# Kiteretsu77/This_and_That_VDM

Measured on AMD Instinct MI355X. Metric: denoise-steps/sec (14-frame 256x448 VGL, 25 steps), higher is better.
Workload: dtype bf16; 1 GPU; VGL denoise step: GestureNet ControlNet + spatio-temporal UNet + per-frame CFG + Euler, latent 14x4x32x56, CFG batch 2, 78 context tokens, heads (5,10,20,20); mode=vgl, requests_per_gpu=1, parallelism=1 independent request(s), one per GPU; RCCL weight broadcast at start-up only, hipgraph=True, finite_output=True, spatial_self_attention=bf16, weights_identical_on_all_ranks=True

## Files before the change

this_and_that_vdm_amd/csrc/gemm.hip:

```cpp
#include <stdlib.h>
#include "gemm_kernel.h"

namespace ttg {
void launch_bf16(GemmP& p, int cfg, hipStream_t st);
void launch_f16(GemmP& p, int cfg, hipStream_t st);
void launch_f32(GemmP& p, int cfg, hipStream_t st);
void launch_sq320_bf16(const GemmP& p, hipStream_t st);
void launch_sq320_f16(const GemmP& p, hipStream_t st);
void launch_pp_bf16(GemmP& p, hipStream_t st);
void launch_pp_f16(GemmP& p, hipStream_t st);
void launch_w320_bf16(GemmP& p, hipStream_t st);
void launch_w320_f16(GemmP& p, hipStream_t st);
void launch_w320h_bf16(GemmP& p, hipStream_t st);
void launch_w320h_f16(GemmP& p, hipStream_t st);
}
using namespace ttg;

namespace {
inline int gemm_taps(int mode) { return mode == 1 || mode == 3 ? 9 : (mode == 2 ? 3 : 1); }

int env_int(const char* name, int dflt) { const char* e = getenv(name); return e ? atoi(e) : dflt; }
int big_tile_bits(int on) { return on == 0 ? 0 : (on == 2 ? 1 : (on == 3 ? 11 : (on == 4 ? 7 : 15))); }
struct Knobs {
  int forced_cfg = env_int("TT_GEMM_CFG", -1);
  int group_m = env_int("TT_GEMM_GROUP_M", 0);
  int forced_split = env_int("TT_GEMM_SPLITK", -1);
  int deep = env_int("TT_GEMM_DEEP", 1);
  int small64 = env_int("TT_GEMM_SMALL64", 2);
  int sq320 = env_int("TT_GEMM_SQ320", 2);
  int sq320_rowvec = env_int("TT_SQ320_ROWVEC", 1);
  int sq320_min_rows = env_int("TT_SQ320_MIN_ROWS", 131072);
  int pp = env_int("TT_GEMM_PP", 1);
  int pp_geglu_min_tiles = env_int("TT_PP_GEGLU_MIN_TILES", 400);
  int pp_geglu_min_fill = env_int("TT_PP_GEGLU_MIN_FILL", 75);
  int pp_min_tiles = env_int("TT_PP_MIN_TILES", 460);
  int pp_min_fill = env_int("TT_PP_MIN_FILL", 90);
  int pp_split_whole = env_int("TT_PP_SPLIT_WHOLE", 1);
  int w320 = big_tile_bits(env_int("TT_GEMM_W320", 1));
  int w320_force = env_int("TT_W320_FORCE", 0);
  int w320_min_fill = env_int("TT_W320_MIN_FILL", 60);
  int f32_split = env_int("TT_F32_SPLIT", 0) ? 1 : 0;
  int f32_split_min_tiles = env_int("TT_F32_SPLIT_MIN_TILES", 160);
  int f32_splitk = env_int("TT_F32_SPLITK", 1);
};
Knobs& knobs() { static Knobs k; return k; }

struct Plan { int cfg, splitk; };

Plan make_plan(int forced, int m, int n, long ktot, bool allow_split, bool wide_ok = true, bool mode0 = false, bool k128 = false) {
  Plan pl{0, 1};
  const int f = forced;
  const long b128 = (long)ceil_div(m, 128) * ceil_div(n, 128);
  const long b12864 = (long)ceil_div(m, 128) * ceil_div(n, 64);
  if (f >= 0 && f < kNumCfgs) pl.cfg = f;
  else if (n % 160 == 0 && n % 128 != 0 && n <= 960 && m >= 2048) pl.cfg = 7;
  else if (m >= 8192 && n >= 1024 && wide_ok) pl.cfg = 3;
  else if (m < 2048 && n >= 2560 && n % 160 == 0) pl.cfg = 7;
  else if (b128 >= 384) pl.cfg = 11;
  else if (b12864 >= 384) pl.cfg = 1;
  else pl.cfg = 2;
  const int fs = knobs().forced_split;
  if (fs >= 1) { pl.splitk = allow_split ? fs : 1; return pl; }
  const long kt = (ktot + 63) / 64;
  const int deep = knobs().deep;
  if (deep && f < 0 && b128 <= 256 && ktot > 0) {
    const int small64 = knobs().small64;
    if (small64 && (small64 != 2 || (m <= 64 && n >= 4096)) && mode0 && ktot <= 2048 && (long)ceil_div(m, 64) * ceil_div(n, 64) <= 512) { pl.cfg = 2; return pl; }
    pl.cfg = (deep == 2 && k128) ? 20 : 16;
    long s = allow_split ? 256 / b128 : 1;
    if (s > kt / 8) s = kt / 8;
    if (s > 16) s = 16;
    pl.splitk = s >= 2 ? (int)s : 1;
    return pl;
  }
  if (allow_split && f < 0 && b128 < 384 && kt >= 40) {
    long s = (512 + b128 - 1) / b128;
    if (s > kt / 8) s = kt / 8;
    if (s > 16) s = 16;
    if (s >= 2) { pl.cfg = 11; pl.splitk = (int)s; }
  }
  return pl;
}

int plan_f32(int m, int n, int min_tiles = 256) { return (long)ceil_div(m, 128) * ceil_div(n, 128) >= min_tiles ? 0 : 1; }

bool sq320_rowvec_ok(const TtGemmArgs* a) {
  if (!a->rowvec) return true;
  if (!knobs().sq320_rowvec || !a->residual) return false;
  if (a->rowvec_mod == 2 && a->rowvec_rows == 1) return true;
  return a->rowvec_mod == 0 && a->rowvec_rows >= 32 && a->rowvec_rows % 32 == 0 && (long)a->rowvec_rows * 2 >= a->m;
}
bool sq320_ok(const TtGemmArgs* a) {
  const int on = knobs().sq320;
  if (on == 2 && a->m < knobs().sq320_min_rows) return false;
  return on && a->dtype != TT_F32 && !a->ln_fold && !a->out_fp8 && knobs().forced_cfg < 0 && a->mode == 0 && a->k1 == 0 && a->k0 == SQ_K && a->n == SQ_N && a->m >= 4096 &&
         !a->geglu && sq320_rowvec_ok(a) && !a->out_f32 && !a->out_col_hw &&
         (!a->blend || (a->blend == a->residual && a->ld_blend == a->ld_res));
}
bool pp_ok(const TtGemmArgs* a) {
  const Knobs& k = knobs();
  if (!k.pp || k.forced_cfg >= 0 || a->dtype == TT_F32 || a->mode != 0 || a->k1 != 0 || a->ln_fold > 1 || a->out_fp8 || a->residual || a->blend ||
      a->rowvec || a->out_f32 || a->out_col_hw || (a->k0 & 63) || a->k0 < 128 || (a->n & 15) || (a->ldo & 7))
    return false;
  const long tiles = (long)ceil_div(a->m, 256) * ceil_div(a->n, 256);
  const long rounds = (tiles + 255) / 256;
  if (a->geglu) return tiles >= k.pp_geglu_min_tiles && tiles * 100 >= rounds * 256 * k.pp_geglu_min_fill;
  return tiles >= k.pp_min_tiles && tiles * 100 >= rounds * 256 * k.pp_min_fill;
}
bool w320_eligible(const TtGemmArgs* a) {
  if (!knobs().w320 || knobs().forced_cfg >= 0 || a->mode == 3 || a->dtype == TT_F32 || a->n % 320 || (a->k0 & 63) || (a->k1 & 63) || gemm_taps(a->mode) * (a->k0 + a->k1) < 128 || a->geglu ||
      a->out_fp8 || a->out_f32 || a->out_col_hw || a->ln_fold > 1 || (a->ln_fold && (a->mode != 0 || a->k1)))
    return false;
  if (a->mode == 1 && (a->stride != 1 || a->upsample || a->hin != a->hout || a->win != a->wout || a->win >= 32768 || a->hin >= 32768)) return false;
  if (a->rowvec && a->rowvec_rows < 32 && !(a->rowvec_rows == 1 && a->rowvec_mod == 2)) return false;
  if ((a->ldo & 3) || (a->residual && (a->ld_res & 3)) || (a->blend && (a->ld_blend & 3)) || (a->rowvec && (a->ld_rowvec & 3))) return false;
  if ((((size_t)a->out | (size_t)a->residual | (size_t)a->blend) & 7) || (((size_t)a->rowvec | (size_t)a->bias) & 15)) return false;
  return true;
}
int w320_route(const TtGemmArgs* a) {
  if (!w320_eligible(a)) return 0;
  const Knobs& k = knobs();
  if (k.w320_force == 1 || k.w320_force == 2) return k.w320_force;
  for (int half = 0; half < 2; ++half) {
    if (half && (!(k.w320 & 2) || ((k.w320 & 4) && a->mode != 1))) break;
    const long tiles = (long)ceil_div(a->m, half ? 128 : 256) * (a->n / 320);
    const long rounds = (tiles + 255) / 256;
    if (tiles * 100 >= rounds * 256 * k.w320_min_fill) return 1 + half;
  }
  return 0;
}
int w320_split(const TtGemmArgs* a) {
  const int bits = knobs().w320;
  if (!w320_eligible(a) || !(bits & 8) || a->ln_fold || a->mode == 2) return 0;
  const long tiles = (long)ceil_div(a->m, 128) * (a->n / 320);
  if ((bits & 4) && (a->mode != 1 || tiles < 64)) return 0;
  const long slabs = (long)gemm_taps(a->mode) * (a->k0 + a->k1) / 64;
  long s = 256 / tiles;
  const long by_k = slabs / (a->mode == 1 ? 20 : 32);
  if (s > by_k) s = by_k;
  if (s > 16) s = 16;
  if (s < 2 || tiles * s < 160 || s * a->m * a->n * 4 >= (1L << 31)) return 0;
  return (int)s;
}
size_t slab_bytes(const TtGemmArgs* a, int split) { return (size_t)split * a->m * a->n * sizeof(float); }
bool ws_fits(const TtGemmArgs* a, int split) { return a->ws && (size_t)a->ws_bytes >= slab_bytes(a, split); }
int pp_head_rows(const TtGemmArgs* a, bool served) {
  if (a->m < 512) return 0;
  if ((a->m & 255) == 0 && (!knobs().pp_split_whole || served)) return 0;
  TtGemmArgs head = *a;
  for (int tr = a->m >> 8; tr >= 2 && (long)(a->m - tr * 256) * 8 <= a->m; --tr) {
    head.m = tr * 256;
    if (head.m < a->m && pp_ok(&head)) return head.m;
  }
  return 0;
}
void pp_split(const TtGemmArgs* a, int rows, TtGemmArgs* head, TtGemmArgs* tail) {
  const size_t es = 2;
  *head = *a; *tail = *a;
  head->m = rows;
  tail->m = a->m - rows;
  tail->a0 = (const char*)a->a0 + (size_t)rows * a->lda0 * es;
  tail->out = (char*)a->out + (size_t)rows * a->ldo * es;
}

const TileCfg& tile_of(int dtype, int cfg) { return dtype == TT_F32 ? kCfgsF32[cfg] : kCfgs[cfg]; }
bool ln_capable(int cfg) { return kCfgs[cfg].ln; }
bool mode3_capable(int cfg) { return kCfgs[cfg].m3; }
Plan mode3_plan(const TtGemmArgs* a, Plan pl) {
  if (a->mode != 3 || a->dtype == TT_F32 || knobs().forced_cfg >= 0 || mode3_capable(pl.cfg)) return pl;
  if (pl.cfg == 20) return Plan{16, pl.splitk};
  const long b128 = (long)ceil_div(a->m, 128) * ceil_div(a->n, 128), b12864 = (long)ceil_div(a->m, 128) * ceil_div(a->n, 64);
  return Plan{b128 >= 384 ? 11 : (b12864 >= 384 ? 1 : 2), 1};
}
bool mode3_served(const TtGemmArgs* a, const Plan& pl) { return a->mode != 3 || tile_of(a->dtype, pl.cfg).m3; }
Plan plan_for(const TtGemmArgs* a) {
  if (a->dtype == TT_F32) {
    const int split_min = knobs().f32_split_min_tiles;
    if (knobs().f32_split) {
      const long b128 = (long)ceil_div(a->m, 128) * ceil_div(a->n, 128);
      const long kt = (long)gemm_taps(a->mode) * (a->k0 + a->k1) / 32;
      if (knobs().f32_splitk && !a->geglu && !a->ln_fold && !a->out_col_hw && b128 < split_min && kt >= 64) {
        long sp = 448 / b128;
        if (sp > kt / 16) sp = kt / 16;
        if (sp > 16) sp = 16;
        if (sp >= 2) return Plan{0, (int)sp};
      }
    }
    return Plan{plan_f32(a->m, a->n, knobs().f32_split ? split_min : 256), 1};
  }
  const long ktot = (long)gemm_taps(a->mode) * (a->k0 + a->k1);
  const bool allow = !a->geglu && !a->ln_fold && !a->out_fp8;
  const bool k128 = (a->k0 & 127) == 0 && (a->k1 & 127) == 0;
  const bool wide_ok = !(a->residual || a->blend || a->rowvec);
  Plan pl = make_plan(knobs().forced_cfg, a->m, a->n, ktot, allow, wide_ok, a->mode == 0, k128);
  if (a->ln_fold && !ln_capable(pl.cfg))
    pl = make_plan(-1, a->m, a->n, ktot, false, wide_ok, a->mode == 0);
  return mode3_plan(a, pl);
}
Plan unsplit_plan(const TtGemmArgs* a) {
  if (a->dtype == TT_F32) return Plan{plan_f32(a->m, a->n, 256), 1};
  return mode3_plan(a, Plan{make_plan(knobs().forced_cfg, a->m, a->n, 0, false, !(a->residual || a->blend || a->rowvec)).cfg, 1});
}

enum class Kind { PP, PP_TWO_PART, SQ320, W320, W320H, W320H_SPLIT, TILED, UNSUPPORTED };
struct Route { Kind kind; int cfg; int splitk; int head_rows; };

Route tiled_route(const TtGemmArgs* a, Plan pl) { return Route{mode3_served(a, pl) ? Kind::TILED : Kind::UNSUPPORTED, pl.cfg, pl.splitk, 0}; }
Route wanted_route(const TtGemmArgs* a) {
  if (pp_ok(a)) return Route{Kind::PP, -1, 1, 0};
  const bool sq = sq320_ok(a);
  const int big = w320_route(a);
  if (const int rows = pp_head_rows(a, sq || big)) return Route{Kind::PP_TWO_PART, -1, 1, rows};
  if (sq) return Route{Kind::SQ320, -1, 1, 0};
  if (big) return Route{big == 1 ? Kind::W320 : Kind::W320H, -1, 1, 0};
  if (const int split = w320_split(a)) return Route{Kind::W320H_SPLIT, -1, split, 0};
  return tiled_route(a, plan_for(a));
}
Route granted_route(const TtGemmArgs* a, Route r) {
  if (r.kind == Kind::W320H_SPLIT && !ws_fits(a, r.splitk)) r = tiled_route(a, plan_for(a));
  if (r.kind == Kind::TILED && r.splitk > 1 && (!ws_fits(a, r.splitk) || slab_bytes(a, r.splitk) >= ((size_t)1 << 31))) r = tiled_route(a, unsplit_plan(a));
  return r;
}
Route resolve(const TtGemmArgs* a) { return granted_route(a, wanted_route(a)); }

TileCfg route_tile(const TtGemmArgs* a, const Route& r) {
  switch (r.kind) {
    case Kind::PP: case Kind::PP_TWO_PART: return TileCfg{-1, 256, 256, 64, 0, 2, 4};
    case Kind::SQ320: return TileCfg{-1, SQ_ROWS, SQ_N, SQ_K, a->residual ? 3 : 5, 1, SQ_WAVES};
    case Kind::W320: return TileCfg{-1, 256, 320, 64, 0, 4, 2};
    case Kind::W320H: case Kind::W320H_SPLIT: return TileCfg{-1, 128, 320, 64, 0, 2, 2};
    default: return tile_of(a->dtype, r.cfg);
  }
}

int32_t stats_rows_on(const TtGemmArgs* a, const Route& r) {
  if (a->geglu || a->out_fp8 || a->out_f32 || a->out_col_hw > 0 || a->ln_fold == 2) return 0;
  if (r.kind == Kind::PP || r.kind == Kind::PP_TWO_PART || r.kind == Kind::SQ320 || r.kind == Kind::UNSUPPORTED) return 0;
  const int seg = a->stats_seg;
  if (r.splitk != 1) {
    if (seg <= 0) return 0;
    for (int rows = seg < 128 ? seg : 128; rows > 0; --rows)
      if (seg % rows == 0) return a->m % rows == 0 ? rows : 0;
    return 0;
  }
  const TileCfg t = route_tile(a, r);
  if (a->blend && !(a->blend == a->residual && a->ld_blend == a->ld_res)) return 0;
  if (a->rowvec && a->rowvec_rows < 32 && !(a->rowvec_rows == 1 && a->rowvec_mod == 2)) return 0;
  if (t.bm > 128 && t.bn != 320 && a->residual) return 0;
  if (a->dtype == TT_F32 && knobs().f32_split && a->residual) return 0;
  if (t.bn == 320 || t.nst == 0) {
    if (a->m % t.bm) return 0;
    return (t.bm == 128 && seg > 0 && seg % 128 && seg % 64 == 0) ? 64 : t.bm;
  }
  const int wave_rows = t.bm / t.wgm;
  const int rows = (seg <= 0 || seg % t.bm == 0) ? t.bm : (seg % wave_rows == 0 ? wave_rows : t.bm);
  return a->m % rows == 0 ? rows : 0;
}
int32_t gn_fused_on(const TtGemmArgs* a, const Route& r) {
  if (a->dtype == TT_F32 || a->geglu || a->out_fp8 || a->out_f32 || a->out_col_hw > 0 || a->stats_out) return 0;
  const int seg = a->stats_seg;
  if (seg <= 0 || a->m % seg || (a->n & 127)) return 0;
  if (r.kind != Kind::W320H_SPLIT && r.kind != Kind::TILED) return 0;
  if (r.splitk <= 1) return 0;
  return splitk_gn_rows(seg, a->n, nullptr) > 0 ? 1 : 0;
}
}

int tt_internal_f32_split() { return knobs().f32_split; }

extern "C" int tt_gemm_set_tile_override(int32_t cfg) {
  if (cfg < -1 || cfg >= kNumCfgs) TT_FAIL(TT_EINVAL, "tt_gemm_set_tile_override: cfg %d (valid -1..%d)", cfg, kNumCfgs - 1);
  knobs().forced_cfg = cfg;
  return TT_OK;
}
extern "C" int tt_gemm_set_streaming_square(int32_t on) {
  knobs().sq320 = on == 2 ? 2 : (on ? 1 : 0);
  return TT_OK;
}
extern "C" int tt_gemm_set_f32_split(int32_t on) { knobs().f32_split = on ? 1 : 0; return TT_OK; }
extern "C" int tt_gemm_set_big_tile(int32_t on) { knobs().w320 = big_tile_bits(on); return TT_OK; }

extern "C" int tt_gemm_plan(const TtGemmArgs* a, int32_t cfg[7]) {
  if (!a || !cfg || a->m <= 0 || a->n <= 0) TT_FAIL(TT_EINVAL, "tt_gemm_plan: bad arguments");
  const Route r = resolve(a);
  if (r.kind == Kind::UNSUPPORTED)
    TT_FAIL(TT_EUNSUPPORTED, "tt_gemm_plan: forced tile configuration %d has no mode-3 variant (mode 3 is built for 1, 2, 11, 16)", r.cfg);
  const TileCfg t = route_tile(a, r);
  cfg[0] = t.bm; cfg[1] = t.bn; cfg[2] = t.bk; cfg[3] = t.nst; cfg[4] = t.wgm; cfg[5] = t.wgn; cfg[6] = r.splitk;
  return TT_OK;
}

extern "C" int32_t tt_gemm_stats_rows(const TtGemmArgs* a) {
  if (!a || a->m <= 0 || a->n <= 0) return 0;
  return stats_rows_on(a, resolve(a));
}

extern "C" int32_t tt_gemm_gn_fused(const TtGemmArgs* a) {
  if (!a || a->m <= 0 || a->n <= 0) return 0;
  return gn_fused_on(a, resolve(a));
}

extern "C" size_t tt_gemm_ws_bytes(const TtGemmArgs* a) {
  if (!a || a->m <= 0 || a->n <= 0) return 0;
  const Route r = wanted_route(a);
  if (r.kind == Kind::PP_TWO_PART) { TtGemmArgs head, tail; pp_split(a, r.head_rows, &head, &tail); return tt_gemm_ws_bytes(&tail); }
  return (r.kind == Kind::W320H_SPLIT || r.kind == Kind::TILED) && r.splitk > 1 ? slab_bytes(a, r.splitk) : 0;
}

namespace {
int fill_params(const TtGemmArgs* a, const Route& r, GemmP& p) {
  if (a->geglu && ((a->n & 15) || a->residual || a->blend || a->rowvec || a->out_f32 || a->out_col_hw))
    TT_FAIL(TT_EINVAL, "tt_gemm: geglu needs n %% 16 == 0 and no other epilogue terms");
  if (a->rowvec && a->rowvec_rows <= 0) TT_FAIL(TT_EINVAL, "tt_gemm: rowvec_rows");
  if (a->gn_out) {
    if (!a->gn_gamma || !a->gn_beta || (a->ld_gn & 3) || ((size_t)a->gn_out & 7)) TT_FAIL(TT_EINVAL, "tt_gemm: gn_out needs gn_gamma, gn_beta, ld_gn %% 4 == 0 and an 8-byte aligned pointer");
    if (!gn_fused_on(a, r)) TT_FAIL(TT_EUNSUPPORTED, "tt_gemm: gn_out on a problem without a split-K reduction pass (tt_gemm_gn_fused(args) == 0)");
  }
  if (a->stats_out && stats_rows_on(a, r) == 0)
    TT_FAIL(TT_EUNSUPPORTED, "tt_gemm: stats_out on a route without a statistics epilogue (tt_gemm_stats_rows(args) == 0)");
  if (a->rowvec_mod < 0 || (a->rowvec_mod > 0 && !a->rowvec)) TT_FAIL(TT_EINVAL, "tt_gemm: rowvec_mod %d (>= 0, needs rowvec)", a->rowvec_mod);
  if (a->ln_fold < 0 || a->ln_fold > 2) TT_FAIL(TT_EINVAL, "tt_gemm: ln_fold %d (0 none, 1 rows of A, 2 rows of W)", a->ln_fold);
  if (a->ln_fold && (a->mode != 0 || a->k1 != 0 || !(a->ln_eps > 0.f)))
    TT_FAIL(TT_EINVAL, "tt_gemm: ln_fold needs mode 0, one source spanning the whole LayerNorm row (k0 = C) and ln_eps > 0");
  if (a->ln_fold == 2 && a->geglu) TT_FAIL(TT_EINVAL, "tt_gemm: ln_fold 2 (columns) cannot be combined with geglu");
  if (a->out_fp8 && (a->dtype == TT_F32 || a->mode != 0 || a->geglu || a->residual || a->blend || a->rowvec || a->out_f32 || (a->ldo & 3)))
    TT_FAIL(TT_EINVAL, "tt_gemm: out_fp8 is for plain 16-bit linears (no geglu / residual / blend / rowvec / fp32 out), ldo %% 4 == 0");
  p.a0 = (const char*)a->a0; p.a1 = (const char*)a->a1; p.k0 = a->k0; p.k1 = a->k1;
  p.lda0 = a->lda0; p.lda1 = a->lda1; p.w = (const char*)a->w; p.ldw = a->ldw;
  p.m = a->m; p.n = a->n; p.mode = a->mode;
  p.nimg = a->nimg; p.hin = a->hin; p.win = a->win; p.hout = a->hout; p.wout = a->wout;
  p.stride = a->stride; p.upsample = a->upsample; p.frames = a->frames; p.hw = a->hw;
  p.bias = a->bias; p.acc_scale = a->acc_scale;
  p.rowvec = a->rowvec; p.rowvec_rows = a->rowvec_rows; p.ld_rowvec = a->ld_rowvec; p.rowvec_mod = a->rowvec ? a->rowvec_mod : 0;
  p.geglu = a->geglu; p.residual = (const char*)a->residual; p.ld_res = a->ld_res;
  p.blend = (const char*)a->blend; p.ld_blend = a->ld_blend; p.alpha = a->alpha;
  const int es = a->dtype == TT_F32 ? 4 : 2;
  p.out = (char*)a->out; p.ldo = a->ldo; p.out_f32 = a->dtype == TT_F32 ? 0 : a->out_f32;
  p.out_col_hw = a->out_col_hw; p.out_col_hwp = a->out_col_hwp;
  p.ln_fold = a->ln_fold; p.ln_eps = a->ln_eps; p.out_fp8 = a->out_fp8; p.stats = a->stats_out; p.stat_rows = a->gn_out ? a->stats_seg : (a->stats_out ? stats_rows_on(a, r) : 0);
  p.f32_split = a->dtype == TT_F32 ? knobs().f32_split : 0;
  p.presplit = a->presplit;
  if (a->presplit) {
    if ((a->presplit & ~3) || a->dtype != TT_F32 || !p.f32_split)
      TT_FAIL(TT_EINVAL, "tt_gemm: presplit operands need TT_F32 with tt_gemm_set_f32_split(1)");
    if (((a->presplit & 1) && a->ln_fold == 1) || ((a->presplit & 2) && a->ln_fold == 2))
      TT_FAIL(TT_EINVAL, "tt_gemm: the LayerNorm statistics cannot be taken from a pre-split operand");
    if ((a->presplit & 1) && a->mode != 0) TT_FAIL(TT_EINVAL, "tt_gemm: a pre-split A operand is a Linear operand (mode 0)");
  }
  p.gn_out = (char*)a->gn_out; p.ld_gn = a->ld_gn; p.gn_gamma = a->gn_gamma; p.gn_beta = a->gn_beta; p.gn_eps = a->gn_eps; p.gn_silu = a->gn_silu;
  if (p.mode == 1 || p.mode == 3) {
    if (p.nimg <= 0 || p.hin <= 0 || p.win <= 0 || p.hout <= 0 || p.wout <= 0 || p.stride < 1)
      TT_FAIL(TT_EINVAL, "tt_gemm: conv geometry");
    if ((long)p.nimg * p.hout * p.wout != p.m) TT_FAIL(TT_EINVAL, "tt_gemm: m != nimg*hout*wout");
  }
  if (p.mode == 2) {
    if (p.frames <= 0 || p.hw <= 0 || p.m % ((long)p.frames * p.hw)) TT_FAIL(TT_EINVAL, "tt_gemm: tconv geometry");
  }
  p.taps = gemm_taps(p.mode);
  {
    const long rows = p.mode == 1 || p.mode == 3 ? (long)p.nimg * p.hin * p.win : (long)p.m;
    const long a0b = ((rows - 1) * p.lda0 + p.k0) * es, a1b = p.k1 ? ((rows - 1) * p.lda1 + p.k1) * es : 16;
    const long wb = ((long)(p.n - 1) * p.ldw + (long)p.taps * (p.k0 + p.k1)) * es;
    if (a0b >= (1L << 31) || a1b >= (1L << 31) || wb >= (1L << 31))
      TT_FAIL(TT_EUNSUPPORTED, "tt_gemm: operand larger than 2 GiB (32-bit buffer offsets)");
    p.a0_bytes = (unsigned)a0b; p.a1_bytes = (unsigned)a1b; p.w_bytes = (unsigned)wb;
    const long n_out = p.geglu ? p.n / 2 : p.n;
    const long outb = ((long)(p.m - 1) * p.ldo + (p.out_col_hw > 0 ? p.ldo : n_out)) * (p.out_f32 ? 4 : (p.out_fp8 ? 1 : es));
    const long resb = p.residual ? ((long)(p.m - 1) * p.ld_res + p.n) * es : 0;
    const long blb = p.blend ? ((long)(p.m - 1) * p.ld_blend + p.n) * es : 0;
    long rv_last = p.rowvec ? (p.m - 1) / p.rowvec_rows : 0;
    if (p.rowvec_mod > 0 && rv_last > p.rowvec_mod - 1) rv_last = p.rowvec_mod - 1;
    const long rvb = p.rowvec ? (rv_last * p.ld_rowvec + p.n) * 4 : 0;
    if (outb >= (1L << 31) || resb >= (1L << 31) || blb >= (1L << 31) || rvb >= (1L << 31))
      TT_FAIL(TT_EUNSUPPORTED, "tt_gemm: epilogue operand larger than 2 GiB (32-bit buffer offsets)");
    p.out_bytes = (unsigned)outb; p.res_bytes = (unsigned)resb; p.blend_bytes = (unsigned)blb;
    p.bias_bytes = p.bias ? (unsigned)p.n * 4u : 0u; p.rowvec_bytes = (unsigned)rvb;
  }
  p.splitk = r.splitk; p.group_m = 1;
  p.group_m_override = r.kind == Kind::PP || r.kind == Kind::TILED ? knobs().group_m : 0;
  p.ws = r.splitk > 1 ? (float*)a->ws : nullptr;
  p.ws_bytes = r.splitk > 1 ? (unsigned)slab_bytes(a, r.splitk) : 0u;
  return TT_OK;
}
}

extern "C" int tt_gemm(const TtGemmArgs* a, tt_stream_t stream) {
  if (!a || !a->a0 || !a->w || !a->out) TT_FAIL(TT_EINVAL, "tt_gemm: null operand");
  if (a->m <= 0 || a->n <= 0 || a->k0 <= 0) TT_FAIL(TT_EINVAL, "tt_gemm: empty problem m=%d n=%d k0=%d", a->m, a->n, a->k0);
  if (a->dtype != TT_BF16 && a->dtype != TT_F16 && a->dtype != TT_F32) TT_FAIL(TT_EINVAL, "tt_gemm: bad dtype");
  if ((a->k0 & 7) || (a->k1 & 7) || (a->n & 3)) TT_FAIL(TT_EINVAL, "tt_gemm: k0/k1 must be multiples of 8 and n of 4");
  if ((a->lda0 & 7) || (a->k1 && (a->lda1 & 7)) || (a->ldw & 7)) TT_FAIL(TT_EINVAL, "tt_gemm: row strides must be multiples of 8 elements");
  if (a->k1 && !a->a1) TT_FAIL(TT_EINVAL, "tt_gemm: k1 > 0 without a1");
  if (a->mode < 0 || a->mode > 3) TT_FAIL(TT_EINVAL, "tt_gemm: bad mode %d", a->mode);
  if (a->mode == 3 && a->upsample) TT_FAIL(TT_EINVAL, "tt_gemm: mode 3 (bottom / right zero padding) has no fused upsample");
  const Route r = resolve(a);
  if (r.kind == Kind::PP_TWO_PART) {
    TtGemmArgs head, tail;
    pp_split(a, r.head_rows, &head, &tail);
    const int rc = tt_gemm(&head, stream);
    return rc != TT_OK ? rc : tt_gemm(&tail, stream);
  }
  GemmP p;
  if (const int rc = fill_params(a, r, p)) return rc;
  hipStream_t st = (hipStream_t)stream;
  const bool bf16 = a->dtype == TT_BF16;
  switch (r.kind) {
    case Kind::PP: if (bf16) launch_pp_bf16(p, st); else launch_pp_f16(p, st); break;
    case Kind::SQ320: if (bf16) launch_sq320_bf16(p, st); else launch_sq320_f16(p, st); break;
    case Kind::W320: if (bf16) launch_w320_bf16(p, st); else launch_w320_f16(p, st); break;
    case Kind::W320H: case Kind::W320H_SPLIT: if (bf16) launch_w320h_bf16(p, st); else launch_w320h_f16(p, st); break;
    case Kind::TILED:
      if (bf16) launch_bf16(p, r.cfg, st);
      else if (a->dtype == TT_F16) launch_f16(p, r.cfg, st);
      else launch_f32(p, r.cfg, st);
      break;
    default:
      TT_FAIL(TT_EUNSUPPORTED, "tt_gemm: forced tile configuration %d has no mode-3 variant (mode 3 is built for 1, 2, 11, 16)", r.cfg);
  }
  TT_CHECK_LAUNCH("tt_gemm");
  return TT_OK;
}
```

this_and_that_vdm_amd/csrc/gemm_kernel.h:

```cpp
#pragma once
#include <stdlib.h>
#include <type_traits>
#include "common.h"

namespace ttg {


struct FastDiv { unsigned mul, sh; };
static inline FastDiv make_fastdiv(long d_) {
  unsigned long long d = d_ < 1 ? 1 : (unsigned long long)d_;
  unsigned l = 0;
  while ((1ull << l) < d) ++l;
  FastDiv f;
  f.mul = (unsigned)(((1ull << (31 + l)) + d - 1) / d);
  f.sh = 31 + l;
  return f;
}
__device__ __forceinline__ int fdiv(int n, const FastDiv& f) { return (int)(((unsigned long long)(unsigned)n * f.mul) >> f.sh); }

struct GemmP {
  const char* a0; const char* a1;
  int k0, k1; long lda0, lda1;
  const char* w; long ldw;
  int m, n, mode;
  int nimg, hin, win, hout, wout, stride, upsample;
  int frames, hw;
  const float* bias; float acc_scale;
  const float* rowvec; int rowvec_rows; long ld_rowvec;
  int rowvec_mod;
  int geglu;
  const char* residual; long ld_res;
  const char* blend; long ld_blend; float alpha;
  char* out; long ldo; int out_f32;
  int out_col_hw, out_col_hwp;
  int nk0, nk1, taps, kt_total;
  int tiles_m, tiles_n;
  int group_m_override;
  int group_m;
  unsigned a0_bytes, a1_bytes, w_bytes;
  unsigned out_bytes, res_bytes, blend_bytes, bias_bytes, rowvec_bytes, ws_bytes;
  int splitk;
  float* ws;
  int ln_fold; float ln_eps;
  int out_fp8;
  float* stats;
  int stat_rows;
  char* gn_out; long ld_gn;
  const float* gn_gamma; const float* gn_beta; float gn_eps; int gn_silu;
  int f32_split;
  int presplit;
  FastDiv fd_splitk, fd_per_group, fd_group_m, fd_last_rows, fd_per_tap, fd_hwo, fd_wout, fd_hw, fd_frames, fd_rv_rows, fd_rv_mod;
};

__device__ __forceinline__ unsigned pack4_fp8(const float* v) {
  int w = 0;
  w = __builtin_amdgcn_cvt_pk_fp8_f32(__builtin_amdgcn_fmed3f(v[0], -448.f, 448.f), __builtin_amdgcn_fmed3f(v[1], -448.f, 448.f), w, false);
  w = __builtin_amdgcn_cvt_pk_fp8_f32(__builtin_amdgcn_fmed3f(v[2], -448.f, 448.f), __builtin_amdgcn_fmed3f(v[3], -448.f, 448.f), w, true);
  return (unsigned)w;
}
__device__ __forceinline__ void st32(__amdgpu_buffer_rsrc_t r, int off, unsigned a) {
  __builtin_amdgcn_raw_buffer_store_b32(a, r, off, 0, 0);
}

__device__ __forceinline__ void colstat_strip(const char* ebuf, int q_per_row, int lane, float* srow_sum, float* srow_sq, bool first) {
  if (lane < q_per_row * 4) {
    const int quad = lane >> 2, e4 = (lane & 3) * 4;
    float a = 0.f, b = 0.f;
#pragma unroll 8
    for (int r = 0; r < 32; ++r) {
      const float x = *(const float*)(ebuf + r * 256 + ((quad ^ (r & (q_per_row - 1))) << 4) + e4);
      a += x; b = fmaf(x, x, b);
    }
    if (!first) { a += srow_sum[lane]; b += srow_sq[lane]; }
    srow_sum[lane] = a; srow_sq[lane] = b;
  }
}

__device__ __forceinline__ void ln_stat_shifted(const raw_u32x4_t& f, float c, float& s, float& q) {
  const unsigned w[4] = {f.x, f.y, f.z, f.w};
#pragma unroll
  for (int d = 0; d < 4; ++d) { const float x = __uint_as_float(w[d]) - c; s += x; q = fmaf(x, x, q); }
}


#ifdef TT_GEMM_TIMELINE
static __device__ long long g_tl[8 * 8192];
#define TL(i) do { if (threadIdx.x == 0 && blockIdx.x < 8192) g_tl[blockIdx.x * 8 + (i)] = wall_clock64(); } while (0)
#else
#define TL(i) do { } while (0)
#endif

constexpr int kInv = (int)0x80000000;
typedef unsigned u32x2_t __attribute__((ext_vector_type(2)));
typedef unsigned u32x4_t __attribute__((ext_vector_type(4)));
__device__ __forceinline__ __amdgpu_buffer_rsrc_t make_rsrc(const void* ptr, unsigned bytes) {
  return __builtin_amdgcn_make_buffer_rsrc((void*)ptr, 0, (int)bytes, 0x00020000);
}
__device__ __forceinline__ uint2 ld64(__amdgpu_buffer_rsrc_t r, int off) {
  const u32x2_t v = __builtin_amdgcn_raw_buffer_load_b64(r, off, 0, 0);
  return make_uint2(v.x, v.y);
}
__device__ __forceinline__ float4 ld128f(__amdgpu_buffer_rsrc_t r, int off) {
  const u32x4_t v = __builtin_amdgcn_raw_buffer_load_b128(r, off, 0, 0);
  return make_float4(__uint_as_float(v.x), __uint_as_float(v.y), __uint_as_float(v.z), __uint_as_float(v.w));
}
__device__ __forceinline__ void st64(__amdgpu_buffer_rsrc_t r, int off, unsigned a, unsigned b) {
  __builtin_amdgcn_raw_buffer_store_b64((u32x2_t){a, b}, r, off, 0, 0);
}
__device__ __forceinline__ void st128f(__amdgpu_buffer_rsrc_t r, int off, float4 v) {
  __builtin_amdgcn_raw_buffer_store_b128((u32x4_t){__float_as_uint(v.x), __float_as_uint(v.y), __float_as_uint(v.z), __float_as_uint(v.w)}, r, off, 0, 0);
}
template <typename Tag> __device__ __forceinline__ typename Elem<Tag>::quad_t ldq(__amdgpu_buffer_rsrc_t r, int off) { return ld64(r, off); }
template <> __device__ __forceinline__ uint4 ldq<f32_tag>(__amdgpu_buffer_rsrc_t r, int off) {
  const u32x4_t v = __builtin_amdgcn_raw_buffer_load_b128(r, off, 0, 0);
  return make_uint4(v.x, v.y, v.z, v.w);
}
template <typename Tag> __device__ __forceinline__ void stq(__amdgpu_buffer_rsrc_t r, int off, const float* v) {
  st64(r, off, pack2<Tag>(v[0], v[1]), pack2<Tag>(v[2], v[3]));
}
template <> __device__ __forceinline__ void stq<f32_tag>(__amdgpu_buffer_rsrc_t r, int off, const float* v) {
  st128f(r, off, make_float4(v[0], v[1], v[2], v[3]));
}
template <typename Tag> __device__ __forceinline__ typename Elem<Tag>::quad_t zero_quad();
template <> __device__ __forceinline__ uint2 zero_quad<bf16_tag>() { return make_uint2(0, 0); }
template <> __device__ __forceinline__ uint2 zero_quad<f16_tag>() { return make_uint2(0, 0); }
template <> __device__ __forceinline__ uint4 zero_quad<f32_tag>() { return make_uint4(0, 0, 0, 0); }

template <typename Tag> struct EpiOps { float4 bias, rv; typename Elem<Tag>::quad_t res, bl; };
template <typename Tag>
__device__ __forceinline__ EpiOps<Tag> epi_load(const GemmP& p, int gm, int gn) {
  typedef typename Elem<Tag>::quad_t quad_t;
  constexpr int ES = Elem<Tag>::ES;
  EpiOps<Tag> o;
  o.bias = o.rv = make_float4(0.f, 0.f, 0.f, 0.f);
  o.res = o.bl = zero_quad<Tag>();
  if (p.bias) o.bias = *(const float4*)(p.bias + gn);
  if (p.rowvec) {
    int rg = gm / p.rowvec_rows;
    if (p.rowvec_mod > 0) rg %= p.rowvec_mod;
    o.rv = *(const float4*)(p.rowvec + (long)rg * p.ld_rowvec + gn);
  }
  if (p.residual) o.res = *(const quad_t*)(p.residual + ((long)gm * p.ld_res + gn) * ES);
  if (p.blend) o.bl = *(const quad_t*)(p.blend + ((long)gm * p.ld_blend + gn) * ES);
  return o;
}
template <typename Tag>
__device__ __forceinline__ void epi_finish(const GemmP& p, const EpiOps<Tag>& o, int gm, int gn, float (&v)[4]) {
  typedef typename Elem<Tag>::quad_t quad_t;
  constexpr int ES = Elem<Tag>::ES;
  if (p.bias) { v[0] += o.bias.x; v[1] += o.bias.y; v[2] += o.bias.z; v[3] += o.bias.w; }
#pragma unroll
  for (int e = 0; e < 4; ++e) v[e] *= p.acc_scale;
  if (p.rowvec) { v[0] += o.rv.x; v[1] += o.rv.y; v[2] += o.rv.z; v[3] += o.rv.w; }
  if (p.residual) {
    float r4[4];
    quad_to_f32<Tag>(o.res, r4);
#pragma unroll
    for (int e = 0; e < 4; ++e) v[e] += r4[e];
  }
  if (p.blend) {
    float r4[4];
    quad_to_f32<Tag>(o.bl, r4);
#pragma unroll
    for (int e = 0; e < 4; ++e) v[e] = p.alpha * r4[e] + (1.0f - p.alpha) * v[e];
  }
  if (p.out_fp8) {
    if (p.out_col_hw > 0) {
      const unsigned w = pack4_fp8(v);
#pragma unroll
      for (int e = 0; e < 4; ++e) {
        const int c = gn + e;
        const long oc = (long)(c / p.out_col_hw) * p.out_col_hwp + (c % p.out_col_hw);
        *(unsigned char*)(p.out + (long)gm * p.ldo + oc) = (unsigned char)(w >> (8 * e));
      }
    } else {
      *(unsigned*)(p.out + (long)gm * p.ldo + gn) = pack4_fp8(v);
    }
  } else if (p.out_f32) {
    *(float4*)(p.out + ((long)gm * p.ldo + gn) * 4) = make_float4(v[0], v[1], v[2], v[3]);
  } else if (p.out_col_hw > 0) {
#pragma unroll
    for (int e = 0; e < 4; ++e) {
      const int c = gn + e;
      const long oc = (long)(c / p.out_col_hw) * p.out_col_hwp + (c % p.out_col_hw);
      store1<Tag>(p.out + ((long)gm * p.ldo + oc) * ES, v[e]);
    }
  } else {
    *(quad_t*)(p.out + ((long)gm * p.ldo + gn) * ES) = f32_to_quad<Tag>(v);
  }
}

template <typename Tag>
__device__ __forceinline__ void epilogue_quad(const GemmP& p, int gm, int gn, float (&v)[4]) {
  const EpiOps<Tag> o = epi_load<Tag>(p, gm, gn);
  epi_finish<Tag>(p, o, gm, gn, v);
}

template <int N> __device__ __forceinline__ void wait_vmcnt() {
  asm volatile("s_waitcnt vmcnt(%0)" ::"n"(N) : "memory");
}
template <int G> __device__ __forceinline__ void wait_tiles(int tiles) {
  static_assert(3 * G <= 63, "vmcnt field is 6 bits");
  if (tiles <= 0) wait_vmcnt<0>();
  else if (tiles == 1) wait_vmcnt<G>();
  else if (tiles == 2) wait_vmcnt<2 * G>();
  else wait_vmcnt<3 * G>();
}

constexpr int gemm_lds_bytes(int BM, int BN, int CPR, int NST, int NT) {
  return NST * (((BM * CPR + NT - 1) / NT) + ((BN * CPR + NT - 1) / NT)) * NT * 16;
}
constexpr int gemm_min_waves(int BM, int BN, int CPR, int NST, int NT) {
  const int blocks = (160 * 1024) / gemm_lds_bytes(BM, BN, CPR, NST, NT) >= 2 ? 2 : 1;
  const int w = blocks * (NT / 64) / 4;
  return w < 1 ? 1 : w;
}

template <typename Tag, int BM, int BN, int BK, int NST, int WGM, int WGN, int KMODE_>
__global__ __launch_bounds__(64 * WGM * WGN, gemm_min_waves(BM, BN, BK / Elem<Tag>::EPC, NST, 64 * WGM * WGN))
void gemm_kernel(const GemmP p) {
  extern __shared__ __attribute__((aligned(16))) char smem[];
  constexpr bool SPLIT = (KMODE_ & 8) != 0;
  constexpr bool PRE_B = (KMODE_ & 16) != 0, PRE_A = (KMODE_ & 32) != 0;
  constexpr int KMODE = KMODE_ & 7;
  static_assert(SPLIT || (!PRE_A && !PRE_B), "pre-split operands belong to the split variants");
  static_assert(!SPLIT || std::is_same<Tag, f32_tag>::value, "split products are a TT_F32 mode");
  constexpr bool PAD_BR = KMODE == 5;
  constexpr int MODE = PAD_BR ? 1 : (KMODE >= 3 ? 0 : KMODE);
  constexpr int LN = KMODE == 3 || KMODE == 4 ? KMODE - 2 : 0;
  TL(0);
  kernarg_touch<sizeof(GemmP)>();
  typedef typename Elem<Tag>::quad_t quad_t;
  constexpr int ES = Elem<Tag>::ES, EPC = Elem<Tag>::EPC;
  constexpr int NT = 64 * WGM * WGN;
  constexpr int CPR = BK / EPC;
  constexpr int WTM = BM / WGM, WTN = BN / WGN, FM = WTM / 32, FN = WTN / 32;
  constexpr int AR = (BM * CPR + NT - 1) / NT, BR = (BN * CPR + NT - 1) / NT;
  constexpr int A_BYTES = AR * NT * 16, B_BYTES = BR * NT * 16, STAGE = A_BYTES + B_BYTES;
  constexpr int G = AR + BR;
  constexpr int RPI = NT / CPR;
  static_assert(NT % CPR == 0 && NST >= 2 && NST <= 5 && WTM % 32 == 0 && WTN % 32 == 0, "tile/threads mismatch");

  const int tid = threadIdx.x, lane = tid & 63;
  const int wid = __builtin_amdgcn_readfirstlane(tid >> 6);

  int bid = blockIdx.x;
  {
    const int nwg = gridDim.x, q = nwg >> 3, r = nwg & 7, xcd = bid & 7, idx = bid >> 3;
    bid = (xcd < r ? xcd * (q + 1) : r * (q + 1) + (xcd - r) * q) + idx;
  }
  int split = 0;
  if (p.splitk > 1) { const int t = fdiv(bid, p.fd_splitk); split = bid - t * p.splitk; bid = t; }
  int tile_m, tile_n;
  {
    const int gm = p.group_m;
    const int per_group = gm * p.tiles_n;
    const int grp = fdiv(bid, p.fd_per_group);
    const int first = grp * gm;
    const int r = bid - grp * per_group;
    const bool full = first + gm <= p.tiles_m;
    const int rows = full ? gm : p.tiles_m - first;
    tile_n = full ? fdiv(r, p.fd_group_m) : fdiv(r, p.fd_last_rows);
    tile_m = first + (r - tile_n * rows);
  }
  const int m0 = tile_m * BM, n0 = tile_n * BN;
  const int kt_lo = p.splitk > 1 ? fdiv(p.kt_total * split, p.fd_splitk) : 0;
  const int KT = p.splitk > 1 ? fdiv(p.kt_total * (split + 1), p.fd_splitk) - kt_lo : p.kt_total;

  constexpr int INV = (int)0x80000000;
  const __amdgpu_buffer_rsrc_t ra0 = __builtin_amdgcn_make_buffer_rsrc((void*)p.a0, 0, p.a0_bytes, 0x00020000);
  const __amdgpu_buffer_rsrc_t ra1 = __builtin_amdgcn_make_buffer_rsrc((void*)(p.a1 ? p.a1 : p.a0), 0, p.a1_bytes, 0x00020000);
  const __amdgpu_buffer_rsrc_t rw = __builtin_amdgcn_make_buffer_rsrc((void*)p.w, 0, p.w_bytes, 0x00020000);
  const int crow = tid / CPR, cchunk = tid % CPR;
  int a_chunk[AR];
  int va0[AR], va1[AR];
  int a_img[AR], a_y[AR], a_x[AR];
  bool a_valid[AR];
#pragma unroll
  for (int i = 0; i < AR; ++i) {
    const int r = i * RPI + crow;
    a_chunk[i] = cchunk ^ tile_swz<CPR>(r);
    const int gm = m0 + r;
    a_valid[i] = gm < p.m && r < BM;
    const int g = a_valid[i] ? gm : 0;
    va0[i] = va1[i] = INV;
    a_img[i] = a_y[i] = a_x[i] = 0;
    if constexpr (MODE == 0) {
      if (a_valid[i]) {
        va0[i] = (int)(((long)g * p.lda0 + a_chunk[i] * EPC) * ES);
        va1[i] = (int)(((long)g * p.lda1 + a_chunk[i] * EPC) * ES);
      }
    } else if constexpr (MODE == 1) {
      const int hwo = p.hout * p.wout;
      a_img[i] = fdiv(g, p.fd_hwo);
      const int rem = g - a_img[i] * hwo;
      a_y[i] = fdiv(rem, p.fd_wout);
      a_x[i] = rem - a_y[i] * p.wout;
    } else {
      const int fr = fdiv(g, p.fd_hw);
      a_img[i] = fr - fdiv(fr, p.fd_frames) * p.frames;
      a_y[i] = g;
    }
  }
  int b_chunk[BR], vb[BR];
#pragma unroll
  for (int i = 0; i < BR; ++i) {
    const int r = i * RPI + crow;
    b_chunk[i] = cchunk ^ tile_swz<CPR>(r);
    const int gn = n0 + r;
    vb[i] = (gn < p.n && r < BN) ? (int)(((long)gn * p.ldw + b_chunk[i] * EPC) * ES) : INV;
  }

  int s_tap, s_src, s_kc;
  {
    const int per_tap = p.nk0 + p.nk1;
    s_tap = kt_lo ? fdiv(kt_lo, p.fd_per_tap) : 0;
    const int rem = kt_lo - s_tap * per_tap;
    s_src = rem >= p.nk0 ? 1 : 0;
    s_kc = rem - (s_src ? p.nk0 : 0);
  }
  bool tap_dirty = true;
  auto stage = [&](int slot) {
    if constexpr (MODE != 0) {
      if (tap_dirty) {
        tap_dirty = false;
#pragma unroll
        for (int i = 0; i < AR; ++i) {
          bool ok = a_valid[i];
          long row;
          if constexpr (MODE == 1) {
            constexpr int OFF = PAD_BR ? 0 : 1;
            const int dy = s_tap / 3 - OFF, dx = s_tap - (dy + OFF) * 3 - OFF;
            int iy = a_y[i] * p.stride + dy, ix = a_x[i] * p.stride + dx;
            const bool up = !PAD_BR && p.upsample;
            const int hv = up ? p.hin * 2 : p.hin, wv = up ? p.win * 2 : p.win;
            ok = ok && iy >= 0 && iy < hv && ix >= 0 && ix < wv;
            if (up) { iy >>= 1; ix >>= 1; }
            row = ((long)a_img[i] * p.hin + iy) * p.win + ix;
          } else {
            const int f = a_img[i] + s_tap - 1;
            ok = ok && f >= 0 && f < p.frames;
            row = (long)a_y[i] + (long)(s_tap - 1) * p.hw;
          }
          va0[i] = ok ? (int)((row * p.lda0 + a_chunk[i] * EPC) * ES) : INV;
          va1[i] = ok ? (int)((row * p.lda1 + a_chunk[i] * EPC) * ES) : INV;
        }
      }
    }
    const int src = __builtin_amdgcn_readfirstlane(s_src);
    const int ksrc = src ? p.k1 : p.k0;
    const int kbase = __builtin_amdgcn_readfirstlane(s_kc) * BK;
    const bool tail = kbase + BK > ksrc;
    char* lds_a = smem + slot * STAGE + wid * 1024;
    char* lds_b = smem + slot * STAGE + A_BYTES + wid * 1024;
    const int soff_a = kbase * ES;
    const int soff_w = __builtin_amdgcn_readfirstlane(
        (int)(((long)s_tap * (p.k0 + p.k1) + (src ? p.k0 : 0) + kbase) * ES));
    auto issue = [&](const __amdgpu_buffer_rsrc_t& ra, const int (&va)[AR], auto has_tail) {
#pragma unroll
      for (int i = 0; i < AR; ++i) {
        int v = va[i];
        if constexpr (decltype(has_tail)::value) { if (kbase + a_chunk[i] * EPC >= ksrc) v = INV; }
        __builtin_amdgcn_raw_ptr_buffer_load_lds(ra, (__attribute__((address_space(3))) void*)(lds_a + i * (NT * 16)), 16, v, soff_a, 0, 0);
      }
#pragma unroll
      for (int i = 0; i < BR; ++i) {
        int v = vb[i];
        if constexpr (decltype(has_tail)::value) { if (kbase + b_chunk[i] * EPC >= ksrc) v = INV; }
        __builtin_amdgcn_raw_ptr_buffer_load_lds(rw, (__attribute__((address_space(3))) void*)(lds_b + i * (NT * 16)), 16, v, soff_w, 0, 0);
      }
    };
    if (!tail) {
      if (!src) issue(ra0, va0, std::false_type{}); else issue(ra1, va1, std::false_type{});
    } else {
      if (!src) issue(ra0, va0, std::true_type{}); else issue(ra1, va1, std::true_type{});
    }
    if (++s_kc == (s_src ? p.nk1 : p.nk0)) {
      s_kc = 0;
      if (s_src == 0 && p.nk1 > 0) s_src = 1;
      else { s_src = 0; ++s_tap; tap_dirty = true; }
    }
  };

  const int wr = wid / WGN, wc = wid - wr * WGN;
  f32x16_t acc[FM][FN];
#pragma unroll
  for (int i = 0; i < FM; ++i)
#pragma unroll
    for (int j = 0; j < FN; ++j)
#pragma unroll
      for (int r = 0; r < 16; ++r) acc[i][j][r] = 0.f;

  const int l31 = lane & 31, hi = lane >> 5;
  int a_lds_row[FM], b_lds_row[FN];
#pragma unroll
  for (int i = 0; i < FM; ++i) a_lds_row[i] = wr * WTM + i * 32 + l31;
#pragma unroll
  for (int j = 0; j < FN; ++j) b_lds_row[j] = wc * WTN + j * 32 + l31;

  constexpr int KS = CPR / 2;
  static_assert(KS % 2 == 0, "the pipelined loop reads fragment sets in pairs");
  constexpr int NF = FM + FN;
  const unsigned lds_base = lds_addr(smem);
  auto read_frags = [&](unsigned sa, int ks, raw_u32x4_t (&af)[FM], raw_u32x4_t (&bf)[FN]) {
    const unsigned sb = sa + A_BYTES;
    const int chunk = ks * 2 + hi;
#pragma unroll
    for (int i = 0; i < FM; ++i) af[i] = lds_read16_raw(sa + tile_off<CPR>(a_lds_row[i], chunk));
#pragma unroll
    for (int j = 0; j < FN; ++j) bf[j] = lds_read16_raw(sb + tile_off<CPR>(b_lds_row[j], chunk));
  };
  constexpr int NLN = LN == 1 ? FM : (LN == 2 ? FN : 1);
  float ln_s[NLN], ln_q[NLN];
#pragma unroll
  for (int i = 0; i < NLN; ++i) ln_s[i] = ln_q[i] = 0.f;
  constexpr bool LN_SHIFT = LN != 0 && std::is_same<Tag, f32_tag>::value;
  float ln_c[LN_SHIFT ? NLN : 1];
  if constexpr (LN_SHIFT) {
#pragma unroll
    for (int i = 0; i < NLN; ++i) {
      const int row = LN == 1 ? m0 + a_lds_row[i] : n0 + b_lds_row[i];
      const bool ok = row < (LN == 1 ? p.m : p.n);
      ln_c[i] = ok ? *(const float*)((LN == 1 ? p.a0 : p.w) + (long)row * (LN == 1 ? p.lda0 : p.ldw) * 4) : 0.f;
    }
  }
  uint2 sp_ah[SPLIT ? FM : 1], sp_al[SPLIT ? FM : 1], sp_bh[SPLIT ? FN : 1], sp_bl[SPLIT ? FN : 1];
  f32x16_t accx[SPLIT ? FM : 1][SPLIT ? FN : 1];
  if constexpr (SPLIT) {
#pragma unroll
    for (int i = 0; i < FM; ++i)
#pragma unroll
      for (int j = 0; j < FN; ++j)
#pragma unroll
        for (int r = 0; r < 16; ++r) accx[i][j][r] = 0.f;
  }
  const float kM2048 = -2048.0f;
  auto split4 = [&](const raw_u32x4_t& f, bool pre, uint2& h, uint2& l) {
    if (pre) { h = make_uint2(f.x, f.y); l = make_uint2(f.z, f.w); return; }
    const f32x2_t v01 = (f32x2_t){__uint_as_float(f.x), __uint_as_float(f.y)}, v23 = (f32x2_t){__uint_as_float(f.z), __uint_as_float(f.w)};
    const f16x2_t h01 = __builtin_convertvector(v01 * 0.00390625f, f16x2_t), h23 = __builtin_convertvector(v23 * 0.00390625f, f16x2_t);
    h = make_uint2(__builtin_bit_cast(unsigned, h01), __builtin_bit_cast(unsigned, h23));
    const f32x2_t e01 = v01 * 8.0f, e23 = v23 * 8.0f;
    unsigned l01, l23;
    asm("v_fma_mixlo_f16 %0, %1, %2, %3 op_sel_hi:[1,0,0]" : "=v"(l01) : "v"(h.x), "v"(kM2048), "v"(e01.x));
    asm("v_fma_mixhi_f16 %0, %1, %2, %3 op_sel:[1,0,0] op_sel_hi:[1,0,0]" : "+v"(l01) : "v"(h.x), "v"(kM2048), "v"(e01.y));
    asm("v_fma_mixlo_f16 %0, %1, %2, %3 op_sel_hi:[1,0,0]" : "=v"(l23) : "v"(h.y), "v"(kM2048), "v"(e23.x));
    asm("v_fma_mixhi_f16 %0, %1, %2, %3 op_sel:[1,0,0] op_sel_hi:[1,0,0]" : "+v"(l23) : "v"(h.y), "v"(kM2048), "v"(e23.y));
    l = make_uint2(l01, l23);
  };
#if defined(TT_SPLIT_ABL) && (TT_SPLIT_ABL & 1)
  constexpr bool pre_a = true, pre_b = true;
#else
  constexpr bool pre_a = PRE_A, pre_b = PRE_B;
#endif
#ifndef TT_SPLIT_PIPE
#define TT_SPLIT_PIPE 1
#endif
#ifndef TT_SPLIT_PIPE_ROWS
#define TT_SPLIT_PIPE_ROWS 99
#endif
  constexpr int PIPE_SPLIT_ROWS = FM > 1 ? (TT_SPLIT_PIPE_ROWS < FM ? TT_SPLIT_PIPE_ROWS : FM) : FM;
  uint4 op_ah[SPLIT ? FM : 1], op_al[SPLIT ? FM : 1], op_bh[SPLIT ? FN : 1], op_bl[SPLIT ? FN : 1];
  if constexpr (SPLIT) {
#pragma unroll
    for (int i = 0; i < FM; ++i) op_ah[i] = op_al[i] = make_uint4(0, 0, 0, 0);
#pragma unroll
    for (int j = 0; j < FN; ++j) op_bh[j] = op_bl[j] = make_uint4(0, 0, 0, 0);
  }
  auto split4c = [&](const raw_u32x4_t& f, bool pre, uint2& h, uint2& l) {
    if (pre) { h = make_uint2(f.x, f.y); l = make_uint2(f.z, f.w); return; }
    const f32x2_t v01 = (f32x2_t){__uint_as_float(f.x), __uint_as_float(f.y)}, v23 = (f32x2_t){__uint_as_float(f.z), __uint_as_float(f.w)};
    const f16x2_t h01 = __builtin_convertvector(v01 * 0.00390625f, f16x2_t), h23 = __builtin_convertvector(v23 * 0.00390625f, f16x2_t);
    h = make_uint2(__builtin_bit_cast(unsigned, h01), __builtin_bit_cast(unsigned, h23));
    const f32x2_t r01 = v01 * 8.0f - __builtin_convertvector(h01, f32x2_t) * 2048.0f, r23 = v23 * 8.0f - __builtin_convertvector(h23, f32x2_t) * 2048.0f;
    l = make_uint2(__builtin_bit_cast(unsigned, __builtin_convertvector(r01, f16x2_t)), __builtin_bit_cast(unsigned, __builtin_convertvector(r23, f16x2_t)));
  };
  auto issue_pending = [&](auto lo_tag, auto hi_tag) {
   constexpr int LO = decltype(lo_tag)::value, HI = decltype(hi_tag)::value;
   if constexpr (SPLIT) {
#if !defined(TT_SPLIT_ABL) || !(TT_SPLIT_ABL & 2)
#pragma unroll
    for (int i = LO; i < HI; ++i)
#pragma unroll
// ... 124 lines not shown
      const __amdgpu_buffer_rsrc_t r_res = make_rsrc(p.residual, p.res_bytes);
#pragma unroll
      for (int i = 0; i < FM; ++i)
#pragma unroll
        for (int c = 0; c < NCH; ++c) {
          const int nfr = (2 * c + 1 < FN) ? 2 : 1;
          const int q_per_row = nfr * 8, rows_per_pass = 64 / q_per_row;
          const int gn = n0 + wc * WTN + c * 64 + (lane % q_per_row) * 4;
#pragma unroll
          for (int pass = 0; pass < 8; ++pass) {
            resv[i][c][pass] = zero_quad<Tag>();
            if (pass * rows_per_pass < 32) {
              const int gm = m0 + wr * WTM + i * 32 + pass * rows_per_pass + lane / q_per_row;
              resv[i][c][pass] = ldq<Tag>(r_res, (gm < p.m && gn < p.n) ? (int)(((long)gm * p.ld_res + gn) * ES) : kInv);
            }
          }
        }
    }
  };
  if constexpr (NST == 2) {
    TL(6);
    stage(0);
    TL(7);
    preload_residual();
    TL(1);
    for (int kt = 0; kt < KT; ++kt) {
      wait_vmcnt<0>();
      __builtin_amdgcn_s_barrier();
      asm volatile("" ::: "memory");
#ifdef TT_GEMM_TIMELINE
      if (kt == 0) TL(2);
#endif
      if (kt + 1 < KT) stage((kt + 1) & 1);
      const unsigned sa = lds_base + (kt & 1) * STAGE;
      raw_u32x4_t af[2][FM], bf[2][FN];
      read_frags(sa, 0, af[0], bf[0]);
#pragma unroll
      for (int ks = 0; ks < KS; ++ks) {
        if (ks + 1 < KS) {
          read_frags(sa, ks + 1, af[(ks + 1) & 1], bf[(ks + 1) & 1]);
          lds_wait<NF>();
        } else {
          lds_wait<0>();
        }
        mma(af[ks & 1], bf[ks & 1], ks & 1);
      }
    }
  } else {
    TL(6);
    preload_residual();
    TL(1);
#pragma unroll
    for (int s = 0; s < NST - 1; ++s)
      if (s < KT) stage(s);
    wait_tiles<G>(min(KT - 1, NST - 2));
    __builtin_amdgcn_s_barrier();
    asm volatile("" ::: "memory");
    raw_u32x4_t afA[FM], bfA[FN], afB[FM], bfB[FN];
    read_frags(lds_base, 0, afA, bfA);
    int slot = 0, fill = NST - 1;
    auto tile = [&](int kt, auto last_tag) {
      constexpr bool LAST = decltype(last_tag)::value;
      const unsigned sa = lds_base + slot * STAGE;
      const int nslot = slot + 1 == NST ? 0 : slot + 1;
#pragma unroll
      for (int ks = 0; ks < KS; ks += 2) {
        read_frags(sa, ks + 1, afB, bfB);
        lds_wait<NF>();
        mma(afA, bfA, 0);
        if (ks + 2 < KS) {
          read_frags(sa, ks + 2, afA, bfA);
          lds_wait<NF>();
        } else if constexpr (!LAST) {
          wait_tiles<G>(min(KT - 2 - kt, NST - 3));
          __builtin_amdgcn_s_barrier();
          asm volatile("" ::: "memory");
          if (kt + NST - 1 < KT) stage(fill);
          read_frags(lds_base + nslot * STAGE, 0, afA, bfA);
          lds_wait<NF>();
        } else {
          lds_wait<0>();
        }
        mma(afB, bfB, 1);
      }
      slot = nslot;
      fill = fill + 1 == NST ? 0 : fill + 1;
    };
    for (int kt = 0; kt + 1 < KT; ++kt) tile(kt, std::false_type{});
    tile(KT - 1, std::true_type{});
  }

  if constexpr (SPLIT && TT_SPLIT_PIPE) issue_pending(std::integral_constant<int, 0>{}, std::integral_constant<int, FM>{});
  if constexpr (SPLIT) {
#pragma unroll
    for (int i = 0; i < FM; ++i)
#pragma unroll
      for (int j = 0; j < FN; ++j)
#pragma unroll
        for (int r = 0; r < 16; ++r) acc[i][j][r] = fmaf(accx[i][j][r], 32.0f, acc[i][j][r] * 65536.0f);
  }
  constexpr int CS_OFF = NST * STAGE;
  constexpr int STAT_OFF = NST * STAGE + (KMODE == 4 ? WGM * WGN * 1024 : 0);
  if constexpr (LN != 0) {
    const float inv_k = 1.0f / (float)p.k0;
    float rs[NLN];
#pragma unroll
    for (int i = 0; i < NLN; ++i) {
      const float sm = (ln_s[i] + __shfl_xor(ln_s[i], 32)) * inv_k, sq = (ln_q[i] + __shfl_xor(ln_q[i], 32)) * inv_k;
      rs[i] = rsqrtf(fmaxf(sq - sm * sm, 0.f) + p.ln_eps);
    }
    if constexpr (LN == 1) {
#pragma unroll
      for (int i = 0; i < FM; ++i)
#pragma unroll
        for (int j = 0; j < FN; ++j)
#pragma unroll
          for (int r = 0; r < 16; ++r) acc[i][j][r] *= rs[i];
    } else {
      float* cs = (float*)(smem + CS_OFF + wid * 1024);
#pragma unroll
      for (int j = 0; j < FN; ++j) cs[j * 32 + l31] = rs[j];
    }
  }
  const float* colscale = (const float*)(smem + CS_OFF + wid * 1024);

  TL(3);
  if (!direct) {
    const __amdgpu_buffer_rsrc_t r_bias = make_rsrc(p.bias, p.bias_bytes);
    const __amdgpu_buffer_rsrc_t r_out = p.splitk > 1 ? make_rsrc(p.ws, p.ws_bytes) : make_rsrc(p.out, p.out_bytes);
    auto strip_off = [](int row, int quad, int nq) { return row * 256 + ((quad ^ (row & (nq - 1))) << 4); };
    char* ebuf = smem + wid * 8192;
    static_assert(WGM * WGN * 8192 <= NST * STAGE, "epilogue strips do not fit the ring");
    if (!p.geglu) {
      float4 bias4[NCH];
#pragma unroll
      for (int c = 0; c < NCH; ++c) {
        const int q_per_row = ((2 * c + 1 < FN) ? 2 : 1) * 8;
        const int gn = n0 + wc * WTN + c * 64 + (lane % q_per_row) * 4;
        bias4[c] = ld128f(r_bias, gn < p.n ? gn * 4 : kInv);
      }
      const float alpha = p.blend ? p.alpha : 0.0f, one_m_alpha = 1.0f - alpha;
      __syncthreads();
      TL(4);
      auto run = [&](auto film_tag, auto inpass_tag, auto out8_tag, auto stats_tag) {
        constexpr bool FILM = decltype(film_tag)::value, INPASS = decltype(inpass_tag)::value, OUT8 = decltype(out8_tag)::value;
        constexpr bool STATS = decltype(stats_tag)::value;
        const __amdgpu_buffer_rsrc_t r_rv = make_rsrc(p.rowvec, (FILM || INPASS) ? p.rowvec_bytes : 0);
        const __amdgpu_buffer_rsrc_t r_bl = make_rsrc(p.blend, INPASS ? p.blend_bytes : 0);
        const __amdgpu_buffer_rsrc_t r_res = make_rsrc(p.residual, (INPASS && !EARLY_RES) ? p.res_bytes : 0);
        const int rv_rows = p.rowvec ? p.rowvec_rows : 1;
        const bool parity = FILM && p.rowvec_mod == 2 && rv_rows == 1;
        auto wrap = [&](int g) { return p.rowvec_mod > 0 ? g - fdiv(g, p.fd_rv_mod) * p.rowvec_mod : g; };
        float* sstage = (float*)(smem + STAT_OFF) + wid * (2 * WTN);
#pragma unroll
        for (int i = 0; i < FM; ++i) {
          const int mb = m0 + wr * WTM + i * 32;
          const int grp_raw = fdiv(mb, p.fd_rv_rows);
          const int grp0 = parity ? 0 : wrap(grp_raw), grp1 = parity ? 1 : wrap(grp_raw + 1);
          const int grp_split = parity ? mb : (grp_raw + 1) * rv_rows;
          const int sel_split = parity ? 0x7fffffff : grp_split, sel_odd = parity ? 1 : 0;
#pragma unroll
          for (int jc = 0; jc < FN; jc += 2) {
            const int nfr = (jc + 1 < FN) ? 2 : 1;
            const int q_per_row = nfr * 8;
            const int rows_per_pass = 64 / q_per_row;
            const int qq = lane % q_per_row, rr = lane / q_per_row;
            const int gn = n0 + wc * WTN + jc * 32 + qq * 4;
            const float4 b4 = bias4[jc / 2];
            float4 cs4 = make_float4(1.f, 1.f, 1.f, 1.f);
            if constexpr (LN == 2) cs4 = *(const float4*)(colscale + jc * 32 + qq * 4);
            float4 film_lo = make_float4(0.f, 0.f, 0.f, 0.f), film_hi = film_lo;
            if constexpr (FILM) {
              film_lo = ld128f(r_rv, (mb < p.m && gn < p.n) ? (int)(((long)grp0 * p.ld_rowvec + gn) * 4) : kInv);
              film_hi = ld128f(r_rv, (grp_split < p.m && gn < p.n) ? (int)(((long)grp1 * p.ld_rowvec + gn) * 4) : kInv);
            }
#pragma unroll
            for (int jj = 0; jj < 2; ++jj) {
              if (jc + jj < FN) {
#pragma unroll
                for (int g = 0; g < 4; ++g)
                  *(float4*)(ebuf + strip_off(l31, jj * 8 + 2 * g + hi, nfr * 8)) =
                      make_float4(acc[i][jc + jj][g * 4], acc[i][jc + jj][g * 4 + 1], acc[i][jc + jj][g * 4 + 2], acc[i][jc + jj][g * 4 + 3]);
              }
            }
            constexpr int PB = INPASS ? (BM > 128 ? 2 : 4) : 8;
#pragma unroll
            for (int pb = 0; pb < 8; pb += PB) {
              quad_t rqv[PB], blv[PB];
              float4 rvv[PB];
#pragma unroll
              for (int k = 0; k < PB; ++k) {
                const int pass = pb + k;
                rqv[k] = blv[k] = zero_quad<Tag>();
                rvv[k] = make_float4(0.f, 0.f, 0.f, 0.f);
                if (pass * rows_per_pass < 32) {
                  const int gm = mb + pass * rows_per_pass + rr;
                  const bool ok = gm < p.m && gn < p.n;
                  if constexpr (EARLY_RES) rqv[k] = resv[i][jc / 2][pass];
                  else if constexpr (INPASS) rqv[k] = ldq<Tag>(r_res, ok ? (int)(((long)gm * p.ld_res + gn) * ES) : kInv);
                  if constexpr (INPASS) {
                    rvv[k] = ld128f(r_rv, ok ? (int)(((long)wrap(fdiv(gm, p.fd_rv_rows)) * p.ld_rowvec + gn) * 4) : kInv);
                    blv[k] = ldq<Tag>(r_bl, ok ? (int)(((long)gm * p.ld_blend + gn) * ES) : kInv);
                  }
                }
              }
#pragma unroll
              for (int k = 0; k < PB; ++k) {
                const int pass = pb + k;
                if (pass * rows_per_pass < 32) {
                  const int r = pass * rows_per_pass + rr;
                  const float4 t = *(const float4*)(ebuf + strip_off(r, qq, q_per_row));
                  const int gm = mb + r;
                  const bool ok = gm < p.m && gn < p.n;
                  if (p.splitk > 1) {
                    st128f(r_out, ok ? (int)((((long)split * p.m + gm) * p.n + gn) * 4) : kInv, t);
                  } else {
                    float v[4] = {(t.x * cs4.x + b4.x) * p.acc_scale, (t.y * cs4.y + b4.y) * p.acc_scale,
                                  (t.z * cs4.z + b4.z) * p.acc_scale, (t.w * cs4.w + b4.w) * p.acc_scale};
                    const quad_t rq = rqv[k];
                    quad_t bq = rq;
                    if constexpr (FILM) {
                      const float4 f = ((gm >= sel_split) | ((gm & sel_odd) != 0)) ? film_hi : film_lo;
                      v[0] += f.x; v[1] += f.y; v[2] += f.z; v[3] += f.w;
                    }
                    if constexpr (INPASS) {
                      v[0] += rvv[k].x; v[1] += rvv[k].y; v[2] += rvv[k].z; v[3] += rvv[k].w;
                      bq = (p.blend && !blend_is_res) ? blv[k] : rq;
                    }
                    float r4[4], b4v[4];
                    quad_to_f32<Tag>(rq, r4);
                    quad_to_f32<Tag>(bq, b4v);
#pragma unroll
                    for (int e = 0; e < 4; ++e) v[e] = alpha * b4v[e] + one_m_alpha * (v[e] + r4[e]);
                    if constexpr (OUT8) st32(r_out, ok ? (int)((long)gm * p.ldo + gn) : kInv, pack4_fp8(v));
                    else {
                      const quad_t packed = f32_to_quad<Tag>(v);
                      if constexpr (ES == 2) st64(r_out, ok ? (int)(((long)gm * p.ldo + gn) * ES) : kInv, packed.x, packed.y);
                      else stq<Tag>(r_out, ok ? (int)(((long)gm * p.ldo + gn) * ES) : kInv, v);
                      if constexpr (STATS) {
                        float sv[4];
                        quad_to_f32<Tag>(packed, sv);
                        const bool live = gm < p.m;
                        *(float4*)(ebuf + strip_off(r, qq, q_per_row)) = make_float4(live ? sv[0] : 0.f, live ? sv[1] : 0.f, live ? sv[2] : 0.f, live ? sv[3] : 0.f);
                      }
                    }
                  }
                }
              }
            }
            if constexpr (STATS) colstat_strip(ebuf, q_per_row, lane, sstage + jc * 32, sstage + WTN + jc * 32, i == 0);
          }
        }
      };
      const bool inpass = (p.blend && !blend_is_res) || (p.rowvec && p.rowvec_rows < 32 && !(p.rowvec_mod == 2 && p.rowvec_rows == 1)) ||
                          (!EARLY_RES && p.residual);
      constexpr std::false_type no{};
      constexpr std::true_type yes{};
      const bool kstats = p.stats && p.splitk == 1;
      if (inpass) run(no, yes, no, no);
      else if (p.rowvec) { if (kstats) run(yes, no, no, yes); else run(yes, no, no, no); }
      else if (MODE == 0 && ES == 2 && p.out_fp8) {
        if constexpr (MODE == 0 && ES == 2) run(no, no, yes, no);
      } else { if (kstats) run(no, no, no, yes); else run(no, no, no, no); }
      if (kstats) {
        __syncthreads();
        const float* st0 = (const float*)(smem + STAT_OFF);
        if (p.stat_rows == BM) {
          for (int c = tid; c < BN; c += NT) {
            const int wcc = c / WTN, col = c - wcc * WTN;
            float a = 0.f, b = 0.f;
#pragma unroll
            for (int w = 0; w < WGM; ++w) {
              const float* row = st0 + (w * WGN + wcc) * (2 * WTN);
              a += row[col]; b += row[WTN + col];
            }
            if (n0 + c < p.n) {
              p.stats[((long)tile_m * 2) * p.n + n0 + c] = a;
              p.stats[((long)tile_m * 2 + 1) * p.n + n0 + c] = b;
            }
          }
        } else {
          for (int c = tid; c < BN * WGM; c += NT) {
            const int w = c / BN, cc = c - w * BN, wcc = cc / WTN, col = cc - wcc * WTN;
            const float* row = st0 + (w * WGN + wcc) * (2 * WTN);
            const long srow = (long)tile_m * WGM + w;
            if (n0 + cc < p.n && srow * WTM < p.m) {
              p.stats[(srow * 2) * p.n + n0 + cc] = row[col];
              p.stats[(srow * 2 + 1) * p.n + n0 + cc] = row[WTN + col];
            }
          }
        }
      }
    } else {
      float4 bval[FN][2], bgate[FN][2];
#pragma unroll
      for (int j = 0; j < FN; ++j)
#pragma unroll
        for (int tt = 0; tt < 2; ++tt) {
          const int gnp = n0 + wc * WTN + j * 32 + tt * 16 + 4 * hi;
          bval[j][tt] = ld128f(r_bias, gnp < p.n ? gnp * 4 : kInv);
          bgate[j][tt] = ld128f(r_bias, gnp < p.n ? (gnp + 8) * 4 : kInv);
        }
      __syncthreads();
      TL(4);
#pragma unroll
      for (int i = 0; i < FM; ++i) {
        const int mb = m0 + wr * WTM + i * 32;
#pragma unroll
        for (int jc = 0; jc < FN; jc += 2) {
          const int nfr = (jc + 1 < FN) ? 2 : 1;
#pragma unroll
          for (int jj = 0; jj < 2; ++jj) {
            if (jc + jj < FN) {
#pragma unroll
              for (int tt = 0; tt < 2; ++tt) {
                const float4 bv = bval[jc + jj][tt], bg = bgate[jc + jj][tt];
                const float bvv[4] = {bv.x, bv.y, bv.z, bv.w}, bgv[4] = {bg.x, bg.y, bg.z, bg.w};
                float v[4];
#pragma unroll
                for (int e = 0; e < 4; ++e)
                  v[e] = (acc[i][jc + jj][(2 * tt) * 4 + e] + bvv[e]) * gelu_erf_f(acc[i][jc + jj][(2 * tt + 1) * 4 + e] + bgv[e]);
                *(float4*)(ebuf + strip_off(l31, jj * 4 + tt * 2 + hi, nfr * 4)) = make_float4(v[0], v[1], v[2], v[3]);
              }
            }
          }
          const int q_per_row = nfr * 4;
          const int rows_per_pass = 64 / q_per_row;
          const int qq = lane % q_per_row, rr = lane / q_per_row;
          const int oc = ((n0 + wc * WTN + jc * 32) >> 1) + qq * 4;
#pragma unroll
          for (int pass = 0; pass < 4; ++pass) {
            if (pass * rows_per_pass < 32) {
              const int r = pass * rows_per_pass + rr;
              const float4 t = *(const float4*)(ebuf + strip_off(r, qq, q_per_row));
              const int gm = mb + r;
              const float t4[4] = {t.x, t.y, t.z, t.w};
              stq<Tag>(r_out, (gm < p.m && oc * 2 < p.n) ? (int)(((long)gm * p.ldo + oc) * ES) : kInv, t4);
            }
          }
        }
      }
    }
#ifdef TT_GEMM_TIMELINE
    __builtin_amdgcn_s_waitcnt(0);
    TL(5);
#endif
    return;
  }
#pragma unroll
  for (int i = 0; i < FM; ++i) {
    const int gm = m0 + wr * WTM + i * 32 + l31;
    if (gm >= p.m) continue;
#pragma unroll
    for (int j = 0; j < FN; ++j) {
      const int nb = n0 + wc * WTN + j * 32;
#pragma unroll
      for (int g = 0; g < 4; ++g) {
        const int gn = nb + 8 * g + 4 * hi;
        if (gn >= p.n) continue;
        float v[4];
#pragma unroll
        for (int e = 0; e < 4; ++e) v[e] = acc[i][j][g * 4 + e];
        if constexpr (LN == 2) {
          const float4 c4 = *(const float4*)(colscale + j * 32 + 8 * g + 4 * hi);
          v[0] *= c4.x; v[1] *= c4.y; v[2] *= c4.z; v[3] *= c4.w;
        }
        epilogue_quad<Tag>(p, gm, gn, v);
      }
    }
  }
}

constexpr int SQ_K = 320, SQ_N = 320, SQ_ROWS = 32, SQ_WAVES = SQ_N / 32, SQ_NT = 64 * SQ_WAVES;
constexpr int SQ_CPR = SQ_K / 8;
constexpr int SQ_TILE_BYTES = SQ_ROWS * SQ_K * 2;
constexpr int SQ_PASSES = SQ_ROWS * SQ_CPR / SQ_NT;
static_assert(SQ_ROWS * SQ_CPR % SQ_NT == 0 && SQ_CPR % 8 == 0, "sq320 staging");
__device__ __forceinline__ int sq_swz(int row) { return (row >> 1) & 7; }
__device__ __forceinline__ int sq_off(int row, int chunk) { return (row * SQ_CPR + (chunk ^ sq_swz(row))) << 4; }

template <typename Tag, bool HAS_RES, bool HAS_RV = false>
__global__ __launch_bounds__(SQ_NT) void sq320_kernel(const GemmP p) {
  extern __shared__ __attribute__((aligned(16))) char smem[];
  constexpr int G = HAS_RES ? 2 * SQ_PASSES : SQ_PASSES;
  constexpr int SLOT = HAS_RES ? 2 * SQ_TILE_BYTES : SQ_TILE_BYTES;
  constexpr int NST = HAS_RES ? 3 : 5;
  constexpr int KS = SQ_K / 16;
  const int tid = threadIdx.x, lane = tid & 63;
  const int wid = __builtin_amdgcn_readfirstlane(tid >> 6);
  const int l31 = lane & 31, hi = lane >> 5;
  const int ntiles = (p.m + SQ_ROWS - 1) / SQ_ROWS;
// ... 145 lines not shown
      const float4 b = *(const float4*)(p.ws + ((long)s2 * p.m + gm) * p.n + gn);
      a.x += b.x; a.y += b.y; a.z += b.z; a.w += b.w;
    }
    float v[4] = {a.x, a.y, a.z, a.w};
    epi_finish<Tag>(p, o, gm, gn, v);
  }
}

template <typename Tag>
__global__ __launch_bounds__(256) void splitk_epilogue_stats_kernel(const GemmP p) {
  __shared__ float red[32][8][8];
  kernarg_touch<sizeof(GemmP)>();
  const int R = p.stat_rows, rt = blockIdx.x, tid = threadIdx.x;
  const int qd = tid & 7, rl = tid >> 3;
  const int gn = (int)blockIdx.y * 32 + qd * 4;
  float cs[4] = {0.f, 0.f, 0.f, 0.f}, cq[4] = {0.f, 0.f, 0.f, 0.f};
  if (gn < p.n) {
    for (int r = rl; r < R; r += 32) {
      const int gm = rt * R + r;
      const EpiOps<Tag> o = epi_load<Tag>(p, gm, gn);
      float4 a = *(const float4*)(p.ws + (long)gm * p.n + gn);
      for (int s2 = 1; s2 < p.splitk; ++s2) {
        const float4 b = *(const float4*)(p.ws + ((long)s2 * p.m + gm) * p.n + gn);
        a.x += b.x; a.y += b.y; a.z += b.z; a.w += b.w;
      }
      float v[4] = {a.x, a.y, a.z, a.w};
      epi_finish<Tag>(p, o, gm, gn, v);
#pragma unroll
      for (int e = 0; e < 4; ++e) { const float x = round_store<Tag>(v[e]); cs[e] += x; cq[e] = fmaf(x, x, cq[e]); }
    }
  }
#pragma unroll
  for (int e = 0; e < 4; ++e) { red[rl][qd][e] = cs[e]; red[rl][qd][4 + e] = cq[e]; }
  __syncthreads();
  if (tid < 64) {
    const int q2 = tid >> 3, e = tid & 7, c = (int)blockIdx.y * 32 + q2 * 4 + (e & 3);
    if (c < p.n) {
      float t = red[0][q2][e];
#pragma unroll
      for (int l = 1; l < 32; ++l) t += red[l][q2][e];
      p.stats[((long)rt * 2 + (e >> 2)) * p.n + c] = t;
    }
  }
}
template <typename Tag, int MAXR>
__global__ __launch_bounds__(1024) void splitk_epilogue_gn_kernel(const GemmP p, const int rl_n) {
  typedef typename Elem<Tag>::quad_t quad_t;
  constexpr int ES = Elem<Tag>::ES;
  __shared__ double wsum[16][2];
  __shared__ float s_stat[2];
  kernarg_touch<sizeof(GemmP)>();
  const int R = p.stat_rows, sg = blockIdx.x, grp = blockIdx.y, tid = threadIdx.x;
  const int cpg = p.n >> 5, nq = cpg >> 2;
  const int rl = tid / nq, qd = tid - rl * nq;
  const int gn = grp * cpg + qd * 4;
  const bool lane_ok = rl < rl_n;
  float x[MAXR][4];
  int gmr[MAXR];
  bool ok[MAXR];
  EpiOps<Tag> eo[MAXR];
  const float4 g4 = *(const float4*)(p.gn_gamma + gn), b4 = *(const float4*)(p.gn_beta + gn);
#pragma unroll
  for (int i = 0; i < MAXR; ++i) {
    const int r = rl + i * rl_n;
    ok[i] = lane_ok && r < R;
    gmr[i] = sg * R + (ok[i] ? r : R - 1);
    eo[i] = epi_load<Tag>(p, gmr[i], gn);
    const float4 a = *(const float4*)(p.ws + (long)gmr[i] * p.n + gn);
    x[i][0] = a.x; x[i][1] = a.y; x[i][2] = a.z; x[i][3] = a.w;
  }
  for (int s2 = 1; s2 < p.splitk; ++s2) {
#pragma unroll
    for (int i = 0; i < MAXR; ++i) {
      const float4 b = *(const float4*)(p.ws + ((long)s2 * p.m + gmr[i]) * p.n + gn);
      x[i][0] += b.x; x[i][1] += b.y; x[i][2] += b.z; x[i][3] += b.w;
    }
  }
  double cs = 0.0, cq = 0.0;
#pragma unroll
  for (int i = 0; i < MAXR; ++i) {
    if (ok[i]) {
      epi_finish<Tag>(p, eo[i], gmr[i], gn, x[i]);
#pragma unroll
      for (int e = 0; e < 4; ++e) { x[i][e] = round_store<Tag>(x[i][e]); cs += (double)x[i][e]; cq += (double)x[i][e] * (double)x[i][e]; }
    }
  }
#pragma unroll
  for (int o = 32; o > 0; o >>= 1) { cs += __shfl_xor(cs, o); cq += __shfl_xor(cq, o); }
  if ((tid & 63) == 0) { wsum[tid >> 6][0] = cs; wsum[tid >> 6][1] = cq; }
  __syncthreads();
  if (tid == 0) {
    double a = 0.0, b = 0.0;
    for (int w = 0; w < (((int)blockDim.x + 63) >> 6); ++w) { a += wsum[w][0]; b += wsum[w][1]; }
    const double cnt = (double)R * cpg, mean = a / cnt;
    double var = b / cnt - mean * mean;
    if (var < 0.0) var = 0.0;
    s_stat[0] = (float)mean;
    s_stat[1] = (float)(1.0 / sqrt(var + (double)p.gn_eps));
  }
  __syncthreads();
  const float mean = s_stat[0], rstd = s_stat[1];
  const float sc[4] = {rstd * g4.x, rstd * g4.y, rstd * g4.z, rstd * g4.w};
  const float sh[4] = {b4.x - mean * sc[0], b4.y - mean * sc[1], b4.z - mean * sc[2], b4.w - mean * sc[3]};
#pragma unroll
  for (int i = 0; i < MAXR; ++i) {
    if (ok[i]) {
      float y[4];
#pragma unroll
      for (int e = 0; e < 4; ++e) { const float t = fmaf(x[i][e], sc[e], sh[e]); y[e] = p.gn_silu ? silu_f(t) : t; }
      *(quad_t*)(p.gn_out + ((long)gmr[i] * p.ld_gn + gn) * ES) = f32_to_quad<Tag>(y);
    }
  }
}
static inline int splitk_gn_rows(int seg, int n, int* rl_n) {
  const int nq = n / 128;
  if (nq <= 0 || nq > 256 || seg <= 0) return 0;
  for (int mr = 1; mr <= 8; mr *= 2) {
    const int lanes = (seg + mr - 1) / mr;
    if ((long)lanes * nq <= 1024) { if (rl_n) *rl_n = lanes; return mr; }
  }
  return 0;
}
template <typename Tag>
static inline void launch_splitk_epilogue(const GemmP& p, hipStream_t st) {
  if (p.gn_out) {
    int rl_n = 0;
    const int mr = splitk_gn_rows(p.stat_rows, p.n, &rl_n);
    const dim3 grid(p.m / p.stat_rows, 32), block((rl_n * (p.n / 128) + 63) / 64 * 64);
    if (mr == 1) hipLaunchKernelGGL((splitk_epilogue_gn_kernel<Tag, 1>), grid, block, 0, st, p, rl_n);
    else if (mr == 2) hipLaunchKernelGGL((splitk_epilogue_gn_kernel<Tag, 2>), grid, block, 0, st, p, rl_n);
    else if (mr == 4) hipLaunchKernelGGL((splitk_epilogue_gn_kernel<Tag, 4>), grid, block, 0, st, p, rl_n);
    else hipLaunchKernelGGL((splitk_epilogue_gn_kernel<Tag, 8>), grid, block, 0, st, p, rl_n);
    return;
  }
  if (p.stats) {
    hipLaunchKernelGGL(splitk_epilogue_stats_kernel<Tag>, dim3(p.m / p.stat_rows, (p.n + 31) / 32), dim3(256), 0, st, p);
    return;
  }
  long blocks = ((long)p.m * (p.n >> 2) + 255) / 256;
  if (blocks > 2048) blocks = 2048;
  hipLaunchKernelGGL(splitk_epilogue_kernel<Tag>, dim3((unsigned)blocks), dim3(256), 0, st, p);
}

template <typename Tag, int BM, int BN, int BK, int NST, int WGM, int WGN, int MODE>
void launch_mode(const GemmP& p, hipStream_t st) {
  constexpr int NT_ = 64 * WGM * WGN, CPR_ = BK / Elem<Tag>::EPC;
  constexpr size_t lds = (size_t)NST * (((BM * CPR_ + NT_ - 1) / NT_) + ((BN * CPR_ + NT_ - 1) / NT_)) * NT_ * 16
                         + ((MODE & 7) == 4 ? WGM * WGN * 1024 : 0);
  static_assert(lds + (size_t)WGM * WGN * 2 * (BN / WGN) * sizeof(float) <= 160 * 1024, "LDS ring (+ the statistics staging rows) exceeds 160 KiB");
  static_assert((MODE & 7) != 4 || BN / WGN <= 256, "column-scale array: 1 KiB per wave");
  constexpr size_t stat_lds = (size_t)WGM * WGN * 2 * (BN / WGN) * sizeof(float);
  static unsigned long long attr_done = 0;
  tt_lds_opt_in((const void*)gemm_kernel<Tag, BM, BN, BK, NST, WGM, WGN, MODE>, (int)(lds + stat_lds), &attr_done);
  hipLaunchKernelGGL((gemm_kernel<Tag, BM, BN, BK, NST, WGM, WGN, MODE>), dim3(p.tiles_m * p.tiles_n * p.splitk),
                     dim3(64 * WGM * WGN), (p.stats && p.splitk == 1) ? lds + stat_lds : lds, st, p);
  if (p.splitk > 1) launch_splitk_epilogue<Tag>(p, st);
}

static inline void fill_fastdivs(GemmP& p) {
  p.fd_splitk = make_fastdiv(p.splitk);
  p.fd_per_group = make_fastdiv((long)p.group_m * p.tiles_n);
  p.fd_group_m = make_fastdiv(p.group_m);
  p.fd_last_rows = make_fastdiv(p.tiles_m % p.group_m ? p.tiles_m % p.group_m : p.group_m);
  p.fd_per_tap = make_fastdiv(p.nk0 + p.nk1);
  p.fd_hwo = make_fastdiv((long)p.hout * p.wout);
  p.fd_wout = make_fastdiv(p.wout);
  p.fd_hw = make_fastdiv(p.hw);
  p.fd_frames = make_fastdiv(p.frames);
  p.fd_rv_rows = make_fastdiv(p.rowvec ? p.rowvec_rows : 1);
  p.fd_rv_mod = make_fastdiv(p.rowvec_mod > 0 ? p.rowvec_mod : 1);
}

template <typename Tag, int BM, int BN, int BK, int NST, int WGM, int WGN, bool LNOK = false, bool M3OK = false>
void launch_cfg(GemmP& p, hipStream_t st) {
  p.tiles_m = ceil_div(p.m, BM);
  p.tiles_n = ceil_div(p.n, BN);
  {
    constexpr int NT_ = 64 * WGM * WGN, CPR_ = BK / Elem<Tag>::EPC;
    constexpr long lds_ = (long)NST * (((BM * CPR_ + NT_ - 1) / NT_) + ((BN * CPR_ + NT_ - 1) / NT_)) * NT_ * 16;
    const int window = 32 * (lds_ * 2 <= 160 * 1024 ? 2 : 1);
    int gm = p.group_m_override;
    if (gm <= 0) {
      gm = 1;
      if (p.tiles_n > 8)
        while (gm * 2 * BM * gm * 2 <= (long)window * BN && gm * 2 <= p.tiles_m) gm *= 2;
    }
    p.group_m = gm < 1 ? 1 : (gm > p.tiles_m ? p.tiles_m : gm);
  }
  p.nk0 = ceil_div(p.k0, BK); p.nk1 = p.k1 ? ceil_div(p.k1, BK) : 0;
  p.kt_total = p.taps * (p.nk0 + p.nk1);
  fill_fastdivs(p);
  if (p.mode == 3) {
    if constexpr (M3OK) {
      if constexpr (std::is_same<Tag, f32_tag>::value) {
        if (p.f32_split) {
          if (p.presplit & 2) launch_mode<Tag, BM, BN, BK, NST, WGM, WGN, 13 + 16>(p, st); else launch_mode<Tag, BM, BN, BK, NST, WGM, WGN, 13>(p, st);
          return;
        }
      }
      launch_mode<Tag, BM, BN, BK, NST, WGM, WGN, 5>(p, st);
    }
    return;
  }
  if constexpr (std::is_same<Tag, f32_tag>::value) {
    if (p.f32_split) {
      const int pre = p.presplit & 3;
      if (LNOK && p.ln_fold == 1) {
        if (pre & 2) launch_mode<Tag, BM, BN, BK, NST, WGM, WGN, 11 + 16>(p, st); else launch_mode<Tag, BM, BN, BK, NST, WGM, WGN, 11>(p, st);
        return;
      }
      if (LNOK && p.ln_fold == 2) {
        if (pre & 1) launch_mode<Tag, BM, BN, BK, NST, WGM, WGN, 12 + 32>(p, st); else launch_mode<Tag, BM, BN, BK, NST, WGM, WGN, 12>(p, st);
        return;
      }
      switch (p.mode * 4 + pre) {
        case 0: launch_mode<Tag, BM, BN, BK, NST, WGM, WGN, 8>(p, st); break;
        case 1: launch_mode<Tag, BM, BN, BK, NST, WGM, WGN, 8 + 32>(p, st); break;
        case 2: launch_mode<Tag, BM, BN, BK, NST, WGM, WGN, 8 + 16>(p, st); break;
        case 3: launch_mode<Tag, BM, BN, BK, NST, WGM, WGN, 8 + 48>(p, st); break;
        case 4: case 5: launch_mode<Tag, BM, BN, BK, NST, WGM, WGN, 9>(p, st); break;
        case 6: case 7: launch_mode<Tag, BM, BN, BK, NST, WGM, WGN, 9 + 16>(p, st); break;
        case 8: case 9: launch_mode<Tag, BM, BN, BK, NST, WGM, WGN, 10>(p, st); break;
        default: launch_mode<Tag, BM, BN, BK, NST, WGM, WGN, 10 + 16>(p, st); break;
      }
      return;
    }
  }
  if constexpr (LNOK) {
    if (p.ln_fold == 1) { launch_mode<Tag, BM, BN, BK, NST, WGM, WGN, 3>(p, st); return; }
    if (p.ln_fold == 2) { launch_mode<Tag, BM, BN, BK, NST, WGM, WGN, 4>(p, st); return; }
  }
  switch (p.mode) {
    case 0: launch_mode<Tag, BM, BN, BK, NST, WGM, WGN, 0>(p, st); break;
    case 1: launch_mode<Tag, BM, BN, BK, NST, WGM, WGN, 1>(p, st); break;
    default: launch_mode<Tag, BM, BN, BK, NST, WGM, WGN, 2>(p, st); break;
  }
}

template <typename Tag, bool HAS_RES, bool HAS_RV = false>
void launch_sq320(const GemmP& p, hipStream_t st) {
  constexpr size_t lds = (size_t)(HAS_RES ? 3 * 2 * SQ_TILE_BYTES : 5 * SQ_TILE_BYTES) + SQ_WAVES * 4096;
  static_assert(lds <= 160 * 1024, "sq320 LDS");
  static unsigned long long attr_done = 0;
  tt_lds_opt_in((const void*)sq320_kernel<Tag, HAS_RES, HAS_RV>, (int)lds, &attr_done);
  const int ntiles = (p.m + SQ_ROWS - 1) / SQ_ROWS;
  hipLaunchKernelGGL((sq320_kernel<Tag, HAS_RES, HAS_RV>), dim3(ntiles < 256 ? ntiles : 256), dim3(SQ_NT), lds, st, p);
}

#define TT_GEMM_TILES(X) \
  X( 0, 128, 128,  64, 2, 2, 2, false, false)    \
  X( 1, 128,  64,  64, 3, 2, 2, true,  true )    \
  X( 2,  64,  64,  64, 4, 2, 2, true,  true )    \
  X( 3, 256, 128,  32, 3, 4, 2, true,  false)    \
  X( 4, 256, 256,  32, 3, 2, 4, false, false)    \
  X( 5, 128, 128,  32, 3, 2, 2, false, false)    \
  X( 6, 256, 128,  64, 3, 4, 2, false, false)    \
  X( 7, 128, 160,  64, 2, 4, 1, true,  false)    \
  X( 8, 128, 320,  32, 3, 4, 2, false, false)    \
  X( 9, 256, 256,  64, 2, 2, 4, true,  false)    \
  X(10, 128, 128,  64, 4, 2, 2, false, false)    \
  X(11, 128, 128,  64, 2, 4, 2, true,  true )    \
  X(12, 256, 160,  32, 3, 8, 1, false, false)    \
  X(13, 256, 128,  32, 4, 4, 2, false, false)    \
  X(14, 128, 128,  32, 5, 4, 2, false, false)    \
  X(15, 128, 128,  64, 3, 4, 2, false, false)    \
  X(16, 128, 128,  64, 4, 4, 2, true,  true )    \
  X(17, 256, 256,  32, 4, 2, 4, false, false)    \
  X(18, 256, 128,  64, 2, 4, 2, false, false)    \
  X(19, 256, 128,  32, 5, 4, 2, false, false)    \
  X(20, 128, 128, 128, 2, 4, 2, false, false)
#define TT_GEMM_TILES_F32(X) \
  X( 0, 128, 128,  32, 2, 2, 2, true,  true ) \
  X( 1,  64,  64,  32, 4, 2, 2, true,  true )

struct TileCfg { int idx, bm, bn, bk, nst, wgm, wgn; bool ln, m3; };
#define TT_TILE_ROW(i, bm, bn, bk, nst, wgm, wgn, ln, m3) {i, bm, bn, bk, nst, wgm, wgn, ln, m3},
constexpr TileCfg kCfgs[] = {TT_GEMM_TILES(TT_TILE_ROW)};
constexpr TileCfg kCfgsF32[] = {TT_GEMM_TILES_F32(TT_TILE_ROW)};
#undef TT_TILE_ROW
constexpr int kNumCfgs = sizeof(kCfgs) / sizeof(kCfgs[0]);
template <int N> constexpr bool tiles_in_order(const TileCfg (&t)[N]) {
  for (int i = 0; i < N; ++i) if (t[i].idx != i) return false;
  return true;
}
static_assert(tiles_in_order(kCfgs) && tiles_in_order(kCfgsF32), "a tile's index is its position in the table (the planner and launch() both go by it)");

#define TT_TILE_CASE(i, bm, bn, bk, nst, wgm, wgn, ln, m3) case i: launch_cfg<Tag, bm, bn, bk, nst, wgm, wgn, ln, m3>(p, st); break;
template <typename Tag>
void launch(GemmP& p, int cfg, hipStream_t st) {
  switch (cfg) { TT_GEMM_TILES(TT_TILE_CASE) }
}
template <> void launch<f32_tag>(GemmP& p, int cfg, hipStream_t st);

}
```

this_and_that_vdm_amd/ops.py:

```python
from __future__ import annotations

import ctypes as C
import os
from typing import Optional, Tuple

import torch

from . import _lib
from ._lib import TT_BF16, TT_F16, TT_F32, TtAttnArgs, TtConvArgs, TtEncAttnArgs, TtGemmArgs, check
from .packing import PreSplitF32


PROFILE = None


def _prof_begin():
    if PROFILE is None:
        return None
    e = torch.cuda.Event(enable_timing=True)
    e.record()
    return e


def _prof_end(start, name, flops, shape=None):
    if start is not None:
        e = torch.cuda.Event(enable_timing=True)
        e.record()
        PROFILE.append((name, flops, start, e, shape))


import itertools

_SERIAL = itertools.count(1)
_LAST_WRITE = {}


def _wrote(t: torch.Tensor) -> int:
    n = next(_SERIAL)
    _LAST_WRITE[t.untyped_storage().data_ptr()] = n
    for name in ("_tt_stats", "_tt_gn"):
        if hasattr(t, name):
            delattr(t, name)
    return n


def _handoff_valid(t: torch.Tensor, serial: int, ptr: int, shape) -> bool:
    return _LAST_WRITE.get(t.untyped_storage().data_ptr()) == serial and t.data_ptr() == ptr and tuple(t.shape) == shape


_WS = {}
_WS_RETIRED = []
WS_FLOOR_BYTES = 64 << 20


def _workspace(nbytes: int, device) -> torch.Tensor:
    key = (device, torch.cuda.current_stream().cuda_stream)
    buf = _WS.get(key)
    if buf is None or buf.numel() < nbytes:
        if buf is not None:
            _WS_RETIRED.append(buf)
        buf = _WS[key] = torch.empty(max(nbytes, WS_FLOOR_BYTES), dtype=torch.uint8, device=device)
    return buf


def _code(dt: torch.dtype) -> int:
    if dt == torch.bfloat16:
        return TT_BF16
    if dt == torch.float16:
        return TT_F16
    if dt == torch.float32:
        return TT_F32
    raise RuntimeError(f"libttvdm activations/weights must be bfloat16, float16 or float32, got {dt}")


_F32_SPLIT = os.environ.get("TT_F32_SPLIT", "0") not in ("", "0")


def set_f32_split(on: bool) -> None:
    global _F32_SPLIT
    check(_lib.load().tt_gemm_set_f32_split(int(bool(on))), "tt_gemm_set_f32_split")
    _F32_SPLIT = bool(on)


def f32_split() -> bool:
    return _F32_SPLIT


_TAG = {TT_BF16: "bf16_tag", TT_F16: "f16_tag", TT_F32: "f32_tag"}
FP8 = torch.float8_e4m3fn


def _stream():
    return C.c_void_p(torch.cuda.current_stream().cuda_stream)


def _p(t: Optional[torch.Tensor]):
    if t is None:
        return None
    if not t.is_cuda:
        raise RuntimeError("libttvdm ops need tensors on the HIP device (no CPU fallback)")
    return t.data_ptr()


def _rows2d(t: torch.Tensor) -> Tuple[int, int]:
    assert t.dim() == 2 and t.stride(1) == 1, (t.shape, t.stride())
    return t.stride(0), t.shape[1]


def gemm(a0: torch.Tensor, w: torch.Tensor, *, a1: Optional[torch.Tensor] = None, mode: int = 0, conv=None, tconv=None,
         bias=None, acc_scale: float = 1.0, rowvec=None, rowvec_rows: int = 0, rowvec_mod: int = 0, geglu: bool = False, residual=None,
         blend=None, alpha: float = 0.0, out: Optional[torch.Tensor] = None, out_f32: bool = False, m: Optional[int] = None,
         out_col_pad: Optional[Tuple[int, int]] = None, ln_fold: int = 0, ln_eps: float = 1e-5,
         out_fp8: bool = False, stats: int = 0, gn=None) -> torch.Tensor:
    lib = _lib.load()
    g = TtGemmArgs()
    lda0, k0 = _rows2d(a0)
    g.a0, g.k0, g.lda0 = _p(a0), k0, lda0
    if a1 is not None:
        lda1, k1 = _rows2d(a1)
        g.a1, g.k1, g.lda1 = _p(a1), k1, lda1
    ldw, _ = _rows2d(w)
    n = w.shape[0]
    g.w, g.ldw, g.n = _p(w), ldw, n
    g.mode = mode
    if mode in (1, 3):
        g.nimg, g.hin, g.win, g.hout, g.wout, g.stride, g.upsample = conv
        mm = conv[0] * conv[3] * conv[4]
    elif mode == 2:
        g.frames, g.hw = tconv
        mm = a0.shape[0]
    else:
        mm = a0.shape[0]
    g.m = mm if m is None else m
    g.bias, g.acc_scale = _p(bias), acc_scale
    if rowvec is not None:
        g.rowvec, g.rowvec_rows, g.ld_rowvec, g.rowvec_mod = _p(rowvec), rowvec_rows, rowvec.stride(0), int(rowvec_mod)
        need_rows = rowvec_mod if rowvec_mod > 0 else (((mm if m is None else m) - 1) // rowvec_rows + 1)
        if rowvec.dtype != torch.float32 or rowvec.stride(1) != 1 or rowvec.shape[0] < need_rows or rowvec.shape[1] < n:
            raise RuntimeError(f"gemm: rowvec must be fp32 [>= {need_rows}, >= {n}] with contiguous rows, got {tuple(rowvec.shape)} {rowvec.dtype}")
    g.geglu = int(geglu)
    if residual is not None:
        g.residual, g.ld_res = _p(residual), residual.stride(0)
    if blend is not None:
        g.blend, g.ld_blend, g.alpha = _p(blend), blend.stride(0), alpha
    n_out = n // 2 if geglu else n
    if out is None:
        out = torch.empty((g.m, n_out), dtype=FP8 if out_fp8 else (torch.float32 if out_f32 else a0.dtype), device=a0.device)
    if out_fp8 and out.dtype != FP8:
        raise RuntimeError("out_fp8 needs a torch.float8_e4m3fn output tensor")
    g.out, g.ldo, g.out_f32, g.out_fp8 = _p(out), out.stride(0), int(out_f32), int(out_fp8)
    if out_col_pad is not None:
        g.out_col_hw, g.out_col_hwp = out_col_pad
    g.dtype = _code(a0.dtype)
    g.ln_fold, g.ln_eps = int(ln_fold), float(ln_eps)
    if g.dtype == TT_F32 and _F32_SPLIT:
        g.presplit = (1 if isinstance(a0, PreSplitF32) else 0) | (2 if isinstance(w, PreSplitF32) else 0)
    elif isinstance(a0, PreSplitF32) or isinstance(w, PreSplitF32):
        raise RuntimeError("gemm: a pre-split operand outside the split16 mode (set_f32_split changed after the weights were packed: "
                           "call prepare() / begin() again)")
    need = lib.tt_gemm_ws_bytes(C.byref(g))
    if need:
        ws = _workspace(need, a0.device)
        g.ws, g.ws_bytes = ws.data_ptr(), ws.numel()
    sbuf = gnbuf = None
    if stats and gn is not None and GN_FUSED:
        g.stats_seg = int(stats)
        if lib.tt_gemm_gn_fused(C.byref(g)):
            gnbuf = torch.empty((g.m, n), dtype=out.dtype, device=a0.device)
            g.gn_out, g.ld_gn, g.gn_gamma, g.gn_beta, g.gn_eps, g.gn_silu = gnbuf.data_ptr(), n, _p(gn[0]), _p(gn[1]), float(gn[2]), int(bool(gn[3]))
    if stats and gnbuf is None and GN_TILES and g.m * n <= GN_TILES_MAX_ELEMS:
        g.stats_seg = int(stats) if GN_TILES_SEG else 0
        srows = lib.tt_gemm_stats_rows(C.byref(g))
        if srows > 0 and lib.tt_groupnorm_tiles_supported(int(stats), n, srows, g.dtype):
            sbuf = torch.empty(((g.m + srows - 1) // srows, 2, n), dtype=torch.float32, device=a0.device)
            g.stats_out = sbuf.data_ptr()
    ev = _prof_begin()
    check(lib.tt_gemm(C.byref(g), _stream()), "tt_gemm")
    serial = _wrote(out)
    if sbuf is not None:
        out._tt_stats = (sbuf, srows, serial, out.data_ptr(), tuple(out.shape))
    if gnbuf is not None:
        out._tt_gn = (gnbuf, gn[0].data_ptr(), gn[1].data_ptr(), float(gn[2]), bool(gn[3]), int(stats), serial, out.data_ptr(), tuple(out.shape))
    if ev is not None:
        cfg = (C.c_int32 * 7)()
        lib.tt_gemm_plan(C.byref(g), cfg)
        taps = 9 if mode in (1, 3) else (3 if mode == 2 else 1)
        tag = _TAG[g.dtype]
        if cfg[3] == 0 and cfg[1] == 320:
            kname = f"gemm_w320{'h' if cfg[0] == 128 else ''}_kernel<{tag}, {mode}, {int(bool(ln_fold))}>"
        elif cfg[3] == 0:
            kname = f"gemm_pp_kernel<{tag}, {int(bool(ln_fold))}, {int(bool(geglu))}>"
        elif cfg[0] == 32 and cfg[1] == 320:
            kname = f"sq320_kernel<{tag}, {'true' if residual is not None else 'false'}>"
        else:
            kmode = (5 if mode == 3 else mode if not ln_fold else 2 + ln_fold) + (8 if (g.dtype == TT_F32 and _F32_SPLIT) else 0)
            if mode == 3:
                kmode += 16 if g.presplit & 2 else 0
            kname = f"gemm_kernel<{tag}, {', '.join(str(v) for v in cfg[:6])}, {kmode}>"
        _prof_end(ev, kname, 2.0 * g.m * n * taps * (g.k0 + g.k1),
                  shape=(mode, g.m, n, taps * (g.k0 + g.k1), int(geglu), int(residual is not None)))
    return out


CONV3X3_FUSED = os.environ.get("TT_CONV3X3", "0") == "1"


def conv3x3_supported(h: int, w: int, c0: int, c1: int, n: int, dtype: torch.dtype) -> bool:
    if dtype not in (torch.bfloat16, torch.float16):
        return False
    return bool(_lib.load().tt_conv3x3_supported(h, w, c0, c1, n, _code(dtype)))


def conv3x3(x0, x1, w, nimg: int, h: int, wd: int, *, gn=None, silu: bool = True, bias=None, rowvec=None, rowvec_rows: int = 0,
            residual=None, out=None):
    lib = _lib.load()
    a = TtConvArgs()
    a.x0, a.c0, a.ld0 = _p(x0), x0.shape[1], x0.stride(0)
    if x1 is not None:
        a.x1, a.c1, a.ld1 = _p(x1), x1.shape[1], x1.stride(0)
    n = w.shape[0]
    a.w, a.ldw = _p(w), w.stride(0)
    a.nimg, a.h, a.w_img, a.n = nimg, h, wd, n
    if gn is not None:
        a.gn_scale, a.gn_shift, a.silu = _p(gn[0]), _p(gn[1]), int(silu)
    a.bias = _p(bias)
    if rowvec is not None:
        a.rowvec, a.rowvec_rows, a.ld_rowvec = _p(rowvec), rowvec_rows, rowvec.stride(0)
    if residual is not None:
        a.residual, a.ld_res = _p(residual), residual.stride(0)
    if out is None:
        out = torch.empty((nimg * h * wd, n), dtype=x0.dtype, device=x0.device)
    a.out, a.ldo, a.dtype = _p(out), out.stride(0), _code(x0.dtype)
    ev = _prof_begin()
    check(lib.tt_conv3x3(C.byref(a), _stream()), "tt_conv3x3")
    _wrote(out)
    if ev is not None:
        k = 9 * (a.c0 + a.c1)
        _prof_end(ev, f"conv_patch_kernel<{_TAG[a.dtype]}>", 2.0 * nimg * h * wd * n * k, shape=(1, nimg * h * wd, n, k, 0, int(residual is not None)))
    return out


ATTN_QPROJ = os.environ.get("TT_ATTN_QPROJ", "1") != "0"


def attention_qproj_supported(x, head_dim: int, mask: int) -> bool:
    return ATTN_QPROJ and mask != 0 and head_dim == 64 and x.dtype in (torch.float16, torch.bfloat16) and x.shape[-1] % 64 == 0 and \
        x.stride(0) % 8 == 0 and x.stride(1) == 1


def attention(q, k, vt, out, *, nseq, lq, heads, head_dim, mask, lk, k_seq_stride, v_seq_stride, frames=1, ctx_batches=1,
              batch0=0, qx=None, wq=None, bq=None, ln_eps: float = 1e-5, v_rows: bool = False):
    lib = _lib.load()
    a = TtAttnArgs()
    if qx is not None:
        if wq.dtype != qx.dtype or bq.dtype != torch.float32 or not bq.is_contiguous() or wq.stride(1) != 1 or \
                tuple(wq.shape) != (heads * head_dim, qx.shape[1]) or bq.numel() != heads * head_dim:
            raise RuntimeError(f"attention: fused query projection needs wq [{heads * head_dim}, {qx.shape[1]}] in {qx.dtype} and a contiguous "
                               f"fp32 bq [{heads * head_dim}]; got wq {tuple(wq.shape)} {wq.dtype}, bq {tuple(bq.shape)} {bq.dtype}")
        a.qx, a.ldqx, a.wq, a.ldwq, a.bq, a.qc, a.ln_eps = _p(qx), qx.stride(0), _p(wq), wq.stride(0), _p(bq), qx.shape[1], float(ln_eps)
        q = qx
    else:
        a.q, a.ldq = _p(q), q.stride(0)
    a.k, a.ldk = _p(k), k.stride(0)
    a.vt, a.ldvt = _p(vt), vt.stride(0)
    a.out, a.ldo = _p(out), out.stride(0)
    a.nseq, a.lq, a.heads, a.head_dim = nseq, lq, heads, head_dim
    a.mask, a.lk, a.k_seq_stride, a.v_seq_stride = mask, lk, k_seq_stride, v_seq_stride
    fp8 = q.dtype == FP8
    if fp8 and not (k.dtype == FP8 and vt.dtype == FP8):
        raise RuntimeError("fp8 attention needs q, k and vt in torch.float8_e4m3fn")
    a.frames, a.ctx_batches, a.dtype, a.batch0, a.fp8 = frames, ctx_batches, _code(out.dtype if fp8 else q.dtype), batch0, int(fp8)
    a.v_rows = int(bool(v_rows))
    ev = _prof_begin()
    check(lib.tt_attention(C.byref(a), _stream()), "tt_attention")
    _wrote(out)
    if ev is not None:
        tag = _TAG[a.dtype]
        if fp8:
            kname = f"attn8_kernel<{tag}, {head_dim}>"
        elif v_rows and lk >= 128 and lk % 64 == 0 and os.environ.get("TT_ATTN_PIPE", "1") != "0":
            kname = f"attn_pipe_kernel<{tag}>"
        else:
            kname = f"attn_kernel<{tag}, {head_dim}, {mask}{', true' if qx is not None else ''}{', false, true' if v_rows else ''}>"
        flops = 4.0 * nseq * heads * lq * lk * head_dim + (2.0 * nseq * lq * heads * head_dim * qx.shape[1] if qx is not None else 0.0)
        _prof_end(ev, kname, flops, shape=("attn", nseq * heads, lq, lk, mask, 0))
    return out


def temporal_attention(qkv, out, *, batch, frames, hw, heads, head_dim):
    lib = _lib.load()
    check(lib.tt_temporal_attention(_p(qkv), qkv.stride(0), _p(out), out.stride(0), batch, frames, hw, heads, head_dim,
                                    _code(qkv.dtype), _stream()), "tt_temporal_attention")
    _wrote(out)
    return out


def groupnorm_stats(x0, x1, nimg, hw, frames_per_group, gamma, beta, eps):
    lib = _lib.load()
    c0 = x0.shape[-1]
    c1 = 0 if x1 is None else x1.shape[-1]
    c = c0 + c1
    ws_bytes = lib.tt_groupnorm_ws_bytes(nimg, hw, c)
    ws = torch.empty(ws_bytes // 8, dtype=torch.float64, device=x0.device)
    scale = torch.empty((nimg, c), dtype=torch.float32, device=x0.device)
    shift = torch.empty_like(scale)
    check(lib.tt_groupnorm_stats(_p(x0), c0, _p(x1), c1, nimg, hw, frames_per_group, _p(gamma), _p(beta), eps,
                                 _p(scale), _p(shift), _p(ws), ws_bytes, _code(x0.dtype), _stream()), "tt_groupnorm_stats")
    return scale, shift


def groupnorm_apply(x0, x1, nimg, hw, scale, shift, silu: bool, out=None):
    lib = _lib.load()
    c0 = x0.shape[-1]
    c1 = 0 if x1 is None else x1.shape[-1]
    if out is None:
        out = torch.empty((nimg * hw, c0 + c1), dtype=x0.dtype, device=x0.device)
    check(lib.tt_groupnorm_apply(_p(x0), c0, _p(x1), c1, nimg, hw, _p(scale), _p(shift), int(silu), _p(out), out.stride(0),
                                 _code(x0.dtype), _stream()), "tt_groupnorm_apply")
    _wrote(out)
    return out


GN_SMALL = os.environ.get("TT_GN_SMALL", "1") != "0"
GN_CROSS_MAX_ROWS = int(os.environ.get("TT_GN_CROSS_ROWS", "0"))


GN_TILES = os.environ.get("TT_GN_TILES", "1") != "0"
GN_TILES_SEG = os.environ.get("TT_GN_TILES_SEG", "1") != "0"
GN_FUSED = os.environ.get("TT_GN_FUSED", "1") != "0"
GN_TILES_MAX_ELEMS = int(os.environ.get("TT_GN_TILES_MAX_ELEMS", str(17 << 20)))
if os.environ.get("TT_GN_EMULATE", "0") == "1":
    raise RuntimeError("TT_GN_EMULATE is no longer read by the library (it produced wrong numbers by design): use tools/gn_emulate.py")


def groupnorm(x0, x1, nimg, hw, frames_per_group, gamma, beta, eps, silu: bool):
    lib = _lib.load()
    c0 = x0.shape[-1]
    c1 = 0 if x1 is None else x1.shape[-1]
    fz = getattr(x0, "_tt_gn", None) if x1 is None else None
    if fz is not None and fz[1:6] == (gamma.data_ptr(), beta.data_ptr(), float(eps), bool(silu), frames_per_group * hw) and \
            _handoff_valid(x0, *fz[6:]):
        return fz[0]
    st = getattr(x0, "_tt_stats", None) if (GN_TILES and x1 is None) else None
    if st is not None and not _handoff_valid(x0, *st[2:]):
        st = None
    if st is not None and nimg % frames_per_group == 0 and x0.is_contiguous() and st[0].shape[2] == c0 and \
            lib.tt_groupnorm_tiles_supported(frames_per_group * hw, c0, st[1], _code(x0.dtype)):
        out = torch.empty((nimg * hw, c0), dtype=x0.dtype, device=x0.device)
        check(lib.tt_groupnorm_tiles(_p(x0), c0, _p(st[0]), st[1], nimg // frames_per_group, frames_per_group * hw, _p(gamma), _p(beta), eps,
                                     int(silu), _p(out), out.stride(0), _code(x0.dtype), _stream()), "tt_groupnorm_tiles")
        return out
    if GN_SMALL and frames_per_group > 1 and nimg % frames_per_group == 0 and frames_per_group * hw <= GN_CROSS_MAX_ROWS and \
            lib.tt_groupnorm_small_supported(frames_per_group * hw, c0 + c1, _code(x0.dtype)):
        nimg, hw, frames_per_group = nimg // frames_per_group, frames_per_group * hw, 1
# ... 298 lines not shown
```

this_and_that_vdm_amd/packing.py:

```python
from __future__ import annotations

import os

import torch


def pack_conv3x3(w: torch.Tensor) -> torch.Tensor:
    o, i = w.shape[:2]
    return w.permute(0, 2, 3, 1).reshape(o, 9 * i).contiguous()


def pack_tconv3(w: torch.Tensor) -> torch.Tensor:
    o, i = w.shape[:2]
    return w[:, :, :, 0, 0].permute(0, 2, 1).reshape(o, 3 * i).contiguous()


def pack_conv1x1(w: torch.Tensor) -> torch.Tensor:
    return w.reshape(w.shape[0], w.shape[1]).contiguous()


def pack_geglu(w: torch.Tensor, b: torch.Tensor):
    n2, k = w.shape
    half = n2 // 2
    assert half % 8 == 0
    wp = w.view(2, half // 8, 8, k).permute(1, 0, 2, 3).reshape(n2, k).contiguous()
    bp = b.view(2, half // 8, 8).permute(1, 0, 2).reshape(n2).contiguous()
    return wp, bp


def pad_rows(w: torch.Tensor, multiple: int) -> torch.Tensor:
    n = w.shape[0]
    np_ = (n + multiple - 1) // multiple * multiple
    if np_ == n:
        return w
    out = torch.zeros((np_,) + tuple(w.shape[1:]), dtype=w.dtype, device=w.device)
    out[:n] = w
    return out


DEVICE_ROUNDING = os.environ.get("TT_ZSR_DEVICE", "1") != "0"


def zero_sum_round(w: torch.Tensor, dtype: torch.dtype) -> torch.Tensor:
    if dtype == torch.float32:
        return w.float().contiguous()
    mant, emin = {torch.bfloat16: (7, -126), torch.float16: (10, -14)}[dtype]
    if w.is_cuda and w.dtype == torch.float32 and w.dim() == 2 and w.shape[1] <= 16384 and DEVICE_ROUNDING:
        from . import _lib, ops
        wc = w.detach().contiguous()
        q0 = wc.to(dtype)
        nz = q0 != 0
        if not bool(nz.any()):
            return q0.contiguous()
        _, e = torch.frexp(q0.float().abs())
        e = torch.clamp(e - 1, min=emin)
        hi, lo = int(e[nz].max()), int(e[nz].min())
        out = torch.empty_like(q0)
        _lib.check(_lib.load().tt_zero_sum_round(wc.data_ptr(), wc.stride(0), wc.shape[0], wc.shape[1], hi, lo, out.data_ptr(), out.stride(0),
                                                 ops._code(dtype), ops._stream()), "tt_zero_sum_round")
        return out
    wd = w.detach().double()
    q = w.detach().to(dtype).double()
    up = q > wd
    dn = q < wd
    _, e = torch.frexp(q.abs())
    e = torch.clamp(e - 1, min=emin)
    nz = q != 0
    r = q.sum(dim=1)
    lo = int(e[nz].min()) if bool(nz.any()) else 0
    hi = int(e[nz].max()) if bool(nz.any()) else -1
    moved = torch.zeros_like(nz)
    for only_other_neighbour in (True, False):
        for lvl in range(hi, max(lo, hi - 48) - 1, -1):
            if not bool((r != 0).any()):
                break
            u = 2.0 ** (lvl - mant)
            want = torch.round(r / u).abs()
            if not bool((want != 0).any()):
                continue
            mask = nz & (e == lvl) & ~moved
            if only_other_neighbour:
                mask = mask & torch.where((r > 0)[:, None], up, dn)
            cnt = mask.sum(dim=1)
            n = torch.minimum(want, cnt.double()) * torch.sign(r)
            sel = mask & (torch.cumsum(mask, dim=1, dtype=torch.int32) <= n.abs()[:, None])
            q = q - sel.double() * (torch.sign(n) * u)[:, None]
            moved = moved | sel
            r = r - n * u
    out = q.to(dtype)
    assert torch.equal(out.double(), q), "zero_sum_round: a corrected value is not representable"
    return out.contiguous()


def fold_layernorm(weight: torch.Tensor, bias, gamma: torch.Tensor, beta: torch.Tensor):
    w = weight.detach().float()
    wg = w * gamma.detach().float()[None, :]
    wc = wg - wg.mean(dim=1, keepdim=True)
    b = w @ beta.detach().float()
    if bias is not None:
        b = b + bias.detach().float()
    return wc.contiguous(), b.contiguous()


def permute_q_rows(t: torch.Tensor) -> torch.Tensor:
    n = t.shape[0]
    if n % 16:
        raise ValueError("permute_q_rows: row count must be a multiple of 16")
    idx = torch.arange(n, device=t.device)
    d = (idx & ~12) | ((idx & 4) << 1) | ((idx & 8) >> 1)
    return t[d].contiguous()


class PreSplitF32(torch.Tensor):
    """An fp32-typed [N, K] matrix whose bytes are the pre-split fp16 pairs of TtGemmArgs.presplit (see presplit_f32).  The subclass
    is the marker ops.gemm looks for; row slices / row permutations / contiguous() keep it (and stay valid: the pairing is per row,
    in aligned groups of 4 columns).  Arithmetic on it is meaningless -- pre-split LAST, after every fold that reads the values."""


def presplit_f32(w: torch.Tensor) -> torch.Tensor:
    if isinstance(w, PreSplitF32):
        return w
    if w.dtype != torch.float32 or w.dim() != 2 or w.shape[1] % 4:
        raise ValueError(f"presplit_f32: fp32 [N, K] with K % 4 == 0 expected, got {tuple(w.shape)} {w.dtype}")
    n, k = w.shape
    xs = w.detach().contiguous() * 2.0 ** -8
    h = xs.to(torch.float16)
    l = ((xs - h.float()) * 2048.0).to(torch.float16)
    pairs = torch.stack([h.view(n, k // 4, 4), l.view(n, k // 4, 4)], 2)
    return pairs.reshape(n, 2 * k).contiguous().view(torch.float32).as_subclass(PreSplitF32)
```

this_and_that_vdm_amd/svd/autoencoder_kl_temporal_decoder.py:

```python
from __future__ import annotations

import math
from types import SimpleNamespace
from typing import Optional, Tuple

import torch
import torch.nn as nn

from .. import ops
from ..packing import pack_conv3x3, pack_tconv3
from .layers import Geom, PackRegistry, SpatioTemporalResBlock, Upsample2D, _f32, _Packable
from .modeling_utils import CONFIG_NAME, ConfigMixin, ModelMixin, register_to_config
from .vae_encoder import DiagonalGaussianDistribution, Encoder


def _res(cin: int, cout: int) -> SpatioTemporalResBlock:
    return SpatioTemporalResBlock(cin, cout, temb_channels=None, eps=1e-6, temporal_eps=1e-5, merge_factor=0.0,
                                  merge_strategy="learned", switch_spatial_to_temporal_mix=True)


class VaeAttention(_Packable):

    def __init__(self, query_dim: int, heads: int, dim_head: int, eps: float = 1e-6, norm_num_groups: int = 32):
        super().__init__()
        if heads != 1:
            raise NotImplementedError("the temporal VAE decoder uses one attention head (attention_head_dim = channels)")
        if norm_num_groups != 32:
            raise NotImplementedError("GroupNorm kernels are built for 32 groups")
        self.dim, self.eps = query_dim, eps
        self.group_norm = nn.GroupNorm(norm_num_groups, query_dim, eps=eps)
        self.to_q = nn.Linear(query_dim, query_dim, bias=True)
        self.to_k = nn.Linear(query_dim, query_dim, bias=True)
        self.to_v = nn.Linear(query_dim, query_dim, bias=True)
        self.to_out = nn.ModuleList([nn.Linear(query_dim, query_dim, bias=True), nn.Dropout(0.0)])

    def pack(self, reg, dtype):
        cv = lambda t: t.detach().to(dtype).contiguous()
        self.gamma, self.beta = _f32(self.group_norm.weight), _f32(self.group_norm.bias)
        self.wq, self.bq = cv(self.to_q.weight), _f32(self.to_q.bias)
        self.wk, self.bk = cv(self.to_k.weight), _f32(self.to_k.bias)
        self.wv = cv(self.to_v.weight)
        self.wo = cv(self.to_out[0].weight)
        self.bo = (_f32(self.to_out[0].bias) + self.wo.float() @ _f32(self.to_v.bias)).contiguous()
        self._scratch = {}

    def _scratch_for(self, like: torch.Tensor, n: int, l: int, lp: int):
        key = (like.device, like.dtype, n, l, torch.cuda.current_stream().cuda_stream)
        buf = self._scratch.get(key)
        if buf is None:
            buf = self._scratch[key] = (torch.zeros((self.dim, n * lp), dtype=like.dtype, device=like.device),
                                        torch.empty((l, lp), dtype=torch.float32, device=like.device))
        return buf

    def forward(self, x: torch.Tensor, g: Geom) -> torch.Tensor:
        c, l = self.dim, g.hw
        if l % 4:
            raise NotImplementedError(f"VAE attention over {l} tokens per frame: h*w must be a multiple of 4 (latents are multiples of 8)")
        lp = (l + 7) // 8 * 8
        xn = ops.groupnorm(x, None, g.n, l, 1, self.gamma, self.beta, self.eps, False)
        q = ops.gemm(xn, self.wq, bias=self.bq)
        k = ops.gemm(xn, self.wk, bias=self.bk)
        vt, scores = self._scratch_for(x, g.n, l, lp)
        ops.gemm(self.wv, xn, out=vt, out_col_pad=(l, lp) if lp != l else None)
        o = torch.empty((g.m, c), dtype=x.dtype, device=x.device)
        scale = 1.0 / math.sqrt(c)
        for f in range(g.n):
            rows = slice(f * l, (f + 1) * l)
            ops.gemm(q[rows], k[rows], acc_scale=scale, out=scores[:, :l], out_f32=x.dtype != torch.float32)
            p = ops.softmax_rows(scores, x.dtype, cols=l)
            ops.gemm(p, vt[:, f * lp:(f + 1) * lp], out=o[rows])
        return ops.gemm(o, self.wo, bias=self.bo, residual=x)


class MidBlockTemporalDecoder(_Packable):
    def __init__(self, in_channels: int, out_channels: int, attention_head_dim: int = 512, num_layers: int = 1):
        super().__init__()
        self.resnets = nn.ModuleList([_res(in_channels if i == 0 else out_channels, out_channels) for i in range(num_layers)])
        self.attentions = nn.ModuleList([VaeAttention(in_channels, in_channels // attention_head_dim, attention_head_dim)])

    def pack(self, reg, dtype):
        for m in list(self.resnets) + list(self.attentions):
            m.pack(reg, dtype)

    def forward(self, x, g: Geom):
        x = self.resnets[0](x, None, g, None)
        for resnet, attn in zip(list(self.resnets)[1:], self.attentions):
            x = attn(x, g)
            x = resnet(x, None, g, None)
        return x


class UpBlockTemporalDecoder(_Packable):
    def __init__(self, in_channels: int, out_channels: int, num_layers: int = 1, add_upsample: bool = True):
        super().__init__()
        self.resnets = nn.ModuleList([_res(in_channels if i == 0 else out_channels, out_channels) for i in range(num_layers)])
        self.upsamplers = nn.ModuleList([Upsample2D(out_channels, use_conv=True, out_channels=out_channels)]) if add_upsample else None

    def pack(self, reg, dtype):
        for m in self.resnets:
            m.pack(reg, dtype)
        if self.upsamplers is not None:
            self.upsamplers[0].pack(reg, dtype)

    def forward(self, x, g: Geom):
        for resnet in self.resnets:
            x = resnet(x, None, g, None)
        if self.upsamplers is not None:
            x, g = self.upsamplers[0](x, g)
        return x, g


class TemporalDecoder(_Packable):
    CIN_PAD = 8

    def __init__(self, in_channels: int = 4, out_channels: int = 3, block_out_channels: Tuple[int, ...] = (128, 256, 512, 512),
                 layers_per_block: int = 2):
        super().__init__()
        if in_channels > self.CIN_PAD or out_channels > 4:
            raise NotImplementedError("latent channels <= 8 and image channels <= 4")
        self.in_channels, self.out_channels = in_channels, out_channels
        self.conv_in = nn.Conv2d(in_channels, block_out_channels[-1], 3, padding=1)
        self.mid_block = MidBlockTemporalDecoder(num_layers=layers_per_block, in_channels=block_out_channels[-1],
                                                 out_channels=block_out_channels[-1], attention_head_dim=block_out_channels[-1])
        self.up_blocks = nn.ModuleList([])
        rev = list(reversed(block_out_channels))
        out_ch = rev[0]
        for i in range(len(block_out_channels)):
            prev, out_ch = out_ch, rev[i]
            self.up_blocks.append(UpBlockTemporalDecoder(num_layers=layers_per_block + 1, in_channels=prev, out_channels=out_ch,
                                                         add_upsample=i != len(block_out_channels) - 1))
        self.conv_norm_out = nn.GroupNorm(32, block_out_channels[0], eps=1e-6)
        self.conv_act = nn.SiLU()
        self.conv_out = nn.Conv2d(block_out_channels[0], out_channels, 3, padding=1)
        self.time_conv_out = nn.Conv3d(out_channels, out_channels, (3, 1, 1), padding=(1, 0, 0))

    def pack(self, reg, dtype):
        w = self.conv_in.weight.detach()
        wp = torch.zeros((w.shape[0], self.CIN_PAD, 3, 3), dtype=w.dtype, device=w.device)
        wp[:, :self.in_channels] = w
        self.w_in, self.b_in = pack_conv3x3(wp.to(dtype)), _f32(self.conv_in.bias)
        self.mid_block.pack(reg, dtype)
        for b in self.up_blocks:
            b.pack(reg, dtype)
        self.g_out, self.be_out = _f32(self.conv_norm_out.weight), _f32(self.conv_norm_out.bias)
        w = self.conv_out.weight.detach()
        wo = torch.zeros((self.CIN_PAD,) + tuple(w.shape[1:]), dtype=w.dtype, device=w.device)
        wo[:self.out_channels] = w
        bo = torch.zeros(self.CIN_PAD, dtype=torch.float32, device=w.device)
        bo[:self.out_channels] = self.conv_out.bias.detach().float()
        self.w_out, self.b_out = pack_conv3x3(wo.to(dtype)), bo
        w = self.time_conv_out.weight.detach()
        wt = torch.zeros((4, self.CIN_PAD, 3, 1, 1), dtype=w.dtype, device=w.device)
        wt[:self.out_channels, :self.out_channels] = w
        bt = torch.zeros(4, dtype=torch.float32, device=w.device)
        bt[:self.out_channels] = self.time_conv_out.bias.detach().float()
        self.w_t, self.b_t = pack_tconv3(wt.to(dtype)), bt

    def forward(self, z: torch.Tensor, num_frames: int, dtype: torch.dtype) -> torch.Tensor:
        n, _, h, w = z.shape
        if n % num_frames:
            raise ValueError(f"{n} latent frames are not a multiple of num_frames = {num_frames}")
        g = Geom(n // num_frames, num_frames, h, w)
        x = ops.nchw_to_tokens(z, dtype, ld=self.CIN_PAD)
        x = ops.gemm(x, self.w_in, mode=1, conv=(n, h, w, h, w, 1, 0), bias=self.b_in)
        x = self.mid_block(x, g)
        for blk in self.up_blocks:
            x, g = blk(x, g)
        x = ops.groupnorm(x, None, g.n, g.hw, 1, self.g_out, self.be_out, 1e-6, True)
        x = ops.gemm(x, self.w_out, mode=1, conv=(n, g.h, g.w, g.h, g.w, 1, 0), bias=self.b_out)
        x = ops.gemm(x, self.w_t, mode=2, tconv=(g.frames, g.hw), bias=self.b_t)
        return ops.tokens_to_nchw(x, n, self.out_channels, g.h, g.w, torch.float32)


class AutoencoderKLTemporalDecoder(ModelMixin, ConfigMixin):

    _config_exclude = ("encoder",)

    @register_to_config
    def __init__(self, in_channels: int = 3, out_channels: int = 3, block_out_channels: Tuple[int, ...] = (128, 256, 512, 512),
                 layers_per_block: int = 2, latent_channels: int = 4, sample_size: int = 768, scaling_factor: float = 0.18215,
                 force_upcast: bool = True, encoder=None, native_encoder: bool = False):
        super().__init__()
        if native_encoder and encoder is not None:
            raise ValueError("native_encoder=True runs encode() on the model's own encoder: do not pass a stock encoder= as well")
        self.decoder = TemporalDecoder(latent_channels, out_channels, tuple(block_out_channels), layers_per_block)
        self.native_encoder = bool(native_encoder)
        if self.native_encoder:
            self.encoder = Encoder(in_channels, latent_channels, tuple(block_out_channels), layers_per_block)
            self.quant_conv = nn.Conv2d(2 * latent_channels, 2 * latent_channels, 1)
        self.compute_dtype: Optional[torch.dtype] = None
        self._packed_key = None
        self.__dict__["_stock_encoder"] = None
        self.with_encoder(encoder)

    def with_encoder(self, encoder):
        if encoder is not None and self.native_encoder:
            raise ValueError("this model runs its own encoder (native_encoder=True): a stock encoder cannot be attached")
        if encoder is not None and not callable(getattr(encoder, "encode", None)):
            raise TypeError("encoder must provide encode(x) returning an object with .latent_dist (diffusers' AutoencoderKLTemporalDecoder)")
        self.__dict__["_stock_encoder"] = encoder
        return self

    @classmethod
    def from_pretrained(cls, pretrained_model_name_or_path, *args, encoder=None, **kwargs):
        import json
        import os
        path = pretrained_model_name_or_path
        sub = kwargs.get("subfolder", args[0] if args else None)
        cfg_file = os.path.join(os.path.join(path, sub) if sub else path, CONFIG_NAME)
        if os.path.isfile(cfg_file):
            with open(cfg_file) as f:
                cfg = json.load(f)
            native = kwargs.get("native_encoder", cfg.get("native_encoder", False))
            kinds = cfg.get("down_block_types")
            if native and kinds is not None and any(k != "DownEncoderBlock2D" for k in kinds):
                raise ValueError(f"native_encoder: {cfg_file} names down_block_types {kinds}; only DownEncoderBlock2D is implemented")
        model = super().from_pretrained(pretrained_model_name_or_path, *args, **kwargs)
        return model.with_encoder(encoder)

    def _run_dtype(self) -> torch.dtype:
        if self.compute_dtype is not None:
            return self.compute_dtype
        dt = next(self.parameters()).dtype
        return dt if dt in (torch.float16, torch.bfloat16) else torch.bfloat16

    def prepare(self, force: bool = False):
        p0 = next(self.parameters())
        key = (p0.device, self._run_dtype(), sum(p._version for p in self.parameters()), p0.data_ptr())
        if force or self._packed_key != key:
            if p0.device.type != "cuda":
                raise RuntimeError("AutoencoderKLTemporalDecoder: the decoder runs on the MI355X only (no CPU fallback)")
            self.decoder.pack(PackRegistry(), key[1])
            if self.native_encoder:
                self.encoder.pack(PackRegistry(), key[1], self.quant_conv)
            self._packed_key = key
        return self

    def load_state_dict(self, state_dict, strict: bool = True, **kw):
        if self.native_encoder:
            self._packed_key = None
            return super().load_state_dict(state_dict, strict=strict, **kw)
        sd = {k: v for k, v in state_dict.items() if k.startswith("decoder.")}
        self._packed_key = None
        return super().load_state_dict(sd, strict=strict, **kw)

    def _apply(self, fn, *a, **k):
        self._packed_key = None
        stock = self.__dict__.get("_stock_encoder")
        if isinstance(stock, nn.Module):
# ... 52 lines not shown
```

this_and_that_vdm_amd/svd/denoiser_base.py:

```python
from __future__ import annotations

import os

from typing import List, Optional, Tuple

import torch
import torch.nn as nn

from .. import ops
from .layers import Geom, PackRegistry, StepContext, _f32
from .modeling_utils import ModelMixin
from ..packing import pack_conv3x3


def as_tokens(t: torch.Tensor, dtype: torch.dtype) -> torch.Tensor:
    n, c, h, w = t.shape
    if t.dtype == dtype and t.permute(0, 2, 3, 1).is_contiguous():
        return t.permute(0, 2, 3, 1).reshape(n * h * w, c)
    return ops.nchw_to_tokens(t, dtype)


def as_nchw_view(tok: torch.Tensor, g: Geom) -> torch.Tensor:
    return tok.view(g.n, g.h, g.w, tok.shape[1]).permute(0, 3, 1, 2)


_PRESPLIT_ATTRS = {
    "ResnetBlock2D": ("w1", "w2", "ws"), "TemporalResnetBlock": ("w1", "w2"), "Downsample2D": ("w",), "Upsample2D": ("w",),
    "FeedForward": ("wg", "w2"), "BasicTransformerBlock": ("wqkv", "wo1", "wo2"), "TemporalBasicTransformerBlock": ("wqkv", "wo1", "wo2"),
    "TransformerSpatioTemporalModel": ("w_in", "w_out"),
}


def presplit_packed_weights(root: nn.Module) -> None:
    from ..packing import presplit_f32
    for m in root.modules():
        d = m.__dict__
        for name in _PRESPLIT_ATTRS.get(type(m).__name__, ()):
            t = d.get(name)
            if torch.is_tensor(t) and t.dtype == torch.float32 and t.dim() == 2:
                d[name] = presplit_f32(t)
        if type(m).__name__ == "BasicTransformerBlock" and "wqk" in d:
            c2 = d["wqk"].shape[0]
            d["wqk"], d["wv"] = d["wqkv"][:c2], d["wqkv"][c2:]
        q2 = d.get("q2")
        if q2 is not None and not q2.is_fused and q2.w.dtype == torch.float32:
            q2.w, q2._other = presplit_f32(q2.w), None
    for name in ("_w_in", "_w_out", "_k_w", "_v_w"):
        t = root.__dict__.get(name)
        if torch.is_tensor(t) and t.dtype == torch.float32 and t.dim() == 2:
            root.__dict__[name] = presplit_f32(t)
    for name in ("_zero", "_zero_mid"):
        z = root.__dict__.get(name)
        if isinstance(z, list):
            root.__dict__[name] = [(presplit_f32(w), b) if torch.is_tensor(w) and w.dtype == torch.float32 and w.dim() == 2 else (w, b) for w, b in z]
        elif isinstance(z, tuple) and torch.is_tensor(z[0]) and z[0].dtype == torch.float32 and z[0].dim() == 2:
            root.__dict__[name] = (presplit_f32(z[0]),) + tuple(z[1:])


class DenoiserBase(ModelMixin):
    compute_dtype: Optional[torch.dtype] = None
    attention_fp8: bool = False
    zero_context_shortcut: bool = os.environ.get("TT_ZERO_CTX", "1") != "0"

    _pack_gen = 0

    def _pack_key(self):
        pl = self.__dict__.get("_plist")
        if pl is None:
            pl = self.__dict__["_plist"] = list(self.parameters())
        p0 = pl[0]
        return (p0.device, self._run_dtype(), sum(p._version for p in pl), p0.data_ptr(), ops.f32_split())

    def invalidate_packs(self):
        self._packed_key = None
        self.__dict__.pop("_plist", None)

    def _run_dtype(self) -> torch.dtype:
        if self.compute_dtype is not None:
            return self.compute_dtype
        dt = self.dtype
        return dt if dt in (torch.float16, torch.bfloat16) else torch.bfloat16

    def prepare(self, force: bool = False):
        key = self._pack_key()
        if not force and getattr(self, "_packed_key", None) == key:
            return self
        if next(self.parameters()).device.type != "cuda":
            raise RuntimeError(f"{type(self).__name__}: the denoise path runs on the MI355X only; move the model to the "
                               "HIP device first (there is no CPU fallback)")
        dtype = key[1]
        self.__dict__.pop("_plist", None)
        reg = PackRegistry()
        self._pack_modules(reg, dtype)
        self._film_w = torch.cat(reg.film_w, 0).to(dtype).contiguous()
        self._film_b = torch.cat(reg.film_b, 0).float().contiguous()
        self._k_w = torch.cat(reg.k_w, 0).to(dtype).contiguous()
        self._v_w = torch.cat(reg.v_w, 0).to(dtype).contiguous()
        if dtype == torch.float32 and ops.f32_split():
            presplit_packed_weights(self)
        self._packed_key = self._pack_key()
        self._pack_gen = self._pack_gen + 1
        return self

    def _pack_modules(self, reg: PackRegistry, dtype):
        raise NotImplementedError

    def _embed(self, timestep, added_time_ids, batch: int, device) -> torch.Tensor:
        if not torch.is_tensor(timestep):
            t = torch.full((batch,), float(timestep), dtype=torch.float32, device=device)
        else:
            t = timestep.to(device=device, dtype=torch.float32).reshape(-1).expand(batch).contiguous()
        emb = self.time_embedding(self.time_proj(t))
        ids = added_time_ids.to(device=device, dtype=torch.float32).reshape(-1).contiguous()
        te = self.add_time_proj(ids).reshape(batch, -1)
        ae = self.add_embedding
        hid = ops.small_linear(te, ae.w1, ae.b1, act_out=True)
        return ops.small_linear(hid, ae.w2, ae.b2, out=emb, accumulate=True)

    def film_table(self, timesteps: torch.Tensor, added_time_ids: torch.Tensor, batch: int) -> torch.Tensor:
        self.prepare()
        dev = self._film_w.device
        t = timesteps.to(device=dev, dtype=torch.float32).reshape(-1)
        ids = added_time_ids.to(device=dev, dtype=torch.float32).reshape(batch, -1)
        steps = t.numel()
        out = torch.empty((steps, batch, self._film_w.shape[0]), dtype=torch.float32, device=dev)
        per = max(1, 32 // batch)
        for s0 in range(0, steps, per):
            s1 = min(steps, s0 + per)
            rows = (s1 - s0) * batch
            emb = self.time_embedding(self.time_proj(t[s0:s1].repeat_interleave(batch).contiguous()))
            te = self.add_time_proj(ids.repeat(s1 - s0, 1).reshape(-1).contiguous()).reshape(rows, -1)
            ae = self.add_embedding
            hid = ops.small_linear(te, ae.w1, ae.b1, act_out=True)
            ops.small_linear(hid, ae.w2, ae.b2, out=emb, accumulate=True)
            ops.small_linear(emb, self._film_w, self._film_b, act_in=True, out=out[s0:s1].view(rows, -1))
        return out

    def project_context(self, encoder_hidden_states: torch.Tensor):
        self.prepare()
        dtype = self._run_dtype()
        b, s, d = encoder_hidden_states.shape
        sp = (s + 7) // 8 * 8
        pad = torch.zeros((b, sp, d), dtype=dtype, device=encoder_hidden_states.device)
        pad[:, :s] = encoder_hidden_states.to(dtype)
        pad = pad.view(b * sp, d)
        k_all = ops.gemm(pad, self._k_w)
        vt_all = ops.gemm(self._v_w, pad)
        zero_mask = 0
        if self.zero_context_shortcut and not torch.cuda.is_current_stream_capturing():
            flags = (pad.view(b, -1) == 0).all(1).tolist()
            zero_mask = sum(1 << i for i, z in enumerate(flags) if z)
        return (k_all, vt_all, s, sp, zero_mask)

    def _step_context(self, emb: Optional[torch.Tensor], context, film: Optional[torch.Tensor] = None, request_ctx=None) -> StepContext:
        if film is None:
            film = ops.small_linear(emb, self._film_w, self._film_b, act_in=True)
        k_all, vt_all, s, sp, zero_mask = context
        sc = StepContext(film, k_all, vt_all, s, sp, attn_fp8=bool(self.attention_fp8), zero_mask=zero_mask)
        if request_ctx is not None:
            sc.k_req, sc.vt_req = request_ctx
        return sc

    def _encode(self, x, g: Geom, ctx: StepContext):
        skips: List[Tuple[torch.Tensor, Geom]] = [(x, g)]
        for blk in self.down_blocks:
            x, g, outs = blk(x, g, ctx)
            skips.extend(outs)
        return x, g, skips

    _INFERENCE_ONLY = ("{}: inference-only build -- attention runs on the library's HIP kernels (tt_attention), there are no "
                       "AttentionProcessor objects to read or replace")

    @property
    def attn_processors(self):
        raise NotImplementedError(self._INFERENCE_ONLY.format(f"{type(self).__name__}.attn_processors"))

    def set_attn_processor(self, processor):
        raise NotImplementedError(self._INFERENCE_ONLY.format(f"{type(self).__name__}.set_attn_processor"))

    def set_default_attn_processor(self):
# ... 23 lines not shown
```

this_and_that_vdm_amd/svd/layers.py:

```python
from __future__ import annotations

import math
import os
from dataclasses import dataclass
from typing import Dict, List, Optional, Tuple

import torch
import torch.nn as nn

from .. import ops
from ..packing import fold_layernorm, pack_conv1x1, pack_conv3x3, pack_geglu, pack_tconv3, permute_q_rows, zero_sum_round


ZERO_CTX_TEMPORAL = os.environ.get("TT_ZERO_CTX_T", "1") != "0"
ATTN_V_ROWS = os.environ.get("TT_ATTN_V_ROWS", "1") != "0"
MERGE_FRAMES = os.environ.get("TT_XATTN_MERGE_FRAMES", "1") != "0"


@dataclass
class Geom:
    batch: int
    frames: int
    h: int
    w: int
    batch0: int = 0
    batch_total: int = 0
    requests: int = 1

    @property
    def n(self):
        return self.batch * self.frames

    @property
    def hw(self):
        return self.h * self.w

    @property
    def m(self):
        return self.n * self.hw

    @property
    def ctx_batches(self):
        return self.batch_total or self.batch

    @property
    def cfg(self):
        return self.ctx_batches // self.requests

    def film(self, film: torch.Tensor, off: int, c: int) -> torch.Tensor:
        return film[self.batch0:self.batch0 + self.batch, off:off + c]


class StepContext:

    def __init__(self, film: torch.Tensor, k_all: torch.Tensor, vt_all: torch.Tensor, s_ctx: int, s_pad: int,
                 attn_fp8: bool = False, zero_mask: int = 0):
        self.film, self.k_all, self.vt_all, self.s_ctx, self.s_pad = film, k_all, vt_all, s_ctx, s_pad
        self.attn_fp8 = attn_fp8
        self.zero_mask = zero_mask
        self.k_req = self.vt_req = None

    def live_batches(self, g: "Geom"):
        flags = [(self.zero_mask >> (g.batch0 + i)) & 1 for i in range(g.batch)]
        if not any(flags):
            return None
        live = [i for i, z in enumerate(flags) if not z]
        if not live:
            return (0, 0)
        if live[-1] - live[0] + 1 != len(live):
            return None
        return (live[0], len(live))

    def live_classes(self, g: "Geom"):
        cb, nr = g.cfg, g.requests
        if not self.zero_mask or cb < 2 or g.hw % cb or not ZERO_CTX_TEMPORAL:
            return None
        live = [c for c in range(cb) if not all((self.zero_mask >> (c * nr + r)) & 1 for r in range(nr))]
        return None if len(live) == cb else live

    _VT_CACHE: Dict[tuple, torch.Tensor] = {}

    def vt_buffer(self, c: int, cols: int, like: torch.Tensor, dtype: Optional[torch.dtype] = None) -> torch.Tensor:
        dtype = like.dtype if dtype is None else dtype
        key = (like.device, dtype, c, cols, torch.cuda.current_stream().cuda_stream)
        buf = StepContext._VT_CACHE.get(key)
        if buf is None:
            buf = StepContext._VT_CACHE[key] = torch.zeros((c, cols), dtype=torch.uint8 if dtype == ops.FP8 else dtype,
                                                           device=like.device).view(dtype)
        return buf


class _Side:
    ENABLED = os.environ.get("TT_SIDE_STREAM", "0") == "1"
    _streams: Dict[int, "torch.cuda.Stream"] = {}
    _spare: List["torch.cuda.Stream"] = []
    origin: Optional[int] = None
    _events: List["torch.cuda.Event"] = []

    @staticmethod
    def _event():
        ev = torch.cuda.Event()
        _Side._events.append(ev)
        if len(_Side._events) > 8192 and not torch.cuda.is_current_stream_capturing():
            del _Side._events[:4096]
        return ev

    def __init__(self):
        self.main = torch.cuda.current_stream()
        self.side = None
        capturing = torch.cuda.is_current_stream_capturing()
        if _Side.ENABLED and (not capturing or self.main.cuda_stream == _Side.origin):
            key = self.main.cuda_stream
            self.side = _Side._streams.get(key)
            if self.side is None:
                if capturing:
                    if not _Side._spare:
                        return
                    self.side = _Side._spare.pop()
                else:
                    self.side = torch.cuda.Stream()
                    while len(_Side._spare) < 4:
                        _Side._spare.append(torch.cuda.Stream())
                _Side._streams[key] = self.side
            ev = _Side._event()
            ev.record(self.main)
            self.side.wait_event(ev)

    def __enter__(self):
        if self.side is not None:
            self._guard = torch.cuda.stream(self.side)
            self._guard.__enter__()
        return self

    def __exit__(self, *exc):
        if self.side is not None:
            self._guard.__exit__(*exc)
        return False

    def join(self):
        if self.side is not None:
            ev = _Side._event()
            ev.record(self.side)
            self.main.wait_event(ev)


class PackRegistry:

    def __init__(self):
        self.film_w: List[torch.Tensor] = []
        self.film_b: List[torch.Tensor] = []
        self.film_cols = 0
        self.k_w: List[torch.Tensor] = []
        self.v_w: List[torch.Tensor] = []
        self.kv_cols = 0

    def add_film(self, lin: nn.Linear) -> Tuple[int, int]:
        off = self.film_cols
        self.film_w.append(lin.weight.detach())
        self.film_b.append(lin.bias.detach())
        self.film_cols += lin.out_features
        return off, lin.out_features

    def add_kv(self, to_k: nn.Linear, to_v: nn.Linear) -> Tuple[int, int]:
        off = self.kv_cols
# ... 34 lines not shown

    def pack(self, reg, dtype):
        self.w1, self.b1 = self.linear_1.weight.detach().to(dtype).contiguous(), _f32(self.linear_1.bias)
        self.w2, self.b2 = self.linear_2.weight.detach().to(dtype).contiguous(), _f32(self.linear_2.bias)

    def forward(self, sample: torch.Tensor) -> torch.Tensor:
        hid = ops.small_linear(sample, self.w1, self.b1, act_out=True)
        return ops.small_linear(hid, self.w2, self.b2)


def _gn(x0, x1, g: Geom, frames_per_group, gamma, beta, eps, silu):
    return ops.groupnorm(x0, x1, g.n, g.hw, frames_per_group, gamma, beta, eps, silu)


class ResnetBlock2D(_Packable):

    def __init__(self, *, in_channels: int, out_channels: Optional[int] = None, temb_channels: int = 512,
                 groups: int = 32, eps: float = 1e-6):
        super().__init__()
        out_channels = in_channels if out_channels is None else out_channels
        if groups != 32:
            raise NotImplementedError("GroupNorm kernels are built for 32 groups")
        self.in_channels, self.out_channels, self.eps = in_channels, out_channels, eps
        self.norm1 = nn.GroupNorm(groups, in_channels, eps=eps)
        self.conv1 = nn.Conv2d(in_channels, out_channels, 3, padding=1)
        self.time_emb_proj = nn.Linear(temb_channels, out_channels) if temb_channels is not None else None
        self.norm2 = nn.GroupNorm(groups, out_channels, eps=eps)
        self.conv2 = nn.Conv2d(out_channels, out_channels, 3, padding=1)
        self.conv_shortcut = nn.Conv2d(in_channels, out_channels, 1) if in_channels != out_channels else None

    def pack(self, reg, dtype):
        self.g1, self.be1 = _f32(self.norm1.weight), _f32(self.norm1.bias)
        self.g2, self.be2 = _f32(self.norm2.weight), _f32(self.norm2.bias)
        self.w1, self.b1 = pack_conv3x3(self.conv1.weight.detach().to(dtype)), _f32(self.conv1.bias)
        self.w2, self.b2 = pack_conv3x3(self.conv2.weight.detach().to(dtype)), _f32(self.conv2.bias)
        if self.conv_shortcut is not None:
            self.ws, self.bs = pack_conv1x1(self.conv_shortcut.weight.detach().to(dtype)), _f32(self.conv_shortcut.bias)
        self.film = reg.add_film(self.time_emb_proj) if self.time_emb_proj is not None else None

    def forward(self, x0, x1, g: Geom, ctx: StepContext, next_gn=None):
        film = None
        if self.film is not None:
            off, c = self.film
            film = g.film(ctx.film, off, c)
        c0, c1 = x0.shape[1], (x1.shape[1] if x1 is not None else 0)
        fused = ops.CONV3X3_FUSED and ops.conv3x3_supported(g.h, g.w, c0, c1, self.out_channels, x0.dtype) and \
            ops.conv3x3_supported(g.h, g.w, self.out_channels, 0, self.out_channels, x0.dtype)
        conv = (g.n, g.h, g.w, g.h, g.w, 1, 0)
        if fused:
            st1 = ops.groupnorm_stats(x0, x1, g.n, g.hw, 1, self.g1, self.be1, self.eps)
            hmid = ops.conv3x3(x0, x1, self.w1, g.n, g.h, g.w, gn=st1, silu=True, bias=self.b1, rowvec=film,
                               rowvec_rows=g.frames * g.hw if film is not None else 0)
        else:
            a = ops.groupnorm(x0, x1, g.n, g.hw, 1, self.g1, self.be1, self.eps, True)
            hmid = ops.gemm(a, self.w1, mode=1, conv=conv, bias=self.b1, rowvec=film, rowvec_rows=g.frames * g.hw if film is not None else 0,
                            stats=g.hw, gn=(self.g2, self.be2, self.eps, True))
        if self.conv_shortcut is not None:
            xs = ops.gemm(x0, self.ws, a1=x1, bias=self.bs)
        else:
            if x1 is not None:
                raise RuntimeError("identity shortcut with a concatenated input")
            xs = x0
        if fused:
            st2 = ops.groupnorm_stats(hmid, None, g.n, g.hw, 1, self.g2, self.be2, self.eps)
            return ops.conv3x3(hmid, None, self.w2, g.n, g.h, g.w, gn=st2, silu=True, bias=self.b2, residual=xs)
        a = ops.groupnorm(hmid, None, g.n, g.hw, 1, self.g2, self.be2, self.eps, True)
        return ops.gemm(a, self.w2, mode=1, conv=conv, bias=self.b2, residual=xs, stats=g.frames * g.hw, gn=next_gn)


class TemporalResnetBlock(_Packable):

    def __init__(self, in_channels: int, out_channels: Optional[int] = None, temb_channels: int = 512, eps: float = 1e-6):
        super().__init__()
        out_channels = in_channels if out_channels is None else out_channels
        if in_channels != out_channels:
            raise NotImplementedError("SVD only uses channel-preserving temporal blocks")
        self.eps = eps
        self.norm1 = nn.GroupNorm(32, in_channels, eps=eps)
        self.conv1 = nn.Conv3d(in_channels, out_channels, (3, 1, 1), padding=(1, 0, 0))
        self.time_emb_proj = nn.Linear(temb_channels, out_channels) if temb_channels is not None else None
        self.norm2 = nn.GroupNorm(32, out_channels, eps=eps)
        self.conv2 = nn.Conv3d(out_channels, out_channels, (3, 1, 1), padding=(1, 0, 0))

    def pack(self, reg, dtype):
        self.g1, self.be1 = _f32(self.norm1.weight), _f32(self.norm1.bias)
        self.g2, self.be2 = _f32(self.norm2.weight), _f32(self.norm2.bias)
        self.w1, self.b1 = pack_tconv3(self.conv1.weight.detach().to(dtype)), _f32(self.conv1.bias)
        self.w2, self.b2 = pack_tconv3(self.conv2.weight.detach().to(dtype)), _f32(self.conv2.bias)
        self.film = reg.add_film(self.time_emb_proj) if self.time_emb_proj is not None else None

    def forward(self, s, g: Geom, ctx: StepContext, alpha: float):
        film = g.film(ctx.film, *self.film) if self.film is not None else None
        a = _gn(s, None, g, g.frames, self.g1, self.be1, self.eps, True)
        t = ops.gemm(a, self.w1, mode=2, tconv=(g.frames, g.hw), bias=self.b1, rowvec=film,
                     rowvec_rows=g.frames * g.hw if film is not None else 0, stats=g.frames * g.hw, gn=(self.g2, self.be2, self.eps, True))
        a = _gn(t, None, g, g.frames, self.g2, self.be2, self.eps, True)
        return ops.gemm(a, self.w2, mode=2, tconv=(g.frames, g.hw), bias=self.b2, residual=s, blend=s, alpha=alpha, stats=g.hw)


class AlphaBlender(nn.Module):

    def __init__(self, alpha: float, merge_strategy: str = "learned_with_images", switch_spatial_to_temporal_mix: bool = False):
        super().__init__()
        if merge_strategy not in ("learned_with_images", "learned"):
            raise NotImplementedError(merge_strategy)
        self.switch = bool(switch_spatial_to_temporal_mix)
        self.mix_factor = nn.Parameter(torch.tensor([float(alpha)]))

    def alpha_value(self) -> float:
        a = float(torch.sigmoid(self.mix_factor.detach().float()).item())
        return 1.0 - a if self.switch else a


class SpatioTemporalResBlock(_Packable):
    def __init__(self, in_channels: int, out_channels: Optional[int] = None, temb_channels: int = 512, eps: float = 1e-6,
                 temporal_eps: Optional[float] = None, merge_factor: float = 0.5, merge_strategy="learned_with_images",
                 switch_spatial_to_temporal_mix: bool = False):
        super().__init__()
        oc = out_channels if out_channels is not None else in_channels
        self.spatial_res_block = ResnetBlock2D(in_channels=in_channels, out_channels=oc, temb_channels=temb_channels, eps=eps)
        self.temporal_res_block = TemporalResnetBlock(oc, oc, temb_channels=temb_channels,
                                                      eps=temporal_eps if temporal_eps is not None else eps)
        self.time_mixer = AlphaBlender(merge_factor, merge_strategy, switch_spatial_to_temporal_mix)

    def pack(self, reg, dtype):
        self.spatial_res_block.pack(reg, dtype)
        self.temporal_res_block.pack(reg, dtype)
        self.alpha = self.time_mixer.alpha_value()

    def forward(self, x0, x1, g: Geom, ctx: StepContext):
        t = self.temporal_res_block
        s = self.spatial_res_block(x0, x1, g, ctx, next_gn=(t.g1, t.be1, t.eps, True))
        return t(s, g, ctx, self.alpha)


class Downsample2D(_Packable):
    def __init__(self, channels: int, use_conv: bool = False, out_channels: Optional[int] = None, padding: int = 1, name: str = "conv"):
        super().__init__()
        if not use_conv or padding != 1:
            raise NotImplementedError("SVD uses Downsample2D(use_conv=True, padding=1)")
        self.conv = nn.Conv2d(channels, out_channels or channels, 3, stride=2, padding=1)

    def pack(self, reg, dtype):
        self.w, self.b = pack_conv3x3(self.conv.weight.detach().to(dtype)), _f32(self.conv.bias)

    def forward(self, x, g: Geom):
        ho, wo = (g.h + 2 - 3) // 2 + 1, (g.w + 2 - 3) // 2 + 1
        out = ops.gemm(x, self.w, mode=1, conv=(g.n, g.h, g.w, ho, wo, 2, 0), bias=self.b, stats=ho * wo)
        return out, Geom(g.batch, g.frames, ho, wo, g.batch0, g.batch_total, g.requests)


class Upsample2D(_Packable):
    def __init__(self, channels: int, use_conv: bool = False, use_conv_transpose: bool = False,
                 out_channels: Optional[int] = None, name: str = "conv"):
        super().__init__()
        if not use_conv or use_conv_transpose:
            raise NotImplementedError("SVD uses Upsample2D(use_conv=True)")
        self.conv = nn.Conv2d(channels, out_channels or channels, 3, padding=1)

    def pack(self, reg, dtype):
        self.w, self.b = pack_conv3x3(self.conv.weight.detach().to(dtype)), _f32(self.conv.bias)

    def forward(self, x, g: Geom):
        out = ops.gemm(x, self.w, mode=1, conv=(g.n, g.h, g.w, 2 * g.h, 2 * g.w, 1, 1), bias=self.b, stats=4 * g.hw)
        return out, Geom(g.batch, g.frames, 2 * g.h, 2 * g.w, g.batch0, g.batch_total, g.requests)


class Attention(nn.Module):

    def __init__(self, query_dim: int, cross_attention_dim: Optional[int] = None, heads: int = 8, dim_head: int = 64,
                 dropout: float = 0.0, bias: bool = False, out_bias: bool = True):
        super().__init__()
        self.inner_dim, self.heads, self.dim_head = heads * dim_head, heads, dim_head
        self.is_cross = cross_attention_dim is not None
        cross = cross_attention_dim if self.is_cross else query_dim
        self.to_q = nn.Linear(query_dim, self.inner_dim, bias=bias)
        self.to_k = nn.Linear(cross, self.inner_dim, bias=bias)
        self.to_v = nn.Linear(cross, self.inner_dim, bias=bias)
        self.to_out = nn.ModuleList([nn.Linear(self.inner_dim, query_dim, bias=out_bias), nn.Dropout(dropout)])
        if dim_head not in (64, 128):
            raise NotImplementedError(f"attention head_dim {dim_head}: kernels are built for 64 and 128")


class GEGLU(nn.Module):
    def __init__(self, dim_in: int, dim_out: int):
        super().__init__()
        self.proj = nn.Linear(dim_in, dim_out * 2)


class FeedForward(_Packable):
    def __init__(self, dim: int, dim_out: Optional[int] = None, mult: int = 4, dropout: float = 0.0, activation_fn: str = "geglu"):
        super().__init__()
        if activation_fn != "geglu":
            raise NotImplementedError(activation_fn)
        inner = int(dim * mult)
        self.net = nn.ModuleList([GEGLU(dim, inner), nn.Dropout(dropout), nn.Linear(inner, dim_out if dim_out is not None else dim)])

    def pack(self, reg, dtype, norm: Optional[nn.LayerNorm] = None):
        w, b = self.net[0].proj.weight.detach(), self.net[0].proj.bias
        self.ln_fold, self.ln_eps = 0, 1e-5
        if norm is not None:
            w, b = fold_layernorm(w, b, norm.weight, norm.bias)
            w = zero_sum_round(w, dtype)
            self.ln_fold, self.ln_eps = 1, norm.eps
        self.wg, self.bg = pack_geglu(w.to(dtype), _f32(b))
        self.w2, self.b2 = self.net[2].weight.detach().to(dtype).contiguous(), _f32(self.net[2].bias)

    def forward(self, x, residual, blend=None, alpha=0.0, rowvec=None, rowvec_rows: int = 0):
        hid = ops.gemm(x, self.wg, bias=self.bg, geglu=True, ln_fold=self.ln_fold, ln_eps=self.ln_eps)
        return ops.gemm(hid, self.w2, bias=self.b2, residual=residual, blend=blend, alpha=alpha, rowvec=rowvec, rowvec_rows=rowvec_rows)


def _self_attention(x, attn: Attention, wqk, bqk, wv, eps, g: Geom, ctx: StepContext, wqkv=None, bqkv=None):
    c = attn.inner_dim
    fp8 = ctx.attn_fp8 and x.dtype != torch.float32
    if wqkv is not None and not fp8 and ATTN_V_ROWS and attn.dim_head == 64 and x.dtype in (torch.float16, torch.bfloat16):
        qkv = ops.gemm(x, wqkv, bias=bqkv, ln_fold=1, ln_eps=eps)
        out = torch.empty((g.m, c), dtype=x.dtype, device=x.device)
        return ops.attention(qkv[:, :c], qkv[:, c:2 * c], qkv[:, 2 * c:], out, nseq=g.n, lq=g.hw, heads=attn.heads, head_dim=attn.dim_head,
                             mask=0, lk=g.hw, k_seq_stride=g.hw, v_seq_stride=g.hw, v_rows=True)
    pad = 16 if fp8 else 8
    hwp = (g.hw + pad - 1) // pad * pad
    vt = ctx.vt_buffer(c, g.n * hwp, x, ops.FP8 if fp8 else None)
    side = _Side()
    with side:
        ops.gemm(wv, x, out=vt, out_col_pad=(g.hw, hwp) if hwp != g.hw else None, ln_fold=2, ln_eps=eps, out_fp8=fp8)
    qk = ops.gemm(x, wqk, bias=bqk, ln_fold=1, ln_eps=eps, out_fp8=fp8)
    side.join()
    x_norm = x
    out = torch.empty((g.m, c), dtype=x_norm.dtype, device=x_norm.device)
    return ops.attention(qk[:, :c], qk[:, c:], vt, out, nseq=g.n, lq=g.hw, heads=attn.heads, head_dim=attn.dim_head,
                         mask=0, lk=g.hw, k_seq_stride=g.hw, v_seq_stride=hwp)


class _QProj:

    def __init__(self, w: torch.Tensor, b: torch.Tensor, dim_head: int):
        self.is_fused = ops.ATTN_QPROJ and dim_head == 64 and w.dtype in (torch.float16, torch.bfloat16)
        self.w, self.b = (permute_q_rows(w), permute_q_rows(b.contiguous())) if self.is_fused else (w, b.contiguous())
        self._other = None

    def fused(self):
        return (self.w, self.b) if self.is_fused else None

    def plain(self):
        if not self.is_fused:
            return self.w, self.b
        if self._other is None:
            self._other = (permute_q_rows(self.w), permute_q_rows(self.b))
        return self._other


def _cross_attention(x, attn: Attention, qp: _QProj, eps, kv, g: Geom, ctx: StepContext, temporal: bool):
    off, c = kv
    mask = 2 if temporal else 1
    out = torch.empty((g.m, c), dtype=x.dtype, device=x.device)
    kw = dict(nseq=g.n, lq=g.hw, heads=attn.heads, head_dim=attn.dim_head, mask=mask, lk=ctx.s_ctx, k_seq_stride=ctx.s_pad,
              v_seq_stride=ctx.s_pad, frames=g.frames, ctx_batches=g.ctx_batches, batch0=g.batch0)
    if not temporal and MERGE_FRAMES and g.n % g.frames == 0:
        kw.update(nseq=g.n // g.frames, lq=g.frames * g.hw, frames=1)
    fused = qp.fused()
    if fused is not None and ops.attention_qproj_supported(x, attn.dim_head, mask):
        return ops.attention(None, ctx.k_all[:, off:off + c], ctx.vt_all[off:off + c], out, qx=x, wq=fused[0], bq=fused[1], ln_eps=eps, **kw)
    wq, bq = qp.plain()
    q = ops.gemm(x, wq, bias=bq, ln_fold=1, ln_eps=eps)
    return ops.attention(q, ctx.k_all[:, off:off + c], ctx.vt_all[off:off + c], out, **kw)


def _temporal_cross_requests(x, attn: Attention, qp: _QProj, eps, kv, g: Geom, ctx: StepContext):
    off, c = kv
    nr, cb, rows, csp = g.requests, g.cfg, g.frames * g.hw, g.cfg * ctx.s_pad
    out = torch.empty((g.m, c), dtype=x.dtype, device=x.device)
    kw = dict(nseq=g.frames, lq=g.hw, heads=attn.heads, head_dim=attn.dim_head, mask=2, lk=ctx.s_ctx, k_seq_stride=ctx.s_pad,
              v_seq_stride=ctx.s_pad, frames=g.frames, ctx_batches=cb)
    fused = qp.fused()
    if fused is None or not ops.attention_qproj_supported(x, attn.dim_head, 2):
        fused = None
        wq, bq = qp.plain()
        q = ops.gemm(x, wq, bias=bq, ln_fold=1, ln_eps=eps)
    for b in range(g.batch):
        cls, r = divmod(b, nr)
        k, vt = ctx.k_req[r * csp:(r + 1) * csp, off:off + c], ctx.vt_req[off:off + c, r * csp:(r + 1) * csp]
        sl = slice(b * rows, (b + 1) * rows)
        if fused is not None:
            ops.attention(None, k, vt, out[sl], qx=x[sl], wq=fused[0], bq=fused[1], ln_eps=eps, batch0=cls, **kw)
        else:
            ops.attention(q[sl], k, vt, out[sl], batch0=cls, **kw)
    return out


class BasicTransformerBlock(_Packable):

    def __init__(self, dim: int, num_attention_heads: int, attention_head_dim: int, cross_attention_dim: Optional[int] = None):
        super().__init__()
        self.norm1 = nn.LayerNorm(dim, eps=1e-5)
        self.attn1 = Attention(dim, heads=num_attention_heads, dim_head=attention_head_dim)
        self.norm2 = nn.LayerNorm(dim, eps=1e-5)
        self.attn2 = Attention(dim, cross_attention_dim=cross_attention_dim, heads=num_attention_heads, dim_head=attention_head_dim)
        self.norm3 = nn.LayerNorm(dim, eps=1e-5)
        self.ff = FeedForward(dim)

    def pack(self, reg, dtype):
        cv = lambda t: t.detach().to(dtype).contiguous()
        zr = lambda t: zero_sum_round(t, dtype)
        n1, n2 = self.norm1, self.norm2
        wq, bq = fold_layernorm(self.attn1.to_q.weight, None, n1.weight, n1.bias)
        wk, bk = fold_layernorm(self.attn1.to_k.weight, None, n1.weight, n1.bias)
        wv, bv = fold_layernorm(self.attn1.to_v.weight, None, n1.weight, n1.bias)
        self.wqkv = zr(torch.cat([wq, wk, wv], 0))
        self.bqkv = torch.cat([bq, bk, torch.zeros_like(bq)], 0).contiguous()
        c2 = 2 * wq.shape[0]
        self.wqk, self.bqk, self.wv = self.wqkv[:c2], self.bqkv[:c2], self.wqkv[c2:]
        self.wo1 = cv(self.attn1.to_out[0].weight)
        self.bo1 = (_f32(self.attn1.to_out[0].bias) + self.wo1.float() @ bv).contiguous()
        wq2, bq2 = fold_layernorm(self.attn2.to_q.weight, None, n2.weight, n2.bias)
        self.q2 = _QProj(zr(wq2), bq2, self.attn2.dim_head)
        self.wo2, self.bo2 = cv(self.attn2.to_out[0].weight), _f32(self.attn2.to_out[0].bias)
# ... 129 lines not shown
```

Baseline: 35.15 denoise-steps/s.

## Compute nearest-upsample 3x3 conv as four 2x2 phase convolutions

After: 35.49 denoise-steps/s, median of 6. About the same (+1.0%).

```diff
diff --git a/this_and_that_vdm_amd/csrc/gemm.hip b/this_and_that_vdm_amd/csrc/gemm.hip
--- a/this_and_that_vdm_amd/csrc/gemm.hip
+++ b/this_and_that_vdm_amd/csrc/gemm.hip
@@ -18,6 +18,13 @@
 
 namespace {
 inline int gemm_taps(int mode) { return mode == 1 || mode == 3 ? 9 : (mode == 2 ? 3 : 1); }
+inline bool is_phase(const TtGemmArgs* a) { return a->mode == 1 && a->upsample >= 2; }
+inline int phase_count(const TtGemmArgs* a) { return a->upsample == 6 ? 4 : 1; }
+inline int args_taps(const TtGemmArgs* a) { return is_phase(a) ? 4 : gemm_taps(a->mode); }
+inline bool phase_refused(const TtGemmArgs* a) {
+  return a->stride != 1 || a->k1 || a->a1 || a->residual || a->blend || a->rowvec || a->geglu || a->out_f32 || a->out_fp8 || a->out_col_hw ||
+         a->ln_fold || a->stats_out || a->gn_out || a->hout != 2 * a->hin || a->wout != 2 * a->win;
+}
 
 int env_int(const char* name, int dflt) { const char* e = getenv(name); return e ? atoi(e) : dflt; }
 int big_tile_bits(int on) { return on == 0 ? 0 : (on == 2 ? 1 : (on == 3 ? 11 : (on == 4 ? 7 : 15))); }
@@ -172,8 +179,16 @@
   const long b128 = (long)ceil_div(a->m, 128) * ceil_div(a->n, 128), b12864 = (long)ceil_div(a->m, 128) * ceil_div(a->n, 64);
   return Plan{b128 >= 384 ? 11 : (b12864 >= 384 ? 1 : 2), 1};
 }
-bool mode3_served(const TtGemmArgs* a, const Plan& pl) { return a->mode != 3 || tile_of(a->dtype, pl.cfg).m3; }
+bool mode3_served(const TtGemmArgs* a, const Plan& pl) { return (a->mode != 3 && !is_phase(a)) || tile_of(a->dtype, pl.cfg).m3; }
+Plan phase_plan(const TtGemmArgs* a) {
+  const int ph = phase_count(a);
+  if (a->dtype == TT_F32) return Plan{plan_f32(a->m * ph, a->n, knobs().f32_split ? knobs().f32_split_min_tiles : 256), 1};
+  if (knobs().forced_cfg >= 0) return Plan{knobs().forced_cfg, 1};
+  const long b128 = (long)ceil_div(a->m, 128) * ceil_div(a->n, 128) * ph, b12864 = (long)ceil_div(a->m, 128) * ceil_div(a->n, 64) * ph;
+  return Plan{b128 >= 192 ? 11 : (b12864 >= 384 ? 1 : 2), 1};
+}
 Plan plan_for(const TtGemmArgs* a) {
+  if (is_phase(a)) return phase_plan(a);
   if (a->dtype == TT_F32) {
     const int split_min = knobs().f32_split_min_tiles;
     if (knobs().f32_split) {
@@ -198,6 +213,7 @@
   return mode3_plan(a, pl);
 }
 Plan unsplit_plan(const TtGemmArgs* a) {
+  if (is_phase(a)) return phase_plan(a);
   if (a->dtype == TT_F32) return Plan{plan_f32(a->m, a->n, 256), 1};
   return mode3_plan(a, Plan{make_plan(knobs().forced_cfg, a->m, a->n, 0, false, !(a->residual || a->blend || a->rowvec)).cfg, 1});
 }
@@ -234,7 +250,7 @@
 }
 
 int32_t stats_rows_on(const TtGemmArgs* a, const Route& r) {
-  if (a->geglu || a->out_fp8 || a->out_f32 || a->out_col_hw > 0 || a->ln_fold == 2) return 0;
+  if (a->geglu || a->out_fp8 || a->out_f32 || a->out_col_hw > 0 || a->ln_fold == 2 || is_phase(a)) return 0;
   if (r.kind == Kind::PP || r.kind == Kind::PP_TWO_PART || r.kind == Kind::SQ320 || r.kind == Kind::UNSUPPORTED) return 0;
   const int seg = a->stats_seg;
   if (r.splitk != 1) {
@@ -257,7 +273,7 @@
   return a->m % rows == 0 ? rows : 0;
 }
 int32_t gn_fused_on(const TtGemmArgs* a, const Route& r) {
-  if (a->dtype == TT_F32 || a->geglu || a->out_fp8 || a->out_f32 || a->out_col_hw > 0 || a->stats_out) return 0;
+  if (a->dtype == TT_F32 || a->geglu || a->out_fp8 || a->out_f32 || a->out_col_hw > 0 || a->stats_out || is_phase(a)) return 0;
   const int seg = a->stats_seg;
   if (seg <= 0 || a->m % seg || (a->n & 127)) return 0;
   if (r.kind != Kind::W320H_SPLIT && r.kind != Kind::TILED) return 0;
@@ -282,9 +298,10 @@
 
 extern "C" int tt_gemm_plan(const TtGemmArgs* a, int32_t cfg[7]) {
   if (!a || !cfg || a->m <= 0 || a->n <= 0) TT_FAIL(TT_EINVAL, "tt_gemm_plan: bad arguments");
+  if (is_phase(a) && (a->upsample > 6 || phase_refused(a))) TT_FAIL(TT_EUNSUPPORTED, "tt_gemm_plan: the phase form of the upsample conv does not serve this problem");
   const Route r = resolve(a);
   if (r.kind == Kind::UNSUPPORTED)
-    TT_FAIL(TT_EUNSUPPORTED, "tt_gemm_plan: forced tile configuration %d has no mode-3 variant (mode 3 is built for 1, 2, 11, 16)", r.cfg);
+    TT_FAIL(TT_EUNSUPPORTED, "tt_gemm_plan: forced tile configuration %d has no mode-3 / phase-conv variant (built for 1, 2, 11, 16)", r.cfg);
   const TileCfg t = route_tile(a, r);
   cfg[0] = t.bm; cfg[1] = t.bn; cfg[2] = t.bk; cfg[3] = t.nst; cfg[4] = t.wgm; cfg[5] = t.wgn; cfg[6] = r.splitk;
   return TT_OK;
@@ -348,15 +365,17 @@
     if ((a->presplit & 1) && a->mode != 0) TT_FAIL(TT_EINVAL, "tt_gemm: a pre-split A operand is a Linear operand (mode 0)");
   }
   p.gn_out = (char*)a->gn_out; p.ld_gn = a->ld_gn; p.gn_gamma = a->gn_gamma; p.gn_beta = a->gn_beta; p.gn_eps = a->gn_eps; p.gn_silu = a->gn_silu;
+  const bool phase = is_phase(a);
+  if (phase) { p.hout = p.hin; p.wout = p.win; }
   if (p.mode == 1 || p.mode == 3) {
     if (p.nimg <= 0 || p.hin <= 0 || p.win <= 0 || p.hout <= 0 || p.wout <= 0 || p.stride < 1)
       TT_FAIL(TT_EINVAL, "tt_gemm: conv geometry");
-    if ((long)p.nimg * p.hout * p.wout != p.m) TT_FAIL(TT_EINVAL, "tt_gemm: m != nimg*hout*wout");
+    if ((long)p.nimg * p.hout * p.wout != p.m) TT_FAIL(TT_EINVAL, phase ? "tt_gemm: m != nimg*hin*win (the phase form counts source rows)" : "tt_gemm: m != nimg*hout*wout");
   }
   if (p.mode == 2) {
     if (p.frames <= 0 || p.hw <= 0 || p.m % ((long)p.frames * p.hw)) TT_FAIL(TT_EINVAL, "tt_gemm: tconv geometry");
   }
-  p.taps = gemm_taps(p.mode);
+  p.taps = args_taps(a);
   {
     const long rows = p.mode == 1 || p.mode == 3 ? (long)p.nimg * p.hin * p.win : (long)p.m;
     const long a0b = ((rows - 1) * p.lda0 + p.k0) * es, a1b = p.k1 ? ((rows - 1) * p.lda1 + p.k1) * es : 16;
@@ -365,7 +384,8 @@
       TT_FAIL(TT_EUNSUPPORTED, "tt_gemm: operand larger than 2 GiB (32-bit buffer offsets)");
     p.a0_bytes = (unsigned)a0b; p.a1_bytes = (unsigned)a1b; p.w_bytes = (unsigned)wb;
     const long n_out = p.geglu ? p.n / 2 : p.n;
-    const long outb = ((long)(p.m - 1) * p.ldo + (p.out_col_hw > 0 ? p.ldo : n_out)) * (p.out_f32 ? 4 : (p.out_fp8 ? 1 : es));
+    const long out_rows = phase ? 4L * p.m : (long)p.m;
+    const long outb = ((out_rows - 1) * p.ldo + (p.out_col_hw > 0 ? p.ldo : n_out)) * (p.out_f32 ? 4 : (p.out_fp8 ? 1 : es));
     const long resb = p.residual ? ((long)(p.m - 1) * p.ld_res + p.n) * es : 0;
     const long blb = p.blend ? ((long)(p.m - 1) * p.ld_blend + p.n) * es : 0;
     long rv_last = p.rowvec ? (p.m - 1) / p.rowvec_rows : 0;
@@ -393,6 +413,9 @@
   if (a->k1 && !a->a1) TT_FAIL(TT_EINVAL, "tt_gemm: k1 > 0 without a1");
   if (a->mode < 0 || a->mode > 3) TT_FAIL(TT_EINVAL, "tt_gemm: bad mode %d", a->mode);
   if (a->mode == 3 && a->upsample) TT_FAIL(TT_EINVAL, "tt_gemm: mode 3 (bottom / right zero padding) has no fused upsample");
+  if (a->mode == 1 && (a->upsample < 0 || a->upsample > 6)) TT_FAIL(TT_EINVAL, "tt_gemm: upsample %d (0 none, 1 index map, 2..5 one phase, 6 all four phases)", a->upsample);
+  if (is_phase(a) && phase_refused(a))
+    TT_FAIL(TT_EUNSUPPORTED, "tt_gemm: the phase form of the upsample conv takes one source, stride 1, hout / wout = 2 hin / 2 win and a bias / scale epilogue only");
   const Route r = resolve(a);
   if (r.kind == Kind::PP_TWO_PART) {
     TtGemmArgs head, tail;
@@ -415,7 +438,7 @@
       else launch_f32(p, r.cfg, st);
       break;
     default:
-      TT_FAIL(TT_EUNSUPPORTED, "tt_gemm: forced tile configuration %d has no mode-3 variant (mode 3 is built for 1, 2, 11, 16)", r.cfg);
+      TT_FAIL(TT_EUNSUPPORTED, "tt_gemm: forced tile configuration %d has no mode-3 / phase-conv variant (built for 1, 2, 11, 16)", r.cfg);
   }
   TT_CHECK_LAUNCH("tt_gemm");
   return TT_OK;
diff --git a/this_and_that_vdm_amd/csrc/gemm_kernel.h b/this_and_that_vdm_amd/csrc/gemm_kernel.h
--- a/this_and_that_vdm_amd/csrc/gemm_kernel.h
+++ b/this_and_that_vdm_amd/csrc/gemm_kernel.h
@@ -50,6 +50,7 @@
   int f32_split;
   int presplit;
   FastDiv fd_splitk, fd_per_group, fd_group_m, fd_last_rows, fd_per_tap, fd_hwo, fd_wout, fd_hw, fd_frames, fd_rv_rows, fd_rv_mod;
+  FastDiv fd_phase;
 };
 
 __device__ __forceinline__ unsigned pack4_fp8(const float* v) {
@@ -226,7 +227,8 @@
   static_assert(SPLIT || (!PRE_A && !PRE_B), "pre-split operands belong to the split variants");
   static_assert(!SPLIT || std::is_same<Tag, f32_tag>::value, "split products are a TT_F32 mode");
   constexpr bool PAD_BR = KMODE == 5;
-  constexpr int MODE = PAD_BR ? 1 : (KMODE >= 3 ? 0 : KMODE);
+  constexpr bool PHASE = KMODE == 6;
+  constexpr int MODE = (PAD_BR || PHASE) ? 1 : (KMODE >= 3 ? 0 : KMODE);
   constexpr int LN = KMODE == 3 || KMODE == 4 ? KMODE - 2 : 0;
   TL(0);
   kernarg_touch<sizeof(GemmP)>();
@@ -251,6 +253,11 @@
   }
   int split = 0;
   if (p.splitk > 1) { const int t = fdiv(bid, p.fd_splitk); split = bid - t * p.splitk; bid = t; }
+  int phase = 0, wphase = 0;
+  if constexpr (PHASE) {
+    if (p.upsample == 6) { wphase = fdiv(bid, p.fd_phase); bid -= wphase * (p.tiles_m * p.tiles_n); phase = wphase; }
+    else phase = p.upsample - 2;
+  }
   int tile_m, tile_n;
   {
     const int gm = p.group_m;
@@ -270,7 +277,7 @@
   constexpr int INV = (int)0x80000000;
   const __amdgpu_buffer_rsrc_t ra0 = __builtin_amdgcn_make_buffer_rsrc((void*)p.a0, 0, p.a0_bytes, 0x00020000);
   const __amdgpu_buffer_rsrc_t ra1 = __builtin_amdgcn_make_buffer_rsrc((void*)(p.a1 ? p.a1 : p.a0), 0, p.a1_bytes, 0x00020000);
-  const __amdgpu_buffer_rsrc_t rw = __builtin_amdgcn_make_buffer_rsrc((void*)p.w, 0, p.w_bytes, 0x00020000);
+  const __amdgpu_buffer_rsrc_t rw = __builtin_amdgcn_make_buffer_rsrc((void*)(p.w + (PHASE ? (long)wphase * p.n * p.ldw * ES : 0)), 0, p.w_bytes, 0x00020000);
   const int crow = tid / CPR, cchunk = tid % CPR;
   int a_chunk[AR];
   int va0[AR], va1[AR];
@@ -328,7 +335,11 @@
         for (int i = 0; i < AR; ++i) {
           bool ok = a_valid[i];
           long row;
-          if constexpr (MODE == 1) {
+          if constexpr (PHASE) {
+            const int iy = a_y[i] + (s_tap >> 1) + (phase >> 1) - 1, ix = a_x[i] + (s_tap & 1) + (phase & 1) - 1;
+            ok = ok && iy >= 0 && iy < p.hin && ix >= 0 && ix < p.win;
+            row = ((long)a_img[i] * p.hin + iy) * p.win + ix;
+          } else if constexpr (MODE == 1) {
             constexpr int OFF = PAD_BR ? 0 : 1;
             const int dy = s_tap / 3 - OFF, dx = s_tap - (dy + OFF) * 3 - OFF;
             int iy = a_y[i] * p.stride + dy, ix = a_x[i] * p.stride + dx;
@@ -759,6 +770,15 @@
         const bool parity = FILM && p.rowvec_mod == 2 && rv_rows == 1;
         auto wrap = [&](int g) { return p.rowvec_mod > 0 ? g - fdiv(g, p.fd_rv_mod) * p.rowvec_mod : g; };
         float* sstage = (float*)(smem + STAT_OFF) + wid * (2 * WTN);
+        auto out_row = [&](int gm) {
+          if constexpr (PHASE) {
+            const int img = fdiv(gm, p.fd_hwo), rem = gm - img * (p.hin * p.win);
+            const int y = fdiv(rem, p.fd_wout), x = rem - y * p.win;
+            return ((img * 2 * p.hin + 2 * y + (phase >> 1)) * 2 * p.win) + 2 * x + (phase & 1);
+          } else {
+            return gm;
+          }
+        };
 #pragma unroll
         for (int i = 0; i < FM; ++i) {
           const int mb = m0 + wr * WTM + i * 32;
@@ -819,6 +839,7 @@
                   const float4 t = *(const float4*)(ebuf + strip_off(r, qq, q_per_row));
                   const int gm = mb + r;
                   const bool ok = gm < p.m && gn < p.n;
+                  const int om = out_row(gm);
                   if (p.splitk > 1) {
                     st128f(r_out, ok ? (int)((((long)split * p.m + gm) * p.n + gn) * 4) : kInv, t);
                   } else {
@@ -839,11 +860,11 @@
                     quad_to_f32<Tag>(bq, b4v);
 #pragma unroll
                     for (int e = 0; e < 4; ++e) v[e] = alpha * b4v[e] + one_m_alpha * (v[e] + r4[e]);
-                    if constexpr (OUT8) st32(r_out, ok ? (int)((long)gm * p.ldo + gn) : kInv, pack4_fp8(v));
+                    if constexpr (OUT8) st32(r_out, ok ? (int)((long)om * p.ldo + gn) : kInv, pack4_fp8(v));
                     else {
                       const quad_t packed = f32_to_quad<Tag>(v);
-                      if constexpr (ES == 2) st64(r_out, ok ? (int)(((long)gm * p.ldo + gn) * ES) : kInv, packed.x, packed.y);
-                      else stq<Tag>(r_out, ok ? (int)(((long)gm * p.ldo + gn) * ES) : kInv, v);
+                      if constexpr (ES == 2) st64(r_out, ok ? (int)(((long)om * p.ldo + gn) * ES) : kInv, packed.x, packed.y);
+                      else stq<Tag>(r_out, ok ? (int)(((long)om * p.ldo + gn) * ES) : kInv, v);
                       if constexpr (STATS) {
                         float sv[4];
                         quad_to_f32<Tag>(packed, sv);
@@ -1295,7 +1316,8 @@
   constexpr size_t stat_lds = (size_t)WGM * WGN * 2 * (BN / WGN) * sizeof(float);
   static unsigned long long attr_done = 0;
   tt_lds_opt_in((const void*)gemm_kernel<Tag, BM, BN, BK, NST, WGM, WGN, MODE>, (int)(lds + stat_lds), &attr_done);
-  hipLaunchKernelGGL((gemm_kernel<Tag, BM, BN, BK, NST, WGM, WGN, MODE>), dim3(p.tiles_m * p.tiles_n * p.splitk),
+  const int phases = ((MODE & 7) == 6 && p.upsample == 6) ? 4 : 1;
+  hipLaunchKernelGGL((gemm_kernel<Tag, BM, BN, BK, NST, WGM, WGN, MODE>), dim3(p.tiles_m * p.tiles_n * p.splitk * phases),
                      dim3(64 * WGM * WGN), (p.stats && p.splitk == 1) ? lds + stat_lds : lds, st, p);
   if (p.splitk > 1) launch_splitk_epilogue<Tag>(p, st);
 }
@@ -1312,6 +1334,7 @@
   p.fd_frames = make_fastdiv(p.frames);
   p.fd_rv_rows = make_fastdiv(p.rowvec ? p.rowvec_rows : 1);
   p.fd_rv_mod = make_fastdiv(p.rowvec_mod > 0 ? p.rowvec_mod : 1);
+  p.fd_phase = make_fastdiv((long)p.tiles_m * p.tiles_n);
 }
 
 template <typename Tag, int BM, int BN, int BK, int NST, int WGM, int WGN, bool LNOK = false, bool M3OK = false>
@@ -1342,6 +1365,18 @@
         }
       }
       launch_mode<Tag, BM, BN, BK, NST, WGM, WGN, 5>(p, st);
+    }
+    return;
+  }
+  if (p.mode == 1 && p.upsample >= 2) {
+    if constexpr (M3OK) {
+      if constexpr (std::is_same<Tag, f32_tag>::value) {
+        if (p.f32_split) {
+          if (p.presplit & 2) launch_mode<Tag, BM, BN, BK, NST, WGM, WGN, 14 + 16>(p, st); else launch_mode<Tag, BM, BN, BK, NST, WGM, WGN, 14>(p, st);
+          return;
+        }
+      }
+      launch_mode<Tag, BM, BN, BK, NST, WGM, WGN, 6>(p, st);
     }
     return;
   }
diff --git a/this_and_that_vdm_amd/ops.py b/this_and_that_vdm_amd/ops.py
--- a/this_and_that_vdm_amd/ops.py
+++ b/this_and_that_vdm_amd/ops.py
@@ -107,6 +107,10 @@
     return t.stride(0), t.shape[1]
 
 
+class PhaseConvRefused(RuntimeError):
+    """gemm(..., conv=(.., upsample >= 2)): tt_gemm does not serve this problem in the phase form (upsample_conv3x3 then runs upsample = 1)"""
+
+
 def gemm(a0: torch.Tensor, w: torch.Tensor, *, a1: Optional[torch.Tensor] = None, mode: int = 0, conv=None, tconv=None,
          bias=None, acc_scale: float = 1.0, rowvec=None, rowvec_rows: int = 0, rowvec_mod: int = 0, geglu: bool = False, residual=None,
          blend=None, alpha: float = 0.0, out: Optional[torch.Tensor] = None, out_f32: bool = False, m: Optional[int] = None,
@@ -119,13 +123,26 @@
     if a1 is not None:
         lda1, k1 = _rows2d(a1)
         g.a1, g.k1, g.lda1 = _p(a1), k1, lda1
-    ldw, _ = _rows2d(w)
-    n = w.shape[0]
+    phase = mode == 1 and conv[6] >= 2
+    if w.dim() == 3:
+        if not (phase and conv[6] == 6 and w.shape[0] == 4 and w.stride(2) == 1 and w.stride(0) == w.shape[1] * w.stride(1)):
+            raise RuntimeError(f"gemm: a 3-D weight is the [4, O, 4*I] phase block of upsample = 6, got {tuple(w.shape)} {w.stride()}")
+        ldw, n = w.stride(1), w.shape[1]
+    else:
+        ldw, _ = _rows2d(w)
+        n = w.shape[0]
+        if phase and conv[6] == 6:
+            if n % 4:
+                raise RuntimeError(f"gemm: upsample = 6 needs the four phases' rows, got {n}")
+            n //= 4
     g.w, g.ldw, g.n = _p(w), ldw, n
     g.mode = mode
+    out_rows = None
     if mode in (1, 3):
         g.nimg, g.hin, g.win, g.hout, g.wout, g.stride, g.upsample = conv
         mm = conv[0] * conv[3] * conv[4]
+        if phase:
+            out_rows, mm = mm, conv[0] * conv[1] * conv[2]
     elif mode == 2:
         g.frames, g.hw = tconv
         mm = a0.shape[0]
@@ -145,7 +162,7 @@
         g.blend, g.ld_blend, g.alpha = _p(blend), blend.stride(0), alpha
     n_out = n // 2 if geglu else n
     if out is None:
-        out = torch.empty((g.m, n_out), dtype=FP8 if out_fp8 else (torch.float32 if out_f32 else a0.dtype), device=a0.device)
+        out = torch.empty((g.m if out_rows is None else out_rows, n_out), dtype=FP8 if out_fp8 else (torch.float32 if out_f32 else a0.dtype), device=a0.device)
     if out_fp8 and out.dtype != FP8:
         raise RuntimeError("out_fp8 needs a torch.float8_e4m3fn output tensor")
     g.out, g.ldo, g.out_f32, g.out_fp8 = _p(out), out.stride(0), int(out_f32), int(out_fp8)
@@ -158,6 +175,11 @@
     elif isinstance(a0, PreSplitF32) or isinstance(w, PreSplitF32):
         raise RuntimeError("gemm: a pre-split operand outside the split16 mode (set_f32_split changed after the weights were packed: "
                            "call prepare() / begin() again)")
+    if phase:
+        if stats or gn is not None or m is not None or out.shape[0] < out_rows:
+            raise PhaseConvRefused("gemm: the phase form has no tile sums / fused GroupNorm / row override")
+        if lib.tt_gemm_plan(C.byref(g), (C.c_int32 * 7)()) != 0:
+            raise PhaseConvRefused(lib.tt_last_error().decode(errors="replace"))
     need = lib.tt_gemm_ws_bytes(C.byref(g))
     if need:
         ws = _workspace(need, a0.device)
@@ -185,6 +207,9 @@
         cfg = (C.c_int32 * 7)()
         lib.tt_gemm_plan(C.byref(g), cfg)
         taps = 9 if mode in (1, 3) else (3 if mode == 2 else 1)
+        nph = 1
+        if phase:
+            taps, nph = 4, 4 if conv[6] == 6 else 1
         tag = _TAG[g.dtype]
         if cfg[3] == 0 and cfg[1] == 320:
             kname = f"gemm_w320{'h' if cfg[0] == 128 else ''}_kernel<{tag}, {mode}, {int(bool(ln_fold))}>"
@@ -193,13 +218,25 @@
         elif cfg[0] == 32 and cfg[1] == 320:
             kname = f"sq320_kernel<{tag}, {'true' if residual is not None else 'false'}>"
         else:
-            kmode = (5 if mode == 3 else mode if not ln_fold else 2 + ln_fold) + (8 if (g.dtype == TT_F32 and _F32_SPLIT) else 0)
-            if mode == 3:
+            kmode = (6 if phase else 5 if mode == 3 else mode if not ln_fold else 2 + ln_fold) + (8 if (g.dtype == TT_F32 and _F32_SPLIT) else 0)
+            if mode == 3 or phase:
                 kmode += 16 if g.presplit & 2 else 0
             kname = f"gemm_kernel<{tag}, {', '.join(str(v) for v in cfg[:6])}, {kmode}>"
-        _prof_end(ev, kname, 2.0 * g.m * n * taps * (g.k0 + g.k1),
-                  shape=(mode, g.m, n, taps * (g.k0 + g.k1), int(geglu), int(residual is not None)))
-    return out
+        _prof_end(ev, kname, 2.0 * g.m * nph * n * taps * (g.k0 + g.k1),
+                  shape=(mode, g.m * nph, n, taps * (g.k0 + g.k1), int(geglu), int(residual is not None)))
+    return out
+
+
+UPSAMPLE_PHASES = os.environ.get("TT_UPSAMPLE_PHASES", "1") != "0"
+
+
+def upsample_conv3x3(x, w, w_up2, nimg: int, h: int, wd: int, *, bias=None, stats: int = 0, phases: Optional[bool] = None):
+    if (UPSAMPLE_PHASES if phases is None else phases) and w_up2 is not None:
+        try:
+            return gemm(x, w_up2, mode=1, conv=(nimg, h, wd, 2 * h, 2 * wd, 1, 6), bias=bias)
+        except PhaseConvRefused:
+            pass
+    return gemm(x, w, mode=1, conv=(nimg, h, wd, 2 * h, 2 * wd, 1, 1), bias=bias, stats=stats)
 
 
 CONV3X3_FUSED = os.environ.get("TT_CONV3X3", "0") == "1"
diff --git a/this_and_that_vdm_amd/packing.py b/this_and_that_vdm_amd/packing.py
--- a/this_and_that_vdm_amd/packing.py
+++ b/this_and_that_vdm_amd/packing.py
@@ -8,6 +8,19 @@
 def pack_conv3x3(w: torch.Tensor) -> torch.Tensor:
     o, i = w.shape[:2]
     return w.permute(0, 2, 3, 1).reshape(o, 9 * i).contiguous()
+
+
+def pack_conv3x3_up2(w: torch.Tensor, dtype: torch.dtype) -> torch.Tensor:
+    o, i = w.shape[:2]
+    acc = w.detach().to(torch.float64 if w.dtype in (torch.float32, torch.float64) else torch.float32)
+    groups = (((0,), (1, 2)), ((0, 1), (2,)))
+    out = torch.empty((4, o, 4, i), dtype=acc.dtype, device=w.device)
+    for py in range(2):
+        for px in range(2):
+            for ty in range(2):
+                for tx in range(2):
+                    out[2 * py + px, :, 2 * ty + tx] = sum(acc[:, :, ky, kx] for ky in groups[py][ty] for kx in groups[px][tx])
+    return out.reshape(4, o, 4 * i).to(dtype).contiguous()
 
 
 def pack_tconv3(w: torch.Tensor) -> torch.Tensor:
diff --git a/this_and_that_vdm_amd/svd/autoencoder_kl_temporal_decoder.py b/this_and_that_vdm_amd/svd/autoencoder_kl_temporal_decoder.py
--- a/this_and_that_vdm_amd/svd/autoencoder_kl_temporal_decoder.py
+++ b/this_and_that_vdm_amd/svd/autoencoder_kl_temporal_decoder.py
@@ -94,7 +94,7 @@
     def __init__(self, in_channels: int, out_channels: int, num_layers: int = 1, add_upsample: bool = True):
         super().__init__()
         self.resnets = nn.ModuleList([_res(in_channels if i == 0 else out_channels, out_channels) for i in range(num_layers)])
-        self.upsamplers = nn.ModuleList([Upsample2D(out_channels, use_conv=True, out_channels=out_channels)]) if add_upsample else None
+        self.upsamplers = nn.ModuleList([Upsample2D(out_channels, use_conv=True, out_channels=out_channels, tile_sums_read=True)]) if add_upsample else None
 
     def pack(self, reg, dtype):
         for m in self.resnets:
diff --git a/this_and_that_vdm_amd/svd/denoiser_base.py b/this_and_that_vdm_amd/svd/denoiser_base.py
--- a/this_and_that_vdm_amd/svd/denoiser_base.py
+++ b/this_and_that_vdm_amd/svd/denoiser_base.py
@@ -25,7 +25,7 @@
 
 
 _PRESPLIT_ATTRS = {
-    "ResnetBlock2D": ("w1", "w2", "ws"), "TemporalResnetBlock": ("w1", "w2"), "Downsample2D": ("w",), "Upsample2D": ("w",),
+    "ResnetBlock2D": ("w1", "w2", "ws"), "TemporalResnetBlock": ("w1", "w2"), "Downsample2D": ("w",), "Upsample2D": ("w", "w_up2"),
     "FeedForward": ("wg", "w2"), "BasicTransformerBlock": ("wqkv", "wo1", "wo2"), "TemporalBasicTransformerBlock": ("wqkv", "wo1", "wo2"),
     "TransformerSpatioTemporalModel": ("w_in", "w_out"),
 }
diff --git a/this_and_that_vdm_amd/svd/layers.py b/this_and_that_vdm_amd/svd/layers.py
--- a/this_and_that_vdm_amd/svd/layers.py
+++ b/this_and_that_vdm_amd/svd/layers.py
@@ -9,7 +9,7 @@
 import torch.nn as nn
 
 from .. import ops
-from ..packing import fold_layernorm, pack_conv1x1, pack_conv3x3, pack_geglu, pack_tconv3, permute_q_rows, zero_sum_round
+from ..packing import fold_layernorm, pack_conv1x1, pack_conv3x3, pack_conv3x3_up2, pack_geglu, pack_tconv3, permute_q_rows, zero_sum_round
 
 
 ZERO_CTX_TEMPORAL = os.environ.get("TT_ZERO_CTX_T", "1") != "0"
@@ -350,17 +350,19 @@
 
 class Upsample2D(_Packable):
     def __init__(self, channels: int, use_conv: bool = False, use_conv_transpose: bool = False,
-                 out_channels: Optional[int] = None, name: str = "conv"):
+                 out_channels: Optional[int] = None, name: str = "conv", tile_sums_read: bool = False):
         super().__init__()
         if not use_conv or use_conv_transpose:
             raise NotImplementedError("SVD uses Upsample2D(use_conv=True)")
         self.conv = nn.Conv2d(channels, out_channels or channels, 3, padding=1)
+        self.tile_sums_read = tile_sums_read
 
     def pack(self, reg, dtype):
         self.w, self.b = pack_conv3x3(self.conv.weight.detach().to(dtype)), _f32(self.conv.bias)
+        self.w_up2 = None if self.tile_sums_read else pack_conv3x3_up2(self.conv.weight.detach(), dtype).flatten(0, 1)
 
     def forward(self, x, g: Geom):
-        out = ops.gemm(x, self.w, mode=1, conv=(g.n, g.h, g.w, 2 * g.h, 2 * g.w, 1, 1), bias=self.b, stats=4 * g.hw)
+        out = ops.upsample_conv3x3(x, self.w, self.w_up2, g.n, g.h, g.w, bias=self.b, stats=4 * g.hw)
         return out, Geom(g.batch, g.frames, 2 * g.h, 2 * g.w, g.batch0, g.batch_total, g.requests)
 
 
```
